# NilsJochem/audio-matcher

Hardware: AMD Instinct MI355X
Metric: audio samples/s matched (whole node), 10 s needle vs 1 h haystack, 1/2/4/8 GPU (higher is better)
Workload: dtype f32

## Files before the change

audio-matcher_amd/csrc/am_api.hip:

```cpp
#include "am_internal.h"

#include <climits>

using namespace am;


static size_t mode_len(size_t w, size_t s, int mode) {
    if (mode == AM_MODE_FULL) return w + s - 1;
    if (mode == AM_MODE_SAME) return w;
    return (w > s ? w - s : 0) + 1;
}


int am::find_peaks_host_array(Ctx* c, const float* d_scores, long long n, float min_prom, long long min_dist,
                              std::vector<am_peak>& all) {
    int rc;
    const PeakPolicy pol = snapshot_opts(nullptr).peak_policy();
    Segment sg; sg.a = 0; sg.b = n;
    PeakArena arena{};
    if ((rc = prepare_results(c, 1, AM_MAX_PEAKS_PER_CHUNK, &arena))) return rc;
    if ((rc = c->side[0].peaks.ensure(sizeof(am_peak) * AM_MAX_PEAKS_PER_CHUNK))) return rc;
    if ((rc = upload_segments(c, std::vector<Segment>(1, sg)))) return rc;
    if ((rc = launch_pick(c, c->side[0], d_scores, n, 0, 1, min_prom, min_dist, nullptr, nullptr, 0, arena, pol))) return rc;
    AM_HIP(hipStreamSynchronize(c->stream));
// ... 460 lines not shown
    AM_HIP(launch_synth(c->stream, d_out, seed, stream, first, (long long)n, amp));
    AM_HIP(hipStreamSynchronize(c->stream));
    return AM_OK;
}

int am_axpy_device(int device, float* d_dst, const float* d_src, size_t n, float gain) {
    if (!d_dst || !d_src) return fail(AM_ERR_INVALID_ARG, "null pointer");
    Ctx* c = nullptr;
    int rc = get_ctx(device, &c);
    if (rc) return rc;
    if (n == 0) return AM_OK;
    std::lock_guard<std::recursive_mutex> lk(c->mu);
    AM_HIP(launch_axpy(c->stream, d_dst, d_src, (long long)n, gain));
    AM_HIP(hipStreamSynchronize(c->stream));
    return AM_OK;
}

int am_synth_pcm16_stereo_device(int device, int16_t* d_out, uint32_t seed, uint32_t stream, uint64_t first, size_t frames, float amp) {
    if (!d_out) return fail(AM_ERR_INVALID_ARG, "null pointer");
    Ctx* c = nullptr;
    int rc = get_ctx(device, &c);
    if (rc) return rc;
    if (frames == 0) return AM_OK;
    std::lock_guard<std::recursive_mutex> lk(c->mu);
    AM_HIP(launch_synth_pcm16(c->stream, d_out, seed, stream, first, (long long)frames, amp));
    AM_HIP(hipStreamSynchronize(c->stream));
    return AM_OK;
}

int am_add_pcm16_device(int device, int16_t* d_dst, const int16_t* d_src, size_t frames) {
    if (!d_dst || !d_src) return fail(AM_ERR_INVALID_ARG, "null pointer");
    Ctx* c = nullptr;
    int rc = get_ctx(device, &c);
    if (rc) return rc;
    if (frames == 0) return AM_OK;
    std::lock_guard<std::recursive_mutex> lk(c->mu);
    AM_HIP(launch_add_pcm16(c->stream, d_dst, d_src, (long long)frames));
    AM_HIP(hipStreamSynchronize(c->stream));
    return AM_OK;
}


int am_debug_column_bench(int device, int wide, int npairs, int iters, int dense, double* k1_ms, double* k3_ms) {
    Ctx* c = nullptr;
    int rc = get_ctx(device, &c);
    if (rc) return rc;
    std::lock_guard<std::recursive_mutex> lk(c->mu);
    if (npairs < 1 || npairs > 64 || iters < 1 || !k1_ms || !k3_ms) return fail(AM_ERR_INVALID_ARG, "bad arguments");
    const Plan* pl = nullptr;
    if ((rc = wide ? get_plan(c, 23, &pl, 9) : get_plan(c, 22, &pl))) return rc;
    const long long N = 1ll << pl->dev.logN, s = 441000, hop = ((N - s + 1) / kTile) * kTile;
    const long long nblocks = 2ll * npairs, out_count = nblocks * hop, src_len = out_count + s - 1 + kTile;
    DevBuf src, work, scores, stats32, side;
    struct Release { DevBuf* b[5]; ~Release() { for (DevBuf* x : b) x->release(); } } release_all{{&src, &work, &scores, &stats32, &side}};
    if ((rc = src.ensure((size_t)src_len * 4)) || (rc = work.ensure((size_t)npairs * (size_t)N * sizeof(float2))) ||
        (rc = scores.ensure((size_t)out_count * 4)) || (rc = stats32.ensure((size_t)(out_count / 32) * sizeof(float2))) ||
        (rc = side.ensure(sparse_bytes(nblocks, pl->dev)))) return rc;
    AM_HIP(launch_synth(c->stream, (float*)src.p, 7, 1, 0, src_len, 0.25f));
    Job job{};
    job.src = src.p; job.src_len = src_len; job.lead = 0; job.src_kind = 0;
    job.dst = (float*)scores.p; job.out_count = out_count; job.hop = (int)hop; job.nblocks = (int)nblocks; job.first_pair = 0;
    ScanCfg scan{};
    fill_scan_cfg(&scan, stats32.p, side.p, nblocks, pl->dev, dense ? -1.0f : 1e30f, FLT_MAX, 60 * 44100, 70 * 44100 - s);
    hipEvent_t e[3];
    for (auto& x : e) AM_HIP(hipEventCreate(&x));
    double t1 = 0, t3 = 0;
    for (int it = -2; it < iters; ++it) {
        AM_HIP(hipEventRecord(e[0], c->stream));
        AM_HIP(launch_k1(c->stream, job, npairs, (float2*)work.p, pl->dev, 0));
        AM_HIP(hipEventRecord(e[1], c->stream));
        AM_HIP(launch_k3(c->stream, job, npairs, (const float2*)work.p, pl->dev, 1e-3f, scan, 0, false));
        AM_HIP(hipEventRecord(e[2], c->stream));
        AM_HIP(hipStreamSynchronize(c->stream));
        float a = 0, b = 0;
        AM_HIP(hipEventElapsedTime(&a, e[0], e[1]));
        AM_HIP(hipEventElapsedTime(&b, e[1], e[2]));
        if (it >= 0) { t1 += a; t3 += b; }
    }
    for (auto& x : e) (void)hipEventDestroy(x);
    *k1_ms = t1 / iters; *k3_ms = t3 / iters;
    return AM_OK;
}

}
```

audio-matcher_amd/csrc/am_context.hip:

```cpp
#include "am_internal.h"

namespace am {

thread_local std::string t_err;

int fail(int code, const std::string& msg) {
    t_err = msg;
    return code;
}
int hip_fail(hipError_t e, const char* what) {
    char buf[256];
    snprintf(buf, sizeof(buf), "%s: %s", what, hipGetErrorString(e));
    t_err = buf;
    return e == hipErrorOutOfMemory ? AM_ERR_OOM : AM_ERR_HIP;
}

static std::mutex g_hooks_mu;
static Hooks g_hooks;
Hooks snapshot_hooks() {
    std::lock_guard<std::mutex> lk(g_hooks_mu);
    return g_hooks;
}

using OptRule = const char* (*)(long long& v);
static const char* opt_any(long long&) { return nullptr; }
static const char* opt_bool(long long& v) { v = v ? 1 : 0; return nullptr; }
static const char* opt_log_n(long long& v) { return v != 0 && (v < kLogNMin || v > kLogNMax) ? "log_n out of range" : nullptr; }
static const char* opt_half(long long& v) { v = v <= 0 ? 0 : (v >= 2 ? 2 : 1); return nullptr; }
static const char* opt_every(long long& v) { v = v < 1 ? 1 : v; return nullptr; }
static const char* opt_arm_at(long long& v) { v = v < -1 ? -2 : v; return nullptr; }
static const char* opt_needle_group(long long& v) { return v < 1 || v > kMaxNeedleGroup ? "needle_group out of range" : nullptr; }
static const char* opt_pairs(long long& v) { return v < 1 || v > 64 ? "pairs_per_group out of range" : nullptr; }
static const char* opt_score_norm(long long& v) { return v < 0 || v > 1 ? "score_norm out of range (0 = off, 1 = NCC)" : nullptr; }
static const char* opt_floor_db(long long& v) { return v < 0 || v > 200 ? "score_norm_floor_db out of range (0..200)" : nullptr; }
static const char* opt_trace_form(long long& v) { return v < 0 || v > 2 ? "trace_form out of range (0 = by bin length, 1 = wave form, 2 = sliced form)" : nullptr; }
static const char* opt_distance(long long& v) {
    return v < 0 || v > 3 ? "distance_rule out of range (bit 0: inclusive, bit 1: between plateau starts)" : nullptr;
}
struct Option {
    const char* name;
    std::atomic<long long> value;
    OptRule rule;
    long long Opts::*field;
};
static Option g_options[] = {
    {"log_n", {0}, opt_log_n, &Opts::log_n},
    {"pairs_per_group", {64}, opt_pairs, &Opts::pairs_per_group},
    {"profile_mask", {-1}, opt_any, &Opts::profile_mask},
    {"profile_every", {1}, opt_every, &Opts::profile_every},
    {"half_pipeline", {0}, opt_half, &Opts::half},
    {"batch_overlap", {1}, opt_bool, &Opts::batch_overlap},
    {"needle_group", {8}, opt_needle_group, &Opts::needle_group},
    {"pick_stream_priority", {0}, opt_bool, &Opts::pick_priority},
    {"pick_group", {1}, opt_bool, &Opts::pick_group},
    {"k3_group", {1}, opt_bool, &Opts::k3_group},
    {"host_pick_wait", {1}, opt_bool, &Opts::host_pick_wait},
    {"device_redo", {1}, opt_bool, &Opts::device_redo},
    {"tail_block", {1}, opt_bool, &Opts::tail_block},
    {"dense_scores", {0}, opt_bool, &Opts::dense},
    {"score_norm", {0}, opt_score_norm, &Opts::score_norm},
    {"score_norm_floor_db", {60}, opt_floor_db, &Opts::score_norm_floor_db},
    {"debug_no_realloc", {0}, opt_bool, &Opts::debug_no_realloc},
    {"debug_redo_arm_at", {-2}, opt_arm_at, &Opts::debug_redo_arm_at},
    {"trace_form", {0}, opt_trace_form, &Opts::trace_form},
    {"peak_filter_order", {0}, opt_bool, &Opts::peak_filter_order},
    {"distance_rule", {0}, opt_distance, &Opts::distance_rule},
    {"tail_window", {0}, opt_bool, &Opts::tail_window},
    {"surrounding_from", {0}, opt_bool, &Opts::surrounding_from},
};
static Option* find_option(const char* key) {
    for (Option& r : g_options)
        if (!strcmp(key, r.name)) return &r;
    return nullptr;
}

thread_local const Opts* t_opts_pin = nullptr;
Opts snapshot_opts(const am_needle* h) {
    if (t_opts_pin) return *t_opts_pin;
    Opts o;
    for (const Option& r : g_options) o.*r.field = r.value.load(std::memory_order_relaxed);
    if (h && h->opt_log_n >= 0) o.log_n = h->opt_log_n;
    if (h && h->opt_half >= 0) o.half = h->opt_half;
    if (h && h->opt_score_norm >= 0) o.score_norm = h->opt_score_norm;
    return o;
}

thread_local int t_no_realloc = 0;
int realloc_refused(const char* what, size_t bytes, size_t cap) {
    char buf[160];
    snprintf(buf, sizeof(buf), "debug_no_realloc: %s buffer would grow from %zu to %zu bytes while a call is queueing", what, cap, bytes);
    return fail(AM_ERR_HIP, buf);
}

static const char* kKernelNames[] = {"k1_cols_fwd", "k2_rows", "k3_cols_inv", "tile_stats", "peaks", "other", "trace", "discover"};
static std::mutex g_ctx_mu;
static std::map<int, Ctx*> g_ctx;

int get_ctx(int device, Ctx** out) {
    std::lock_guard<std::mutex> lk(g_ctx_mu);
    int n = 0;
    hipError_t e = hipGetDeviceCount(&n);
    if (e != hipSuccess || n <= 0) return fail(AM_ERR_NO_DEVICE, "no HIP device available");
    if (device < 0 || device >= n) return fail(AM_ERR_NO_DEVICE, "device ordinal out of range");
    auto it = g_ctx.find(device);
    if (it != g_ctx.end()) { *out = it->second; AM_HIP(hipSetDevice(device)); return AM_OK; }
    AM_HIP(hipSetDevice(device));
    (void)hipSetDeviceFlags(hipDeviceScheduleSpin);
    (void)hipGetLastError();
    AM_HIP(fft_kernels_init());
    Ctx* c = new Ctx();
    c->device = device;
    c->hdr.flags = hipHostMallocMapped | hipHostMallocCoherent;
    c->failcnt.flags = hipHostMallocMapped | hipHostMallocCoherent;
    c->spill.flags = hipHostMallocMapped | hipHostMallocCoherent;
    hipError_t se = hipStreamCreateWithFlags(&c->stream, hipStreamNonBlocking);
    if (se != hipSuccess) { delete c; return hip_fail(se, "hipStreamCreate"); }
    {
        int least = 0, greatest = 0;
        if (snapshot_opts(nullptr).pick_priority && hipDeviceGetStreamPriorityRange(&least, &greatest) == hipSuccess && least != greatest)
            (void)hipStreamCreateWithPriority(&c->stream2, hipStreamNonBlocking, least);
        else
            (void)hipStreamCreateWithFlags(&c->stream2, hipStreamNonBlocking);
        (void)hipGetLastError();
    }
    (void)hipStreamCreateWithFlags(&c->stream_tail, hipStreamNonBlocking);
    (void)hipEventCreateWithFlags(&c->ev_fork, kSyncEvent);
    (void)hipEventCreateWithFlags(&c->ev_join, kSyncEvent);
    (void)hipGetLastError();
    for (int i = 0; i < 2; ++i) {
        (void)hipEventCreateWithFlags(&c->ev_k3[i], kSyncEvent);
        (void)hipEventCreateWithFlags(&c->ev_pick[i], kSyncEvent);
    }
    g_ctx[device] = c;
    *out = c;
    return AM_OK;
}

static hipEvent_t prof_event(Ctx* c) {
    if (!c->pool.empty()) { hipEvent_t e = c->pool.back(); c->pool.pop_back(); return e; }
    hipEvent_t e = nullptr;
    (void)hipEventCreateWithFlags(&e, AM_EVENT_NO_SYSTEM_FENCE ? hipEventDisableSystemFence : hipEventDefault);
// ... 445 lines not shown
```

audio-matcher_amd/csrc/am_correlate.hip:

```cpp
#include "am_internal.h"

namespace am {

static int pick_log_n(size_t s, long long out_count, const Opts& o, int* logN_out) {
    int min_log = kLogNMin;
    while (min_log <= kLogNMax && ((size_t)1 << min_log) < s + 1) ++min_log;
    if (min_log > kLogNMax) return fail(AM_ERR_INVALID_ARG, "needle too long for a forced transform size (2^23 at most; leave log_n at 0 for needle partitioning)");
    if (o.log_n > 0) {
        int l = (int)o.log_n;
        if (l < min_log) l = min_log;
        if (l > kLogNMax) l = kLogNMax;
        *logN_out = l;
        return AM_OK;
    }
    const long long span = out_count + (long long)s - 1;
    if (span > (1ll << 19)) {
        if ((long long)s <= kWideFromSamples) { *logN_out = 21; return AM_OK; }
        if ((long long)s <= kWidestFromSamples) {
            long long hop21 = (1ll << 21) - (long long)s + 1;
            if (hop21 >= 8 * kTile) hop21 = (hop21 / kTile) * kTile;
            *logN_out = (hop21 > 0 && out_count <= 2 * hop21) ? 21 : 22;
            return AM_OK;
        }
        if ((long long)s <= kSegmentFrom) {
            long long hop22 = (1ll << 22) - (long long)s + 1;
            if (hop22 >= 8 * kTile) hop22 = (hop22 / kTile) * kTile;
            *logN_out = (hop22 > 0 && out_count <= 2 * hop22) ? 22 : 23;
            return AM_OK;
        }
    }
    int pref = min_log;
    while (pref < kLogNMax) {
        const double n = (double)((size_t)1 << pref);
        if ((n - (double)s + 1.0) / n >= kMinEfficiency) break;
        ++pref;
    }
    int single = kLogNMin;
    while (single < kLogNMax && (long long)((size_t)1 << single) < span) ++single;
    *logN_out = std::min(pref, std::max(single, min_log));
    return AM_OK;
}

int plan_geometry(size_t s, long long out_count, const Opts& o, Geometry* g) {
    int rc = pick_log_n(s, out_count, o, &g->logN);
    if (rc) return rc;
    g->N = 1ll << g->logN;
    g->hop = g->N - (long long)s + 1;
    if (g->hop >= 8 * kTile) g->hop = (g->hop / kTile) * kTile;
    g->nblocks = (out_count + g->hop - 1) / g->hop;
    g->npairs = (g->nblocks + 1) / 2;
    return AM_OK;
}
bool tail_plan(size_t s, long long out_count, const Opts& o, const Geometry& g, TailPlan* t) {
    t->on = false;
    if (!o.tail_block || o.log_n != 0 || g.logN < 22 || !(g.nblocks & 1) || g.nblocks < 3 || (g.hop % kTile) != 0) return false;
    const long long T = (g.nblocks - 1) * g.hop, rest = out_count - T;
    for (int lt = 21; lt < g.logN; ++lt) {
        const long long N = 1ll << lt;
        long long hop = N - (long long)s + 1;
        if (hop < 8 * kTile) continue;
        hop = (hop / kTile) * kTile;
        if (2 * hop < rest) continue;
        t->on = true; t->T = T;
        t->g.logN = lt; t->g.N = N; t->g.hop = hop; t->g.nblocks = (rest + hop - 1) / hop; t->g.npairs = 1;
        return true;
    }
    return false;
}

static size_t sparse_word_bytes(long long nblocks, const PlanDev& pl) {
    return sizeof(unsigned long long) * (size_t)nblocks * ballot_layout(pl.logN1, pl.logN2).words;
}
size_t sparse_bytes(long long nblocks, const PlanDev& pl) {
    return sparse_word_bytes(nblocks, pl) + sizeof(float) * (size_t)nblocks * ballot_layout(pl.logN1, pl.logN2).tiles;
}
void fill_scan_cfg(ScanCfg* cfg, void* stats32, void* side, long long nblocks, const PlanDev& pl, float margin, float hist_min,
                          long long seg_c, long long seg_d) {
    cfg->stats32 = static_cast<float2*>(stats32);
    cfg->wbits = static_cast<unsigned long long*>(side);
    cfg->tile_theta = reinterpret_cast<float*>(static_cast<char*>(side) + sparse_word_bytes(nblocks, pl));
    cfg->margin = margin;
    cfg->hist_min = hist_min;
    cfg->seg_c = seg_c; cfg->seg_d = seg_d;
    cfg->inv_c = seg_c > 0 ? 1.0 / (double)seg_c : 0.0;
}
SparseScores sparse_view(const ScanCfg& cfg, long long hop, const PlanDev& pl) {
    if (cfg.margin < 0.0f) return SparseScores{nullptr, cfg.stats32, nullptr, (int)hop, pl.logN2, pl.logN1, 1.0 / (double)hop};
    return SparseScores{cfg.wbits, cfg.stats32, cfg.tile_theta, (int)hop, pl.logN2, pl.logN1, 1.0 / (double)hop};
}

bool needle_is_segmented(const am_needle* h, const Opts& o) {
    return (long long)h->n > kSegmentFrom && o.log_n == 0;
}
static void needle_segments(am_needle* h) {
    if (!h->segments.empty()) return;
    const long long n = (long long)h->n;
    const long long nseg = (n + kSegmentLen - 1) / kSegmentLen;
    for (long long i = 0; i < nseg; ++i) {
        const long long a = n * i / nseg, b = n * (i + 1) / nseg;
        am_needle* sub = new am_needle();
        sub->ctx = h->ctx; sub->d_needle = h->d_needle + a; sub->n = (size_t)(b - a);
        sub->inv_autocorr = h->inv_autocorr; sub->owns_data = false;
        h->segments.push_back(sub);
        h->seg_off.push_back(a);
    }
}

bool plan_fuses_scan(const PlanDev& pl, const Geometry& g) { return plan_has_scan(pl) && (g.hop % kTile) == 0; }

int pass_plan(am_needle* h, const Opts& o, long long out_count, bool allow_tail, PassPlan* pp) {
    Ctx* c = h->ctx;
    *pp = PassPlan{};
    int rc;
    if (needle_is_segmented(h, o)) {
        pp->kind = PassKind::Partitioned;
        needle_segments(h);
        Opts os = o;
        os.half = 0;
        pp->parts.resize(h->segments.size());
        for (size_t i = 0; i < pp->parts.size(); ++i) {
            if ((rc = pass_plan(h->segments[i], os, out_count, false, &pp->parts[i]))) return rc;
            pp->need.work = std::max(pp->need.work, pp->parts[i].need.work);
        }
        return AM_OK;
    }
    if (h->n <= (size_t)kDirectMaxNeedle && o.log_n == 0) return AM_OK;
    pp->kind = PassKind::Transform;
    Geometry& g = pp->g;
    if ((rc = plan_geometry(h->n, out_count, o, &g))) return rc;
    if ((rc = get_plan(c, g.logN, &pp->pl))) return rc;
    if ((rc = needle_k2_spectrum(h, o, pp->pl, &pp->hc, &pp->hs))) return rc;
    pp->fused = plan_fuses_scan(pp->pl->dev, g);
    if (allow_tail && pp->fused && c->stream_tail && c->ev_fork && c->ev_join && tail_plan(h->n, out_count, o, g, &pp->tail)) {
        if ((rc = get_plan(c, pp->tail.g.logN, &pp->tail_pl))) return rc;
        if ((rc = needle_k2_spectrum(h, o, pp->tail_pl, &pp->tail_hc, &pp->tail_hs))) return rc;
        pp->need.work_tail = (size_t)pp->tail.g.N * sizeof(float2);
    }
    pp->nblocks = pp->tail.on ? g.nblocks - 1 : g.nblocks;
    pp->npairs = pp->tail.on ? g.npairs - 1 : g.npairs;
    pp->main_count = pp->tail.on ? pp->tail.T : out_count;
    pp->ppg = std::min(std::max<long long>(1, o.pairs_per_group), pp->npairs);
    pp->need.work = (size_t)pp->ppg * (size_t)g.N * sizeof(float2);
    pp->need.npairs = g.npairs;
    if (pp->fused) {
        pp->need.stats32 = (size_t)((out_count + 31) / 32) * sizeof(float2);
        pp->need.side = sparse_bytes(g.nblocks, pp->pl->dev);
    }
    return AM_OK;
}

static int run_tail_block(Ctx* c, const PassPlan& pp, const void* d_src, long long src_len,
                          float* d_dst, long long out_count, float factor, const ScanCfg& main_scan, int src_kind) {
    hipStream_t st = c->stream_tail;
    const TailPlan& tail = pp.tail;
    const PlanDev& pl = pp.tail_pl->dev;
    const HalfScale& hs = pp.tail_hs;
    int rc;
    if ((rc = c->work_tail.ensure(pp.need.work_tail))) return rc;
    Job job = tail_job(tail, d_src, src_len, out_count, src_kind);
    job.dst = d_dst + tail.T;
    ScanCfg scan{};
    scan.stats32 = main_scan.stats32 ? main_scan.stats32 + tail.T / 32 : nullptr;
    scan.margin = -1.0f; scan.hist_min = FLT_MAX;
    { ProfScope ps(c, KN_OTHER, st); AM_HIP(launch_k1(st, job, 1, (float2*)c->work_tail.p, pl, hs.level)); }
    { ProfScope ps(c, KN_OTHER, st); AM_HIP(launch_k2(st, 1, (float2*)c->work_tail.p, pp.tail_hc, pl, nullptr, hs.level, hs.hscale, hs.pre, true)); }
    { ProfScope ps(c, KN_OTHER, st); AM_HIP(launch_k3(st, job, 1, (const float2*)c->work_tail.p, pl, hs.k3(factor), scan, hs.level, false)); }
    if (main_scan.stats32 && main_scan.margin >= 0.0f && main_scan.wbits && main_scan.tile_theta) {
        const BallotLayout bl = ballot_layout(pp.pl->dev.logN1, pp.pl->dev.logN2);
        const size_t blk = (size_t)(pp.g.nblocks - 1);
        AM_HIP(hipMemsetAsync(main_scan.wbits + blk * bl.words, 0xFF, bl.words * sizeof(unsigned long long), st));
        AM_HIP(hipMemsetD32Async(reinterpret_cast<hipDeviceptr_t>(main_scan.tile_theta + blk * bl.tiles), (int)0xFF7FFFFFu, bl.tiles, st));
    }
    return AM_OK;
}

static int run_correlation_one(am_needle* h, const PassPlan& pp, const void* d_src, long long src_len, long long lead,
                               float* d_dst, long long out_count, float factor,
                               const ScanRequest* scan_req, ScanResult* res, int src_kind, bool accumulate);

int run_correlation(am_needle* h, const Opts& o, const void* d_src, long long src_len, long long lead,
                           float* d_dst, long long out_count, float factor,
                           const ScanRequest* scan_req, ScanResult* res, int src_kind, const PassPlan* plan) {
    int rc;
    PassPlan own;
    if (!plan) {
        if ((rc = pass_plan(h, o, out_count, scan_req && !scan_req->no_scan && lead == 0, &own))) return rc;
        plan = &own;
    }
    if (res) { res->fused = false; res->redo_ok = false; res->sparse = plain_scores(); }
    if (plan->kind != PassKind::Partitioned) return run_correlation_one(h, *plan, d_src, src_len, lead, d_dst, out_count, factor, scan_req, res, src_kind, false);
    if (scan_req && scan_req->skip_launch) return fail(AM_ERR_INVALID_ARG, "internal: streaming ingest does not run early pairs for partitioned needles");
    for (size_t i = 0; i < plan->parts.size(); ++i) {
        ScanRequest plain{};
        if (scan_req) {
            plain.margin = -1.0f; plain.range_a = scan_req->range_a; plain.range_b = scan_req->range_b;
            plain.before_k3 = i == 0 ? scan_req->before_k3 : nullptr;
            plain.no_scan = true;
        }
        if ((rc = run_correlation_one(h->segments[i], plan->parts[i], d_src, src_len, lead - h->seg_off[i], d_dst, out_count, factor,
                                      scan_req ? &plain : nullptr, nullptr, src_kind, i > 0)))
            return rc;
    }
    return AM_OK;
}

static int run_correlation_one(am_needle* h, const PassPlan& pp, const void* d_src, long long src_len, long long lead,
                               float* d_dst, long long out_count, float factor,
                               const ScanRequest* scan_req, ScanResult* res, int src_kind, bool accumulate) {
    Ctx* c = h->ctx;
    Job job{};
    job.src = d_src; job.src_len = src_len; job.lead = lead; job.src_kind = src_kind;
    job.dst = d_dst; job.out_count = out_count;
    if (pp.kind == PassKind::Direct) {
        ProfScope ps(c, KN_OTHER);
        AM_HIP(launch_direct(c->stream, job, h->d_needle, (int)h->n, factor));
        return AM_OK;
    }
    int rc;
    const PlanDev& pl = pp.pl->dev;
    const HalfScale& hs = pp.hs;
    const TailPlan& tail = pp.tail;
    const long long N = pp.g.N, hop = pp.g.hop, npairs = pp.npairs, ppg = pp.ppg;
    const ScanBuffers out = (scan_req && scan_req->out.work) ? scan_req->out : scan_buffers(c->side[0]);
    DevBuf& wk = *out.work;
    if ((rc = wk.ensure((size_t)ppg * (size_t)N * sizeof(float2)))) return rc;
    ScanCfg scan{};
    bool fused = false;
    if (scan_req && !scan_req->no_scan) {
        if (res) res->sparse = SparseScores{nullptr, nullptr, nullptr, (int)hop, pl.logN2, pl.logN1, 1.0 / (double)hop};
        if (pp.fused) {
            const long long side_blocks = std::max(pp.g.nblocks, scan_req->side_nblocks);
            if ((rc = out.stats32->ensure((size_t)((out_count + 31) / 32) * sizeof(float2)))) return rc;
            if ((rc = out.wflags->ensure(sparse_bytes(side_blocks, pl)))) return rc;
            fill_scan_cfg(&scan, out.stats32->p, out.wflags->p, side_blocks, pl, scan_req->margin, scan_req->hist_min, scan_req->seg_c, scan_req->seg_d);
            fused = true;
            if (res) { res->fused = true; res->sparse = sparse_view(scan, hop, pl); }
        }
    }
    const float k3scale = hs.k3(factor);
    job.out_count = pp.main_count; job.hop = (int)hop; job.nblocks = (int)pp.nblocks;
    if (scan_req && scan_req->skip_launch) return AM_OK;
    long long pair_lo = 0, pair_hi = npairs;
    bool with_tail = tail.on;
    if (scan_req && scan_req->range_b > scan_req->range_a) {
        pair_lo = (scan_req->range_a / hop) / 2;
        pair_hi = std::min(npairs, ((scan_req->range_b - 1) / hop) / 2 + 1);
        with_tail = tail.on && scan_req->range_b > tail.T;
    }
    if (scan_req && scan_req->tail_by_caller) with_tail = false;
// ... 268 lines not shown
```

audio-matcher_amd/csrc/am_engine.hip:

```cpp
#include "am_internal.h"

namespace am {

static int launch_pick_group(Ctx* c, const K3Group& kg, long long n_scores, int seg_off, int nsegs, float min_prom, long long min_dist,
                             const SparseScores& sp_common, int* bad, const int* hdr_off, const PeakArena& arena, const PeakPolicy& pol,
                             hipStream_t st) {
    if (nsegs == 0 || n_scores <= 0 || kg.n <= 0) return AM_OK;
    int rc;
    const size_t nz = (size_t)kg.n, total = nz * (size_t)nsegs;
    const long long ntiles = (n_scores + kTile - 1) / kTile;
    PickGroup pg{};
    pg.n = kg.n;
    for (int z = 0; z < kg.n; ++z) {
        if ((rc = c->grp_stats[z].ensure((size_t)ntiles * sizeof(float2)))) return rc;
        pg.g[z] = kg.dst[z]; pg.stats[z] = static_cast<float2*>(c->grp_stats[z].p);
        pg.stats32[z] = kg.stats32[z]; pg.wbits[z] = kg.wbits[z]; pg.theta[z] = kg.tile_theta[z];
        pg.hdr_off[z] = hdr_off[z];
    }
    { ProfScope ps(c, KN_STATS, st);
      AM_HIP(launch_stats_reduce(st, pg.stats32[0], n_scores, pg.stats[0], bad, &pg)); }
    if ((rc = wide_reserve(c, total))) return rc;
    if ((rc = c->side[0].peaks.ensure(total * AM_MAX_PEAKS_PER_CHUNK * sizeof(am_peak)))) return rc;
    {
        ProfScope ps(c, KN_PEAKS, st);
// ... 56 lines not shown
            ScoreSide& sd = c->side[set];
            if ((rc = sd.scores.ensure(max_scores * sizeof(float)))) return rc;
            if ((rc = sd.peaks.ensure(sizeof(am_peak) * max_segs * AM_MAX_PEAKS_PER_CHUNK))) return rc;
            if ((rc = sd.stats.ensure((max_scores + kTile - 1) / kTile * sizeof(float2)))) return rc;
        }
        return wide_reserve(c, max_segs);
    }
    int wait_pick(bool on_host) {
        if (!overlap || seq < 2) return AM_OK;
        if (on_host) AM_HIP(hipEventSynchronize(c->ev_pick[set()]));
        else AM_HIP(hipStreamWaitEvent(c->stream, c->ev_pick[set()], 0));
        return AM_OK;
    }
    int k3_done() {
        if (!overlap) return AM_OK;
        AM_HIP(hipEventRecord(c->ev_k3[set()], c->stream));
        AM_HIP(hipStreamWaitEvent(c->stream2, c->ev_k3[set()], 0));
        return AM_OK;
    }
    int pick_done() {
        if (overlap) AM_HIP(hipEventRecord(c->ev_pick[set()], c->stream2));
        ++seq;
        return AM_OK;
    }
    int drain() {
        AM_HIP(hipStreamSynchronize(c->stream));
        if (overlap) AM_HIP(hipStreamSynchronize(c->stream2));
        return AM_OK;
    }
};

static int match_alone(am_needle* h, const void* d_hay, size_t len, const am_match_params* p, am_peak* out, size_t cap, size_t slot,
                       size_t* n_out, int src_kind, const PartSpec* part, int* worst) {
    const int rc = match_many(h, &d_hay, &len, 1, p, out ? out + slot * cap : nullptr, cap, &n_out[slot], src_kind, 0, 1, false, nullptr, part);
    if (rc == AM_ERR_CAPACITY) *worst = rc;
    return rc == AM_ERR_CAPACITY ? AM_OK : rc;
}

static int pick_alone(am_needle* h, const Opts& o, const am_match_params* p, const void* src, long long src_len, float factor,
                      const ScanRequest& req, long long n_scores, int seg_idx, const Segment& sg, int spare_hdr, uint64_t shift, int src_kind,
                      const NormSpec& nrm, std::vector<am_peak>& all) {
    Ctx* c = h->ctx;
    const PeakPolicy pol = o.peak_policy();
    int rc;
    PeakArena own{};
    if ((rc = c->spill.ensure(sizeof(am_peak) * AM_MAX_PEAKS_PER_CHUNK))) return rc;
    AM_HIP(hipMemsetAsync(c->arena_cur.p, 0, sizeof(unsigned), c->stream));
    own.base = static_cast<am_peak*>(c->spill.p); own.cursor = static_cast<unsigned*>(c->arena_cur.p);
    own.cap = AM_MAX_PEAKS_PER_CHUNK;
    ScoreSide& side = c->side[0];
    if ((rc = side.scores.ensure((size_t)n_scores * sizeof(float)))) return rc;
    float* d_scores = (float*)side.scores.p;
    ScanResult res{};
    if ((rc = run_correlation(h, o, src, src_len, 0, d_scores, n_scores, factor, &req, &res, src_kind))) return rc;
    if (nrm.on) {
        if ((rc = normalise_scores(c, c->stream, nrm, src, src_len, src_kind, 0, (long long)h->n, d_scores, sg.a, std::min(sg.b, n_scores))))
            return rc;
        res.fused = false;
    }
    if ((rc = launch_pick(c, side, d_scores, n_scores, seg_idx, 1, p->min_prominence, (long long)p->min_distance, nullptr, &res, spare_hdr, own, pol))) return rc;
    AM_HIP(hipStreamSynchronize(c->stream));
    const SegHeader& hd = static_cast<const SegHeader*>(c->hdr.p)[spare_hdr];
    const size_t old = all.size();
    if (hd.overflow & 1) {
        if ((rc = pick_chunk_big(c, d_scores, n_scores, seg_idx, sg, p->min_prominence, (long long)p->min_distance, &res, hd.seg_min, all, pol)))
            return rc;
    } else append_header_peaks(hd, own, all);
    for (size_t j = old; j < all.size(); ++j) { all[j].start += shift; all[j].end += shift; }
    return AM_OK;
}

struct TailSlots { size_t scores, stats; };
static bool tail_batchable(const TailPlan& t) { return t.on && t.g.logN == 21; }
static int launch_tail_batch(am_needle* h, const std::vector<PassPlan>& plans, const std::vector<size_t>& members, int half_idx,
                             const TailSlots& sl, const void* const* d_hays, const size_t* lens, float factor, int src_kind) {
    Ctx* c = h->ctx;
    const PassPlan& lead = plans[members[0]];
    const TailPlan& first = lead.tail;
    const Plan* pl = lead.tail_pl;
    const float2* hc = lead.tail_hc;
    const HalfScale& hs = lead.tail_hs;
    TailBatch tb{};
    tb.n = (int)members.size();
    for (int j = 0; j < tb.n; ++j) {
        const size_t k = members[j];
        const size_t slot = (size_t)half_idx * kMaxTailBatch + (size_t)j;
        const Job job = tail_job(plans[k].tail, d_hays[k], (long long)lens[k], (long long)(lens[k] - h->n + 1), src_kind);
        tb.src[j] = job.src;
        tb.src_len[j] = job.src_len;
        tb.out_count[j] = job.out_count;
        tb.dst[j] = static_cast<float*>(c->tail_scores.p) + slot * sl.scores;
        tb.stats32[j] = static_cast<float2*>(c->tail_stats.p) + slot * sl.stats;
    }
    float2* work = static_cast<float2*>(c->work_tail.p);
    { ProfScope ps(c, KN_OTHER); AM_HIP(launch_tail_batch_k1(c->stream, tb, (int)first.g.hop, src_kind, work, pl->dev, hs.level)); }
    { ProfScope ps(c, KN_OTHER); AM_HIP(launch_k2(c->stream, tb.n, work, hc, pl->dev, nullptr, hs.level, hs.hscale, hs.pre, true)); }
    { ProfScope ps(c, KN_OTHER); AM_HIP(launch_tail_batch_k3(c->stream, tb, (int)first.g.hop, work, pl->dev, hs.k3(factor), hs.level)); }
    return AM_OK;
}

static int classify_nonfinite(am_needle* h, const PassPlan& pp, const float* d_hay, size_t len,
                              const std::vector<Segment>& segs, int s0, int s1,
                              std::vector<char>* drop, std::vector<char>* again) {
    Ctx* c = h->ctx;
    const long long s = (long long)h->n;
    const int nch = s1 - s0;
    drop->assign(nch, 0); again->assign(nch, 0);
    std::vector<Segment> ranges;
    for (int i = s0; i < s1; ++i)
        ranges.push_back(Segment{segs[i].a, std::min<long long>((long long)len, segs[i].b + s - 1)});
    const long long npairs = pp.kind == PassKind::Transform ? pp.npairs : 0;
    for (long long q = 0; q < npairs; ++q) ranges.push_back(pp.pair_reads(q, (long long)len));
    if (pp.tail.on) ranges.push_back(pp.tail_reads((long long)len));
    std::vector<int> flags(ranges.size(), 0);
    int rc = nonfinite_flags(c, d_hay, ranges.data(), (int)ranges.size(), flags.data());
    if (rc) return rc;
    for (int i = 0; i < nch; ++i) {
        if (flags[i]) { (*drop)[i] = 1; continue; }
        if (pp.kind == PassKind::Partitioned) { (*again)[i] = 1; continue; }
        const Segment sg = segs[s0 + i];
        for (long long q = 0; q < npairs && !(*again)[i]; ++q)
            if (flags[nch + q] && 2 * q * pp.g.hop < sg.b && (2 * q + 2) * pp.g.hop > sg.a) (*again)[i] = 1;
        if (pp.tail.on && flags[nch + npairs] && pp.tail.T < sg.b) (*again)[i] = 1;
    }
    return AM_OK;
}

int match_many(am_needle* h, const void* const* d_hays, const size_t* lens, size_t n_hay,
               const am_match_params* p, am_peak* out, size_t cap_per_hay, size_t* n_out, int src_kind,
               size_t index_base, size_t index_stride, bool fire_hooks, const StreamPre* pre, const PartSpec* part) {
    Ctx* c = h->ctx;
    const Opts o = snapshot_opts(h);
    const PeakPolicy pol = o.peak_policy();
    Hooks hooks = fire_hooks ? snapshot_hooks() : Hooks{};
    if (part) hooks.fn = nullptr;
    if (part && n_hay != 1) return fail(AM_ERR_INVALID_ARG, "internal: a part is one haystack");
    auto G = [&](size_t k) { return index_base + k * index_stride; };
    const size_t s = h->n;
    if (p->chunk == 0) return fail(AM_ERR_INVALID_ARG, "chunk must be > 0");
    if (p->scale < AM_SCALE_NONE || p->scale > AM_SCALE_MY) return fail(AM_ERR_INVALID_ARG, "bad scale");
    const NormSpec nrm = norm_spec(h, o);
    if (nrm.on && (pre || part)) return fail(AM_ERR_INVALID_ARG, AM_NORM_UNSUPPORTED);
    int rc = norm_check(nrm, p->scale);
    if (rc) return rc;
    const bool my = p->scale == AM_SCALE_MY;
    const float factor = nrm.on ? norm_factor(nrm) : scale_factor(h, p->scale, (size_t)(p->chunk + p->overlap));
    const int sm = p->scale == AM_SCALE_LIB ? 1 : 0;
    ScanRequest base{};
    base.margin = nrm.on ? -1.0f : write_margin(o, p);
    const bool sparse_ok = base.margin >= 0.0f;
    base.hist_min = nrm.on ? FLT_MAX : h->hist_min(sm);
    base.seg_c = (long long)p->chunk;
    base.seg_d = (long long)(p->chunk + p->overlap) - (long long)s;
    for (size_t k = 0; k < n_hay; ++k) n_out[G(k)] = 0;
    ChunkPlan cp;
    plan_chunks(s, d_hays, lens, n_hay, p, o, my, part ? part->max_windows : (size_t)-1, &cp);
    const std::vector<Segment>& segs = cp.segs;
    const std::vector<int>& seg_off = cp.seg_off;
    const size_t nsegs = segs.size();
    if (nsegs == 0 && cp.short_segs.empty()) return AM_OK;
    if (cp.too_many(1)) return fail(AM_ERR_INVALID_ARG, "chunk size too small for this haystack (more than 2^18 chunks)");
    size_t n_active = 0;
    for (size_t k = 0; k < n_hay; ++k) n_active += cp.ns(k) > 0;
    ScoreSets sets(c, o, n_active);
    if ((rc = sets.size(cp.max_scores, cp.max_segs))) return rc;
    std::vector<PassPlan> plans(n_hay);
    Footprint need;
    for (size_t k = 0; k < n_hay; ++k) {
        if (cp.n_chunks[k] == 0 || cp.ns(k) == 0) continue;
        if ((rc = pass_plan(h, o, (long long)(lens[k] - s + 1), pre == nullptr, &plans[k]))) return rc;
        need.take(plans[k].need);
    }
    std::vector<int> tail_slot(n_hay, -1);
    TailSlots tslots{0, 0};
    bool batch_tails = false;
    if (need.work_tail) {
        size_t n_tails = 0;
        for (size_t k = 0; k < n_hay; ++k)
            if (tail_batchable(plans[k].tail)) {
                ++n_tails;
// ... 289 lines not shown
        tail_plan(s, out_count, o, geo[k], &tails[k]);
    }
    std::map<int, std::vector<const float2*>> hcs;
    auto spectra = [&](int logN) -> int {
        if (hcs.count(logN)) return AM_OK;
        const Plan* pl = nullptr;
        int rc2 = get_plan(c, logN, &pl);
        std::vector<const float2*>& v = hcs[logN];
        v.resize(m);
        HalfScale hs;
        for (size_t i = 0; i < m && !rc2; ++i) rc2 = needle_k2_spectrum(needles[ord[i]], o, pl, &v[i], &hs);
        return rc2;
    };
    for (size_t k = 0; k < n_hay; ++k)
        if (ns_max(k) > 0 && (rc = spectra(geo[k].logN))) return rc;
    const size_t group_opt = (size_t)std::min<long long>(std::max<long long>(1, o.needle_group), kMaxNeedleGroup);
    {
        const bool groups_ok = o.k3_group && group_opt > 1 && m > 1 && !o.half && (m % group_opt) != 1 && c->stream_tail != nullptr;
        for (size_t k = 0; k < n_hay; ++k) {
            if (!tails[k].on) continue;
            const Plan* plk = nullptr;
            if (ns_max(k) == 0 || !groups_ok || !tail_batchable(tails[k]) || get_plan(c, geo[k].logN, &plk) || !plan_is_c512(plk->dev)) {
                tails[k].on = false;
                continue;
            }
            max_tail = std::max(max_tail, (size_t)tails[k].g.N);
            if ((rc = spectra(tails[k].g.logN))) return rc;
        }
        if (max_tail) {
            if ((rc = c->work_tail.ensure(std::max(c->work_tail.cap, max_tail * sizeof(float2))))) return rc;
            if ((rc = c->work_tail2.ensure(std::min(group_opt, m) * max_tail * sizeof(float2)))) return rc;
        }
    }
    size_t n_pairs_active = 0;
    for (size_t k = 0; k < n_hay; ++k) n_pairs_active += ns_max(k) > 0 ? m : 0;
    ScoreSets sets(c, o, n_pairs_active);
    DevBuf& fwd = c->side[0].work;
    if ((rc = fwd.ensure(max_matrix * sizeof(float2)))) return rc;
    if ((rc = c->work2.ensure(std::min(group_opt, m) * max_matrix * sizeof(float2)))) return rc;
    if ((rc = sets.size(max_scores, max_segs))) return rc;
    for (int set = 0; set < sets.count(); ++set) {
        if ((rc = c->side[set].stats32.ensure((max_scores + 31) / 32 * sizeof(float2)))) return rc;
        if ((rc = c->side[set].wflags.ensure(max_wflags))) return rc;
    }
    const size_t k3_group = (o.k3_group && group_opt > 1 && m > 1 && !o.half && max_wflags > 0) ? std::min(group_opt, m) : 0;
    for (int set = 0; set < sets.count(); ++set)
        for (size_t q = 0; q < k3_group; ++q) {
            if ((rc = c->grp_scores[set][q].ensure(max_scores * sizeof(float)))) return rc;
            if ((rc = c->grp_stats32[set][q].ensure((max_scores + 31) / 32 * sizeof(float2)))) return rc;
            if ((rc = c->grp_wflags[set][q].ensure(max_wflags))) return rc;
        }
    if (k3_group && o.pick_group) {
        const size_t total = k3_group * max_segs;
        for (size_t z = 0; z < k3_group; ++z)
            if ((rc = c->grp_stats[z].ensure((max_scores + kTile - 1) / kTile * sizeof(float2)))) return rc;
        if ((rc = wide_reserve(c, total))) return rc;
        if ((rc = c->side[0].peaks.ensure(total * AM_MAX_PEAKS_PER_CHUNK * sizeof(am_peak)))) return rc;
    }
    PeakArena arena{};
    if ((rc = prepare_results(c, nhdr, nhdr * 8 + 4096, &arena))) return rc;
    if ((rc = upload_segments(c, all_segs))) return rc;
    if ((rc = c->badflag.ensure(sizeof(int) * n_hay))) return rc;
    int* h_bad = static_cast<int*>(c->badflag.p);
    memset(h_bad, 0, sizeof(int) * n_hay);
    SegHeader* h_hdr = static_cast<SegHeader*>(c->hdr.p);
    const float margin = write_margin(o, p);
    QueueingScope queueing(o.debug_no_realloc != 0);
    for (size_t k = 0; k < n_hay; ++k) {
        if (ns_max(k) == 0) continue;
        if (hooks.fn) hooks.fn(hooks.user, G(k), 0, (size_t)ns_max(k));
        const Geometry& g = geo[k];
        const Plan* pl = nullptr;
        if ((rc = get_plan(c, g.logN, &pl))) return rc;
        const std::vector<const float2*>& hc = hcs[g.logN];
        const long long out_count = (long long)(lens[k] - s_min + 1);
        const int half = (o.half && (plan_is_r16(pl->dev) || plan_is_c512(pl->dev))) ? (o.half >= 2 ? 2 : 1) : 0;
        const size_t group = (!half && plan_k2_has_group(pl->dev)) ? group_opt : 1;
        const size_t matrix = (size_t)g.npairs * (size_t)g.N;
        const bool fused = plan_fuses_scan(pl->dev, g);
        const TailPlan& tail = tails[k];
        const int main_pairs = (int)(tail.on ? g.npairs - 1 : g.npairs);
        const Plan* plt = nullptr;
        Job job{}, job_t{};
        job.src = d_hays[k]; job.src_len = (long long)lens[k]; job.lead = 0; job.src_kind = src_kind;
        job.out_count = tail.on ? tail.T : out_count; job.hop = (int)g.hop; job.nblocks = (int)(tail.on ? g.nblocks - 1 : g.nblocks); job.first_pair = 0;
        { ProfScope ps(c, KN_K1); AM_HIP(launch_k1(c->stream, job, main_pairs, (float2*)fwd.p, pl->dev, half)); }
        if (tail.on) {
            if ((rc = get_plan(c, tail.g.logN, &plt))) return rc;
            job_t = tail_job(tail, d_hays[k], (long long)lens[k], out_count, src_kind);
            ProfScope ps(c, KN_OTHER);
            AM_HIP(launch_k1(c->stream, job_t, 1, (float2*)c->work_tail.p, plt->dev, 0));
        }
        for (size_t i = 0; i < m; ++i) {
            am_needle* h = needles[ord[i]];
            const size_t in_group = i % group;
            const float2* inv_rows = (const float2*)c->work2.p + in_group * matrix;
            const size_t gn = std::min(group, m - (i - in_group));
            if (group > 1 && in_group == 0) {
                K2Group grp{};
                grp.n = (int)gn;
                for (int q = 0; q < grp.n; ++q) { grp.hc[q] = hc[i + q]; grp.dst[q] = (float2*)c->work2.p + (size_t)q * matrix; }
                { ProfScope ps(c, KN_K2); AM_HIP(launch_k2_group(c->stream, main_pairs, (const float2*)fwd.p, grp, pl->dev)); }
                if (tail.on) {
                    K2Group gt{};
                    gt.n = (int)gn;
                    const std::vector<const float2*>& hct = hcs[tail.g.logN];
                    for (int q = 0; q < gt.n; ++q) { gt.hc[q] = hct[i + q]; gt.dst[q] = (float2*)c->work_tail2.p + (size_t)q * (size_t)tail.g.N; }
                    ProfScope ps(c, KN_OTHER);
                    AM_HIP(launch_k2_group(c->stream, 1, (const float2*)c->work_tail.p, gt, plt->dev));
                }
            }
            const bool grouped_k3 = k3_group && group > 1 && gn > 1 && fused && !half && plan_k3_has_group(pl->dev);
            if (grouped_k3 && in_group != 0) continue;
            const int set = sets.set();
            if (grouped_k3) {
                K3Group kg{};
                kg.n = (int)gn;
                ScanResult scans[kMaxNeedleGroup];
                int* const bad = (src_kind == 0 || o.half) ? &h_bad[k] : nullptr;
                ScanCfg common{};
                bool same_plan = true, same_edges = true;
                for (size_t q = 0; q < gn; ++q) {
                    am_needle* hq = needles[ord[i + q]];
                    ScanCfg cfg{};
                    fill_scan_cfg(&cfg, c->grp_stats32[set][q].p, c->grp_wflags[set][q].p, g.nblocks, pl->dev, margin, hq->hist_min(sm),
                                  (long long)p->chunk, (long long)(p->chunk + pj[ord[i + q]].overlap) - (long long)hq->n);
                    scans[q] = ScanResult{};
                    scans[q].fused = true;
                    scans[q].sparse = sparse_view(cfg, g.hop, pl->dev);
                    if (q == 0) common = cfg;
                    same_plan = same_plan && plan_of[i + q] == plan_of[i];
                    same_edges = same_edges && cfg.seg_d == common.seg_d;
                    kg.work[q] = (const float2*)c->work2.p + q * matrix;
                    kg.dst[q] = (float*)c->grp_scores[set][q].p;
                    kg.stats32[q] = cfg.stats32; kg.wbits[q] = cfg.wbits; kg.tile_theta[q] = cfg.tile_theta;
                    kg.hist_min[q] = cfg.hist_min;
                    kg.out_scale[q] = half_scale(hq, o, pl->dev).k3(scale_factor(hq, p->scale, 1));
                    kg.out_count[q] = std::max(0ll, std::min(count_of(k, i + q), job.out_count));
                    kg.seg_d[q] = cfg.seg_d;
                }
                kg.seg_c = common.seg_c; kg.inv_c = common.inv_c;
                if (!same_edges) common.seg_c = 0;
                if ((rc = sets.wait_pick(false))) return rc;
                { ProfScope ps(c, KN_K3); AM_HIP(launch_k3_group(c->stream, job, main_pairs, kg, pl->dev, common)); }
                if (tail.on) {
                    K3Group kt = kg;
                    for (size_t q = 0; q < gn; ++q) {
                        kt.work[q] = (const float2*)c->work_tail2.p + q * (size_t)tail.g.N;
                        kt.dst[q] = kg.dst[q] + tail.T; kt.stats32[q] = kg.stats32[q] + tail.T / 32;
                        kt.wbits[q] = nullptr; kt.tile_theta[q] = nullptr; kt.hist_min[q] = FLT_MAX;
                        kt.out_count[q] = std::max(0ll, count_of(k, i + q) - tail.T);
                        kt.seg_d[q] = 0;
                    }
                    kt.seg_c = 0; kt.inv_c = 0.0;
                    ScanCfg dense{};
                    dense.stats32 = kt.stats32[0]; dense.margin = -1.0f; dense.hist_min = FLT_MAX;
                    ProfScope ps(c, KN_OTHER);
                    AM_HIP(launch_k3_group(c->stream, job_t, 1, kt, plt->dev, dense));
                    if (margin >= 0.0f)
                        AM_HIP(launch_tail_preset_group(c->stream, kg, (long long)(g.nblocks - 1), pl->dev.logN1, pl->dev.logN2));
                }
                if ((rc = sets.k3_done())) return rc;
                if (o.pick_group && same_plan && plan_i(i).ns(k) > 0) {
                    int hoff[kMaxNeedleGroup];
                    for (size_t q = 0; q < gn; ++q) hoff[q] = hdr_of(k, i + q);
                    if ((rc = launch_pick_group(c, kg, count_of(k, i), seg_of(k, i), plan_i(i).ns(k), p->min_prominence, (long long)p->min_distance,
                                                scans[0].sparse, bad, hoff, arena, pol, sets.pick_stream()))) return rc;
                } else
                for (size_t q = 0; q < gn; ++q)
                    if (plan_i(i + q).ns(k) > 0 &&
                        (rc = launch_pick(c, c->side[0], kg.dst[q], count_of(k, i + q), seg_of(k, i + q), plan_i(i + q).ns(k), p->min_prominence,
                                          (long long)p->min_distance, bad, &scans[q], hdr_of(k, i + q), arena, pol, sets.pick_stream()))) return rc;
                if ((rc = sets.pick_done())) return rc;
                continue;
            }
            const int ns = plan_i(i).ns(k);
            if (ns == 0) continue;
            float* d_scores = sets.scores();
            Job jn = job;
            jn.dst = d_scores;
            jn.out_count = std::min(count_of(k, i), job.out_count);
            ScoreSide& side = sets.side();
            int* const bad = (src_kind == 0 || o.half) ? &h_bad[k] : nullptr;
            ScanResult scan{};
            scan.fused = fused;
            scan.sparse = SparseScores{nullptr, nullptr, nullptr, (int)g.hop, pl->dev.logN2, pl->dev.logN1, 1.0 / (double)g.hop};
            ScanCfg cfg{};
            if (fused) {
                fill_scan_cfg(&cfg, side.stats32.p, side.wflags.p, g.nblocks, pl->dev, margin, h->hist_min(sm), (long long)p->chunk,
                              (long long)(p->chunk + pj[ord[i]].overlap) - (long long)h->n);
                scan.sparse = sparse_view(cfg, g.hop, pl->dev);
            }
            const float factor = scale_factor(h, p->scale, 1);
            const HalfScale hs = half_scale(h, o, pl->dev);
            if (group == 1) {
                ProfScope ps(c, KN_K2);
                AM_HIP(launch_k2(c->stream, (int)g.npairs, (float2*)fwd.p, hc[i], pl->dev, (float2*)c->work2.p, hs.level, hs.hscale, hs.pre));
            }
            if ((rc = sets.wait_pick(false))) return rc;
            { ProfScope ps(c, KN_K3); AM_HIP(launch_k3(c->stream, jn, (int)g.npairs, inv_rows, pl->dev, hs.k3(factor), cfg, half)); }
            if ((rc = sets.k3_done())) return rc;
            if ((rc = launch_pick(c, side, d_scores, count_of(k, i), seg_of(k, i), ns, p->min_prominence, (long long)p->min_distance,
                                  bad, &scan, hdr_of(k, i), arena, pol, sets.pick_stream()))) return rc;
            if ((rc = sets.pick_done())) return rc;
        }
    }
    queueing.end();
    if ((rc = sets.drain())) return rc;
    std::vector<am_peak> all;
    std::vector<std::pair<size_t, size_t>> redo;
    for (size_t k = 0; k < n_hay; ++k) {
        for (size_t i = 0; i < m; ++i) {
            const int ns = plan_i(i).ns(k);
            if (ns == 0) continue;
            const size_t j = ord[i];
            const SegHeader* hd = h_hdr + hdr_of(k, i);
            const size_t slot = G(k) * nn + j;
            bool again = h_bad[k] != 0;
            float lowest = FLT_MAX;
            for (int q = 0; q < ns && !again; ++q) {
                if (hd[q].overflow & 7) again = true;
                lowest = std::min(lowest, hd[q].seg_min);
            }
            if (!again) needles[j]->remember_min(sm, lowest);
            if (again) { redo.emplace_back(k, j); continue; }
            all.clear();
            for (int q = 0; q < ns; ++q) append_header_peaks(hd[q], arena, all);
            rc = merge_peaks(all, &pj[j], o.surrounding_from != 0, out ? out + slot * cap_per_pair : nullptr, cap_per_pair, &n_out[slot]);
            if (rc == AM_ERR_CAPACITY) worst = rc;
            else if (rc) return rc;
        }
    }
    for (const auto& kj : redo)
        if ((rc = match_alone(needles[kj.second], d_hays[kj.first], lens[kj.first], &pj[kj.second], out, cap_per_pair, G(kj.first) * nn + kj.second,
                              n_out, src_kind, nullptr, &worst))) return rc;
    if (hooks.fn)
        for (size_t k = 0; k < n_hay; ++k)
            if (ns_max(k) > 0) hooks.fn(hooks.user, G(k), 1, (size_t)ns_max(k));
    return worst;
}

// ... 2 lines not shown
```

audio-matcher_amd/csrc/am_fft.hip:

```cpp
#include "am_kernels.h"

#include <float.h>
#include <stdlib.h>
#include <algorithm>
#include <atomic>
#include <hip/hip_fp16.h>

namespace am {

__device__ __forceinline__ float2 cadd(float2 a, float2 b) { return make_float2(a.x + b.x, a.y + b.y); }
__device__ __forceinline__ float2 csub(float2 a, float2 b) { return make_float2(a.x - b.x, a.y - b.y); }
__device__ __forceinline__ float2 cmul(float2 a, float2 b) {
    return make_float2(a.x * b.x - a.y * b.y, a.x * b.y + a.y * b.x);
}
__device__ __forceinline__ float2 cmulc(float2 a, float2 b) {
    return make_float2(a.x * b.x + a.y * b.y, a.y * b.x - a.x * b.y);
}
__device__ __forceinline__ float2 mul_neg_i(float2 a) { return make_float2(a.y, -a.x); }
__device__ __forceinline__ float2 mul_pos_i(float2 a) { return make_float2(-a.y, a.x); }

__device__ __forceinline__ float2 tw_big(const PlanDev& pl, unsigned m) {
    return cmul(pl.twhi[m >> pl.logLo], pl.twlo[m & ((1u << pl.logLo) - 1u)]);
}

// ... 263 lines not shown
struct K1Twiddles { float2 w256, w256q, base0, base1, step0, step1, step0q, step1q; };
__device__ __forceinline__ K1Twiddles k1_twiddles(const PlanDev& pl, long long col, int hi) {
    const unsigned maskN = (unsigned)((1ll << pl.logN) - 1);
    K1Twiddles w;
    w.w256 = pl.tw1[hi];
    w.w256q = pl.tw1[4 * hi];
    w.base0 = tw_big(pl, ((unsigned)col * (unsigned)hi) & maskN);
    w.base1 = tw_big(pl, (((unsigned)col + 1u) * (unsigned)hi) & maskN);
    tw_big_pair(pl, ((unsigned)col * 16u) & maskN, w.step0, w.step0q);
    tw_big_pair(pl, (((unsigned)col + 1u) * 16u) & maskN, w.step1, w.step1q);
    return w;
}
template <int KIND>
__device__ __forceinline__ void k1_load(const Job& job, long long col, int in_stride, int hi, long long baseA, long long baseB,
                                        bool validB, bool fast, float2 (&x0)[16], float2 (&x1)[16]) {
    if (fast) {
#pragma unroll
        for (int a = 0; a < 16; ++a) {
            const long long off = (long long)(a * 16 + hi) * in_stride + col;
            const float2 va = load_sample2<KIND>(job.src, baseA + off), vb = load_sample2<KIND>(job.src, baseB + off);
            x0[a] = make_float2(va.x, vb.x);
            x1[a] = make_float2(va.y, vb.y);
        }
    } else {
#pragma unroll
        for (int a = 0; a < 16; ++a) {
            const long long n = (long long)(a * 16 + hi) * in_stride + col;
            const float2 va = load2_padded<KIND>(job.src, baseA + n, job.src_len);
            const float2 vb = validB ? load2_padded<KIND>(job.src, baseB + n, job.src_len) : make_float2(0.f, 0.f);
            x0[a] = make_float2(va.x, vb.x);
            x1[a] = make_float2(va.y, vb.y);
        }
    }
}
__device__ __forceinline__ void k1_transform(const K1Twiddles& w, float2* lds2, int hi, int cp, float2 (&x0)[16], float2 (&x1)[16]) {
    dif<16, false>(x0);
    dif<16, false>(x1);
    twiddle_brev<16, false>(x0, w.w256, w.w256q);
    twiddle_brev<16, false>(x1, w.w256, w.w256q);
#pragma unroll
    for (int ap = 0; ap < 16; ++ap) lds2[(ap * 16 + hi) * 17 + cp] = x0[brev<16>(ap)];
    __syncthreads();
#pragma unroll
    for (int b = 0; b < 16; ++b) x0[b] = lds2[(hi * 16 + b) * 17 + cp];
    __syncthreads();
#pragma unroll
    for (int ap = 0; ap < 16; ++ap) lds2[(ap * 16 + hi) * 17 + cp] = x1[brev<16>(ap)];
    __syncthreads();
#pragma unroll
    for (int b = 0; b < 16; ++b) x1[b] = lds2[(hi * 16 + b) * 17 + cp];
    dif<16, false>(x0);
    dif<16, false>(x1);
    twiddle_chain<16, false, true>(x0, w.base0, w.step0, w.step0q);
    twiddle_chain<16, false, true>(x1, w.base1, w.step1, w.step1q);
}
template <int KIND>
__device__ __forceinline__ void k1_tile(const Job& job, const PlanDev& pl, float2* lds2, long long col, int in_stride,
                                        int hi, int cp, long long baseA, long long baseB, bool validB, bool fast,
                                        float2 (&x0)[16], float2 (&x1)[16]) {
    const K1Twiddles w = k1_twiddles(pl, col, hi);
    k1_load<KIND>(job, col, in_stride, hi, baseA, baseB, validB, fast, x0, x1);
    k1_transform(w, lds2, hi, cp, x0, x1);
}

__device__ __forceinline__ void k1_transform_h16(const K1Twiddles& w, uint2* ldsu, int hi, int cp, h2 (&x0)[16], h2 (&x1)[16]) {
    dif<16, false>(x0);
    dif<16, false>(x1);
    twiddle_apply2<16, false, true>(x0, x1, w.w256);
#pragma unroll
    for (int ap = 0; ap < 16; ++ap) ldsu[(ap * 16 + hi) * 17 + cp] = make_uint2(h2_bits(x0[brev<16>(ap)]), h2_bits(x1[brev<16>(ap)]));
    __syncthreads();
#pragma unroll
    for (int b = 0; b < 16; ++b) {
        const uint2 v = ldsu[(hi * 16 + b) * 17 + cp];
        x0[b] = bits_h2(v.x);
        x1[b] = bits_h2(v.y);
    }
    dif<16, false>(x0);
    dif<16, false>(x1);
    twiddle_chain<16, false, true>(x0, w.base0, w.step0);
    twiddle_chain<16, false, true>(x1, w.base1, w.step1);
}

template <int KIND, int HALF>
__device__ __forceinline__ void k1_cols_fwd_r16_tile(const Job& job, float2* __restrict__ work, const PlanDev& pl) {
    extern __shared__ float4 lds4[];
    const int t = threadIdx.x;
    const int hi = t >> 4, cp = t & 15;
    const int n2_0 = blockIdx.x << kColsLog;
    const int pair = job.first_pair + blockIdx.y;
    const long long blkA = 2ll * pair, blkB = blkA + 1;
    const bool validB = blkB < job.nblocks;
    const long long N = 1ll << pl.logN;
    const long long baseA = blkA * job.hop - job.lead;
    const long long baseB = blkB * job.hop - job.lead;
    const bool fast = ((reinterpret_cast<uintptr_t>(job.src) & 7) == 0) && ((baseA & 1) == 0) && ((baseB & 1) == 0) &&
                      baseA >= 0 && baseA + N <= job.src_len && validB && baseB + N <= job.src_len;
    float2 x0[16], x1[16];
    if constexpr (HALF == 2) {
        const long long col = (long long)n2_0 + 2 * cp;
        const K1Twiddles w = k1_twiddles(pl, col, hi);
        k1_load<KIND>(job, col, kN2, hi, baseA, baseB, validB, fast, x0, x1);
        h2 hx0[16], hx1[16];
#pragma unroll
        for (int a = 0; a < 16; ++a) { hx0[a] = to_h2(x0[a]); hx1[a] = to_h2(x1[a]); }
        k1_transform_h16(w, reinterpret_cast<uint2*>(lds4), hi, cp, hx0, hx1);
        uint2* __restrict__ out2 = reinterpret_cast<uint2*>(reinterpret_cast<unsigned*>(work) + ((size_t)blockIdx.y << pl.logN) + n2_0) + cp;
#pragma unroll
        for (int bp = 0; bp < 16; ++bp) {
            const size_t k1 = (size_t)(hi + 16 * bp);
            out2[k1 * (kN2 / 2)] = make_uint2(h2_bits(hx0[brev<16>(bp)]), h2_bits(hx1[brev<16>(bp)]));
        }
        return;
    }
    k1_tile<KIND>(job, pl, reinterpret_cast<float2*>(lds4), (long long)n2_0 + 2 * cp, kN2, hi, cp, baseA, baseB, validB, fast, x0, x1);
    if (HALF) {
        uint2* __restrict__ out2 = reinterpret_cast<uint2*>(reinterpret_cast<unsigned*>(work) + ((size_t)blockIdx.y << pl.logN) + n2_0) + cp;
#pragma unroll
        for (int bp = 0; bp < 16; ++bp) {
            const size_t k1 = (size_t)(hi + 16 * bp);
            out2[k1 * (kN2 / 2)] = make_uint2(pack_h2(x0[brev<16>(bp)]), pack_h2(x1[brev<16>(bp)]));
        }
        return;
    }
    float4* __restrict__ out4 = reinterpret_cast<float4*>(work + ((size_t)blockIdx.y << pl.logN) + n2_0) + cp;
#pragma unroll
    for (int bp = 0; bp < 16; ++bp) {
        const size_t k1 = (size_t)(hi + 16 * bp);
        out4[k1 * (kN2 / 2)] = make_float4(x0[brev<16>(bp)].x, x0[brev<16>(bp)].y,
                                             x1[brev<16>(bp)].x, x1[brev<16>(bp)].y);
    }
}
template <int KIND, int HALF>
__global__ void __launch_bounds__(256, 3)
k1_cols_fwd_r16(Job job, float2* __restrict__ work, PlanDev pl) {
    k1_cols_fwd_r16_tile<KIND, HALF>(job, work, pl);
}
template <int KIND, int HALF>
__global__ void __launch_bounds__(256, 3)
tail_cols_fwd_r16(TailBatch tb, int hop, float2* __restrict__ work, PlanDev pl) {
    const unsigned z = blockIdx.y;
    Job job;
    job.src = tb.src[z]; job.src_len = tb.src_len[z]; job.lead = 0; job.dst = nullptr; job.out_count = tb.out_count[z];
    job.hop = hop; job.nblocks = (int)((tb.out_count[z] + hop - 1) / hop); job.first_pair = -(int)z; job.src_kind = KIND;
    k1_cols_fwd_r16_tile<KIND, HALF>(job, work, pl);
}

__device__ __forceinline__ void wave_sync_lds() {
    __builtin_amdgcn_fence(__ATOMIC_ACQ_REL, "wavefront");
    __builtin_amdgcn_wave_barrier();
}

struct K2Lane {
    int t, hi, cp;
    unsigned voff;
    float2 wj0, wj1, wc0, wc1;
    float2 qj0, qj1, qc0, qc1;
};
__device__ __forceinline__ K2Lane k2_lane(const PlanDev& pl, int t = threadIdx.x) {
    K2Lane k;
    k.t = t; k.hi = k.t >> 4; k.cp = k.t & 15;
    k.voff = (unsigned)k.t * 16u;
    const float4 j = pl.k2j[2 * k.t], jq = pl.k2j[2 * k.t + 1], c = pl.k2c[2 * k.cp], cq = pl.k2c[2 * k.cp + 1];
    k.wj0 = make_float2(j.x, j.y); k.wj1 = make_float2(j.z, j.w);
    k.qj0 = make_float2(jq.x, jq.y); k.qj1 = make_float2(jq.z, jq.w);
    k.wc0 = make_float2(c.x, c.y); k.wc1 = make_float2(c.z, c.w);
    k.qc0 = make_float2(cq.x, cq.y); k.qc1 = make_float2(cq.z, cq.w);
    return k;
}

__device__ __forceinline__ void k2_forward12(const K2Lane& k, __amdgpu_buffer_rsrc_t rrow, float4* lds4) {
    const int t = k.t, hi = k.hi, cp = k.cp;
    float2 x0[16], x1[16];
#pragma unroll
    for (int a = 0; a < 16; ++a) {
        const float4 v = buf_load4(rrow, k.voff, a * 4096);
        x0[a] = make_float2(v.x, v.y);
        x1[a] = make_float2(v.z, v.w);
    }
    dif<16, false>(x0);
    dif<16, false>(x1);
    twiddle_brev<16, false>(x0, k.wj0, k.qj0);
    twiddle_brev<16, false>(x1, k.wj1, k.qj1);
#pragma unroll
    for (int ap = 0; ap < 16; ++ap)
        lds4[ap * 256 + t] = make_float4(x0[brev<16>(ap)].x, x0[brev<16>(ap)].y,
                                         x1[brev<16>(ap)].x, x1[brev<16>(ap)].y);
    __syncthreads();
#pragma unroll
    for (int b = 0; b < 16; ++b) {
        const float4 v = lds4[hi * 256 + b * 16 + cp];
        x0[b] = make_float2(v.x, v.y);
        x1[b] = make_float2(v.z, v.w);
    }
    dif<16, false>(x0);
    dif<16, false>(x1);
    twiddle_brev<16, false>(x0, k.wc0, k.qc0);
    twiddle_brev<16, false>(x1, k.wc1, k.qc1);
    wave_sync_lds();
#pragma unroll
    for (int bp = 0; bp < 16; ++bp)
        lds4[(hi * 16 + bp) * 16 + (cp ^ bp)] = make_float4(x0[brev<16>(bp)].x, x0[brev<16>(bp)].y,
                                                            x1[brev<16>(bp)].x, x1[brev<16>(bp)].y);
    wave_sync_lds();
}

__device__ __forceinline__ void k2_forward3(const K2Lane& k, const float4* lds4, float2 (&z)[32]) {
#pragma unroll
    for (int i = 0; i < 16; ++i) {
        const float4 v = lds4[k.t * 16 + (i ^ k.cp)];
        z[2 * i] = make_float2(v.x, v.y);
        z[2 * i + 1] = make_float2(v.z, v.w);
    }
    dif<32, false>(z);
}

__device__ __forceinline__ void k2_fetch_quarter(__amdgpu_buffer_rsrc_t rh, unsigned voff, int part, float4 (&h)[4]) {
#pragma unroll
    for (int i = 0; i < 4; ++i) h[i] = buf_load4(rh, voff, (part * 4 + i) * 4096);
}
__device__ __forceinline__ void k2_multiply_quarter(const float2 (&z)[32], const float4 (&h)[4], int part, float2 (&q)[32]) {
#pragma unroll
    for (int i = 0; i < 4; ++i) {
        const int e = part * 4 + i;
        q[brev<32>(2 * e)] = cmul(z[2 * e], make_float2(h[i].x, h[i].y));
        q[brev<32>(2 * e + 1)] = cmul(z[2 * e + 1], make_float2(h[i].z, h[i].w));
    }
}
// ... 632 lines not shown
#pragma unroll
    for (int a = 0; a < 16; ++a) {
        const unsigned pos = chunk ^ ((((unsigned)a & 3u) << 1) | hb);
        lds2[a * (16 << HB) + hi * 16 + (int)((pos << 1) | half)] = make_float2(c0[a], c1[a]);
    }
}
template <int HB>
__device__ __forceinline__ void scan_row_minmax(const float4* lds4, int row, bool whole, int nvalid, float& mn, float& mx) {
    const unsigned k = scan_swizzle<HB>((unsigned)row);
    float4 v[8];
#pragma unroll
    for (int i = 0; i < 8; ++i) v[i] = lds4[row * 8 + (int)((unsigned)i ^ k)];
    if (!whole) {
        mn = FLT_MAX; mx = -FLT_MAX;
#pragma unroll
        for (int i = 0; i < 8; ++i) {
            const int c0 = i << 2;
            const float e[4] = {v[i].x, v[i].y, v[i].z, v[i].w};
#pragma unroll
            for (int j = 0; j < 4; ++j)
                if (c0 + j < nvalid) { mn = fminf(mn, e[j]); mx = fmaxf(mx, e[j]); }
        }
        return;
    }
    mn = min3_raw(v[0].x, v[0].y, v[0].z); mx = max3_raw(v[0].x, v[0].y, v[0].z);
    mn = min3_raw(mn, v[0].w, v[1].x);     mx = max3_raw(mx, v[0].w, v[1].x);
#pragma unroll
    for (int i = 1; i < 8; ++i) {
        if (i > 1) { mn = min3_raw(mn, v[i - 1].w, v[i].x); mx = max3_raw(mx, v[i - 1].w, v[i].x); }
        mn = min3_raw(mn, v[i].y, v[i].z); mx = max3_raw(mx, v[i].y, v[i].z);
    }
    mn = fminf(mn, v[7].w); mx = fmaxf(mx, v[7].w);
}

__device__ __forceinline__ long long mod_recip(long long x, long long c, double inv_c) {
    long long q = (long long)((double)x * inv_c);
    long long r = x - q * c;
    if (r < 0) r += c;
    else if (r >= c) r -= c;
    return r;
}
__device__ __forceinline__ bool run_has_chunk_edge(long long lo, long long c, long long d, double inv_c) {
    if (c <= 0) return true;
    if (mod_recip(lo + 31, c, inv_c) <= 31) return true;
    const long long hi2 = lo + 31 - d;
    if (hi2 < 0) return false;
    return mod_recip(hi2, c, inv_c) <= 31;
}

struct K3Edges {
    long long outA, outB;
    int relcA, reldA, relcB, reldB;
    bool one_edge;
};
__device__ __forceinline__ K3Edges k3_edges(const Job& job, const ScanCfg& scan, long long blkA, long long blkB) {
    K3Edges e;
    e.outA = blkA * job.hop; e.outB = blkB * job.hop;
    e.one_edge = scan.stats32 != nullptr && scan.seg_c >= (long long)job.hop + 32;
    e.relcA = e.reldA = e.relcB = e.reldB = 0x7fffffff;
    if (scan.edges_n > 0) {
        const int s = (int)(blkA >> 1) - job.first_pair;
        e.relcA = scan.edge_rel[s][0]; e.reldA = scan.edge_rel[s][1];
        e.relcB = scan.edge_rel[s][2]; e.reldB = scan.edge_rel[s][3];
        return e;
    }
    if (e.one_edge) {
        const long long c = scan.seg_c, d = scan.seg_d;
        const long long m = mod_recip(e.outA, c, scan.inv_c);
        const long long ecA = m == 0 ? e.outA : e.outA + (c - m);
        long long edA = d;
        if (e.outA > d) {
            const long long m2 = mod_recip(e.outA - d, c, scan.inv_c);
            edA = m2 == 0 ? e.outA : e.outA + (c - m2);
        }
        const long long ecB = ecA >= e.outB ? ecA : ecA + c;
        const long long edB = edA >= e.outB ? edA : edA + c;
        auto rel = [](long long edge, long long start) { const long long r = edge - start; return r < 0x7fffffffll ? (int)r : 0x7fffffff; };
        e.relcA = rel(ecA, e.outA); e.reldA = rel(edA, e.outA);
        e.relcB = rel(ecB, e.outB); e.reldB = rel(edB, e.outB);
    }
    return e;
}

template <int HB, bool ACC = false, bool SCALED = false>
__device__ __forceinline__ void k3_finish(const Job& job, const ScanCfg& scan, const K3Edges& ed, float2* lds2,
                                          int n2_0, int out_stride, int t, long long blkA, long long blkB,
                                          float out_scale, const float2 (&x0)[16], const float2 (&x1)[16]) {
    const int hi = t >> 4, cp = t & 15;
    const long long col = n2_0 + 2 * cp;
    const long long outA = ed.outA, outB = ed.outB;
    const bool one_edge = ed.one_edge;
    const bool dst8 = ((reinterpret_cast<uintptr_t>(job.dst) & 7) == 0) && ((job.hop & 1) == 0);
    long long limA = job.out_count - outA; if (limA > job.hop) limA = job.hop;
    long long limB = blkB < job.nblocks ? job.out_count - outB : 0; if (limB > job.hop) limB = job.hop;
    float sa0[16], sa1[16], sb0[16], sb1[16];
#pragma unroll
    for (int a = 0; a < 16; ++a) {
        const float2 v0 = x0[brev<16>(a)], v1 = x1[brev<16>(a)];
        if (SCALED) {
            sa0[a] = v0.x; sa1[a] = v1.x;
            sb0[a] = v0.y; sb1[a] = v1.y;
        } else {
            sa0[a] = v0.x * out_scale; sa1[a] = v1.x * out_scale;
            sb0[a] = v0.y * out_scale; sb1[a] = v1.y * out_scale;
        }
    }
    unsigned wantA[2] = {0x11111111u, 0x11111111u}, wantB[2] = {0x11111111u, 0x11111111u};
    if (!ACC && scan.stats32 != nullptr) {
        const int row = scan_row_of<HB>(t);
        const int rowrun = row * out_stride + n2_0;
        const int leftA = (int)limA - rowrun, leftB = (int)limB - rowrun;
        const bool wholeA = leftA >= 32 || leftA <= 0, wholeB = leftB >= 32 || leftB <= 0;
        const float4* lds4 = reinterpret_cast<const float4*>(lds2);
        float rmnA, rmxA, rmnB, rmxB;
        __syncthreads();
        scan_put<HB>(lds2, hi, cp, sa0, sa1);
        wave_sync_lds();
        scan_row_minmax<HB>(lds4, row, wholeA, leftA < 32 ? leftA : 32, rmnA, rmxA);
        wave_sync_lds();
        scan_put<HB>(lds2, hi, cp, sb0, sb1);
        wave_sync_lds();
        scan_row_minmax<HB>(lds4, row, wholeB, leftB < 32 ? leftB : 32, rmnB, rmxB);
        float tminA = wave_min_f(leftA > 0 ? rmnA : FLT_MAX), tminB = wave_min_f(leftB > 0 ? rmnB : FLT_MAX);
        float* slots = reinterpret_cast<float*>(lds2 + scan_row_of<HB>(t & ~63) * 16);
        wave_sync_lds();
        if ((t & 63) == 0) { slots[0] = tminA; slots[1] = tminB; }
        __syncthreads();
#pragma unroll
        for (int w = 0; w < (1 << (HB - 2)); ++w) {
            const float* v = reinterpret_cast<const float*>(lds2 + scan_row_of<HB>(w * 64) * 16);
            tminA = fminf(tminA, v[0]);
            tminB = fminf(tminB, v[1]);
        }
        const bool dense = scan.margin < 0.0f;
        const float thA = dense ? -FLT_MAX : fminf(fminf(tminA, tminB), scan.hist_min) + scan.margin, thB = thA;
        bool edgeA, edgeB;
        if (one_edge) {
            edgeA = leftA > 0 && ((unsigned)(ed.relcA - rowrun) <= 31u || (unsigned)(ed.reldA - rowrun) <= 31u);
            edgeB = leftB > 0 && ((unsigned)(ed.relcB - rowrun) <= 31u || (unsigned)(ed.reldB - rowrun) <= 31u);
        } else {
            edgeA = leftA > 0 && run_has_chunk_edge(outA + rowrun, scan.seg_c, scan.seg_d, scan.inv_c);
            edgeB = leftB > 0 && run_has_chunk_edge(outB + rowrun, scan.seg_c, scan.seg_d, scan.inv_c);
        }
        const bool pa = (leftA > 0 && rmxA >= thA) || edgeA, pb = (leftB > 0 && rmxB >= thB) || edgeB;
        const unsigned long long ba = __ballot(pa), bb = __ballot(pb);
        const unsigned sh = (unsigned)hi & 3u;
        wantA[0] = ((unsigned)ba >> sh) & 0x11111111u; wantA[1] = ((unsigned)(ba >> 32) >> sh) & 0x11111111u;
        wantB[0] = ((unsigned)bb >> sh) & 0x11111111u; wantB[1] = ((unsigned)(bb >> 32) >> sh) & 0x11111111u;
        const long long tileA = blkA * (out_stride >> kColsLog) + ((unsigned)n2_0 >> kColsLog), tileB = tileA + (out_stride >> kColsLog);
        if (t == 0 && scan.tile_theta != nullptr) {
            scan.tile_theta[tileA] = thA;
            if (blkB < job.nblocks) scan.tile_theta[tileB] = thB;
        }
        if ((t & 63) == 0 && scan.wbits != nullptr) {
            scan.wbits[(tileA << (HB - 2)) + (t >> 6)] = ba;
            if (blkB < job.nblocks) scan.wbits[(tileB << (HB - 2)) + (t >> 6)] = bb;
        }
        if (leftA > 0) scan.stats32[(outA + rowrun) >> 5] = make_float2(rmnA, rmxA);
        if (leftB > 0) scan.stats32[(outB + rowrun) >> 5] = make_float2(rmnB, rmxB);
    }
    if (wantA[0] | wantA[1]) {
#pragma unroll
        for (int a = 0; a < 16; ++a) {
            if (!((wantA[a >> 3] >> ((a & 7) * 4)) & 1u)) continue;
            const long long n = (long long)(a * (1 << HB) + hi) * out_stride + col;
            if (dst8 && n + 1 < limA) {
                float2* ptr = reinterpret_cast<float2*>(job.dst + outA + n);
                float2 v = make_float2(sa0[a], sa1[a]);
                if (ACC) { const float2 o = *ptr; v.x += o.x; v.y += o.y; }
                *ptr = v;
            } else {
                if (n < limA) job.dst[outA + n] = sa0[a] + (ACC ? job.dst[outA + n] : 0.0f);
                if (n + 1 < limA) job.dst[outA + n + 1] = sa1[a] + (ACC ? job.dst[outA + n + 1] : 0.0f);
            }
            if (ACC && (a & 3) == 3) __builtin_amdgcn_sched_barrier(0);
        }
    }
    if (wantB[0] | wantB[1]) {
#pragma unroll
        for (int a = 0; a < 16; ++a) {
            if (!((wantB[a >> 3] >> ((a & 7) * 4)) & 1u)) continue;
            const long long n = (long long)(a * (1 << HB) + hi) * out_stride + col;
            if (dst8 && n + 1 < limB) {
                float2* ptr = reinterpret_cast<float2*>(job.dst + outB + n);
                float2 v = make_float2(sb0[a], sb1[a]);
                if (ACC) { const float2 o = *ptr; v.x += o.x; v.y += o.y; }
                *ptr = v;
            } else {
                if (n < limB) job.dst[outB + n] = sb0[a] + (ACC ? job.dst[outB + n] : 0.0f);
                if (n + 1 < limB) job.dst[outB + n + 1] = sb1[a] + (ACC ? job.dst[outB + n + 1] : 0.0f);
            }
            if (ACC && (a & 3) == 3) __builtin_amdgcn_sched_barrier(0);
        }
    }
}


template <bool ACC = false>
__device__ __forceinline__ void k3_tile(const Job& job, const PlanDev& pl, const ScanCfg& scan, float2* lds2,
                                        int n2_0, int out_stride, int t, long long blkA, long long blkB,
                                        float out_scale, float2 (&x0)[16], float2 (&x1)[16], const ScanCfg* geo = nullptr) {
    const int hi = t >> 4, cp = t & 15;
    const long long N = 1ll << pl.logN;
    const long long col = n2_0 + 2 * cp;
    const K3Edges ed = k3_edges(job, geo ? *geo : scan, blkA, blkB);
    const unsigned maskN = (unsigned)(N - 1);
    const float2 w256 = pl.tw1[hi], w256q = pl.tw1[4 * hi];
    {
        const unsigned n2 = (unsigned)col;
        float2 base0 = tw_big(pl, (n2 * (unsigned)hi) & maskN);
        float2 base1 = tw_big(pl, ((n2 + 1) * (unsigned)hi) & maskN);
        base0.x *= out_scale; base0.y *= out_scale;
        base1.x *= out_scale; base1.y *= out_scale;
        float2 step0, step1, step0q, step1q;
        tw_big_pair(pl, (n2 * 16u) & maskN, step0, step0q);
        tw_big_pair(pl, ((n2 + 1) * 16u) & maskN, step1, step1q);
        twiddle_chain<16, true, false>(x0, base0, step0, step0q);
        dif<16, true>(x0);
#pragma unroll
        for (int b = 0; b < 16; ++b) lds2[(hi * 16 + b) * 16 + cp] = x0[brev<16>(b)];
        twiddle_chain<16, true, false>(x1, base1, step1, step1q);
    }
    dif<16, true>(x1);
    __syncthreads();
#pragma unroll
    for (int ap = 0; ap < 16; ++ap) x0[ap] = lds2[(ap * 16 + hi) * 16 + cp];
    __syncthreads();
#pragma unroll
    for (int b = 0; b < 16; ++b) lds2[(hi * 16 + b) * 16 + cp] = x1[brev<16>(b)];
    twiddle_nat<16, true>(x0, w256, w256q);
    dif<16, true>(x0);
    __syncthreads();
#pragma unroll
    for (int ap = 0; ap < 16; ++ap) x1[ap] = lds2[(ap * 16 + hi) * 16 + cp];
    twiddle_nat<16, true>(x1, w256, w256q);
    dif<16, true>(x1);
    k3_finish<4, ACC, true>(job, scan, ed, lds2, n2_0, out_stride, t, blkA, blkB, out_scale, x0, x1);
}

__device__ __forceinline__ void k3_tile_h16(const Job& job, const PlanDev& pl, const ScanCfg& scan, float2* lds2,
                                            int n2_0, int out_stride, int t, long long blkA, long long blkB,
                                            float out_scale, h2 (&hx0)[16], h2 (&hx1)[16]) {
    const int hi = t >> 4, cp = t & 15;
    const long long N = 1ll << pl.logN;
    const long long col = n2_0 + 2 * cp;
    const K3Edges ed = k3_edges(job, scan, blkA, blkB);
    const unsigned maskN = (unsigned)(N - 1);
    const float2 w256 = pl.tw1[hi];
    {
        const unsigned n2 = (unsigned)col;
        const float2 base0 = tw_big(pl, (n2 * (unsigned)hi) & maskN);
        const float2 base1 = tw_big(pl, ((n2 + 1) * (unsigned)hi) & maskN);
        const float2 step0 = tw_big(pl, (n2 * 16u) & maskN);
        const float2 step1 = tw_big(pl, ((n2 + 1) * 16u) & maskN);
        twiddle_chain<16, true, false>(hx0, base0, step0);
        twiddle_chain<16, true, false>(hx1, base1, step1);
    }
    dif<16, true>(hx0);
    dif<16, true>(hx1);
    uint2* ldsu = reinterpret_cast<uint2*>(lds2);
#pragma unroll
    for (int b = 0; b < 16; ++b) ldsu[(hi * 16 + b) * 16 + cp] = make_uint2(h2_bits(hx0[brev<16>(b)]), h2_bits(hx1[brev<16>(b)]));
    __syncthreads();
    float2 x0[16], x1[16];
#pragma unroll
    for (int ap = 0; ap < 16; ++ap) {
        const uint2 v = ldsu[(ap * 16 + hi) * 16 + cp];
        x0[ap] = to_f2(bits_h2(v.x));
        x1[ap] = to_f2(bits_h2(v.y));
    }
    twiddle_nat<16, true>(x0, w256);
    twiddle_nat<16, true>(x1, w256);
    dif<16, true>(x0);
    dif<16, true>(x1);
    k3_finish<4>(job, scan, ed, lds2, n2_0, out_stride, t, blkA, blkB, out_scale, x0, x1);
}

constexpr int kK3Waves = 3;
constexpr int kK3LoadAux = 2, kK3hLoadAux = 2;
template <int HALF, bool ACC>
__device__ __forceinline__ void k3_cols_inv_r16_tile(unsigned lin, float4* lds4, const Job& job, const float2* __restrict__ work,
                                                     const PlanDev& pl, float out_scale, const ScanCfg& scan, const ScanCfg* geo = nullptr) {
    const int t = threadIdx.x;
    const int hi = t >> 4, cp = t & 15;
    const unsigned xcd = lin & 7u, seq = lin >> 3;
    const unsigned slot = seq >> 5, half = (seq >> 4) & 1u, tl = seq & 15u;
    const int n2_0 = (int)(((half * 8u + xcd) * 16u + tl) << kColsLog);
    const int pair = job.first_pair + (int)slot;
    if (scan.only_pairs != nullptr && scan.only_pairs[pair] == 0) return;
    const long long blkA = 2ll * pair, blkB = blkA + 1;
    if constexpr (HALF == 2) {
        const uint2* __restrict__ in2 = reinterpret_cast<const uint2*>(reinterpret_cast<const unsigned*>(work) + ((size_t)slot << pl.logN) + n2_0) + cp;
        h2 hx0[16], hx1[16];
#pragma unroll
        for (int bp = 0; bp < 16; ++bp) {
            const uint2 v = in2[(size_t)(hi + 16 * bp) * (kN2 / 2)];
            hx0[bp] = bits_h2(v.x);
            hx1[bp] = bits_h2(v.y);
        }
        k3_tile_h16(job, pl, scan, reinterpret_cast<float2*>(lds4), n2_0, kN2, t, blkA, blkB, out_scale, hx0, hx1);
        return;
    }
    float2 x0[16], x1[16];
    if (HALF) {
        const uint2* __restrict__ in2 = reinterpret_cast<const uint2*>(reinterpret_cast<const unsigned*>(work) + ((size_t)slot << pl.logN) + n2_0) + cp;
#pragma unroll
        for (int bp = 0; bp < 16; ++bp) {
            const uint2 v = in2[(size_t)(hi + 16 * bp) * (kN2 / 2)];
            x0[bp] = unpack_h2(v.x);
            x1[bp] = unpack_h2(v.y);
        }
    } else {
        const __amdgpu_buffer_rsrc_t rin = make_rsrc(work + ((size_t)slot << pl.logN) + n2_0, (unsigned)((((size_t)1 << pl.logN) - n2_0) * 8));
        const unsigned voff = (unsigned)hi * (kN2 * 8u) + (unsigned)cp * 16u;
#pragma unroll
        for (int bp = 0; bp < 16; ++bp) {
            const float4 v = buf_load4<kK3LoadAux>(rin, voff, (unsigned)bp * (16u * kN2 * 8u));
            x0[bp] = make_float2(v.x, v.y);
            x1[bp] = make_float2(v.z, v.w);
        }
    }
    k3_tile<ACC>(job, pl, scan, reinterpret_cast<float2*>(lds4), n2_0, kN2, t, blkA, blkB, out_scale, x0, x1, geo);
}
template <int HALF, bool ACC = false, int REDO = 0>
__global__ void __launch_bounds__(256, REDO ? 4 : kK3Waves)
k3_cols_inv_r16(Job job, const float2* __restrict__ work, PlanDev pl, float out_scale, ScanCfg scan) {
    extern __shared__ float4 lds4[];
    if constexpr (REDO != 0) {
        for (unsigned lin = blockIdx.x; lin < (unsigned)scan.redo_tiles; lin += gridDim.x) {
            k3_cols_inv_r16_tile<HALF, ACC>(lin, lds4, job, work, pl, out_scale, scan);
            __syncthreads();
        }
    } else {
        k3_cols_inv_r16_tile<HALF, ACC>(blockIdx.x, lds4, job, work, pl, out_scale, scan);
    }
}

__global__ void __launch_bounds__(256, kK3Waves)
k3_cols_inv_r16_group(Job job, PlanDev pl, ScanCfg scan, K3Group grp) {
    extern __shared__ float4 lds4[];
    const unsigned z = blockIdx.y;
    job.dst = grp.dst[z]; job.out_count = grp.out_count[z];
    ScanCfg mine;
    mine.stats32 = grp.stats32[z]; mine.wbits = grp.wbits[z]; mine.tile_theta = grp.tile_theta[z]; mine.hist_min = grp.hist_min[z];
    mine.margin = scan.margin; mine.seg_c = grp.seg_c; mine.seg_d = grp.seg_d[z]; mine.inv_c = grp.inv_c;
    mine.only_pairs = nullptr; mine.redo_tiles = 0; mine.edges_n = 0;
    k3_cols_inv_r16_tile<0, false>(blockIdx.x, lds4, job, grp.work[z], pl, grp.out_scale[z], mine, &scan);
}

template <int HALF>
__global__ void __launch_bounds__(256, kK3Waves)
tail_cols_inv_r16(TailBatch tb, int hop, const float2* __restrict__ work, PlanDev pl, float out_scale) {
    extern __shared__ float4 lds4[];
    const unsigned z = blockIdx.y;
    Job job;
    job.src = nullptr; job.src_len = 0; job.lead = 0; job.dst = tb.dst[z]; job.out_count = tb.out_count[z];
    job.hop = hop; job.nblocks = (int)((tb.out_count[z] + hop - 1) / hop); job.first_pair = 0; job.src_kind = 0;
    ScanCfg mine;
    mine.stats32 = tb.stats32[z]; mine.wbits = nullptr; mine.tile_theta = nullptr; mine.margin = -1.0f; mine.hist_min = FLT_MAX;
    mine.seg_c = 0; mine.seg_d = 0; mine.inv_c = 0.0; mine.only_pairs = nullptr; mine.redo_tiles = 0; mine.edges_n = 0;
    const float2* mywork = HALF ? reinterpret_cast<const float2*>(reinterpret_cast<const unsigned*>(work) + ((size_t)z << pl.logN))
                                : work + ((size_t)z << pl.logN);
    k3_cols_inv_r16_tile<HALF, false>(blockIdx.x, lds4, job, mywork, pl, out_scale, mine);
}

__global__ void __launch_bounds__(256)
tail_commit_kernel(const float* __restrict__ tsc, float* __restrict__ sc, long long n, const float2* __restrict__ tst, float2* __restrict__ st32,
                   unsigned long long* __restrict__ wbits, long long words, float* __restrict__ theta, int tiles) {
    const long long tid = (long long)blockIdx.x * blockDim.x + threadIdx.x, nth = (long long)gridDim.x * blockDim.x;
    const long long n4 = n >> 2;
    const float4* __restrict__ t4 = reinterpret_cast<const float4*>(tsc);
    float4* __restrict__ s4 = reinterpret_cast<float4*>(sc);
    for (long long i = tid; i < n4; i += nth) s4[i] = t4[i];
    for (long long i = (n4 << 2) + tid; i < n; i += nth) sc[i] = tsc[i];
    const long long n32 = (n + 31) >> 5;
    for (long long i = tid; i < n32; i += nth) st32[i] = tst[i];
    if (wbits != nullptr)
        for (long long i = tid; i < words; i += nth) wbits[i] = ~0ull;
    if (theta != nullptr)
        for (long long i = tid; i < tiles; i += nth) theta[i] = -FLT_MAX;
}

__global__ void __launch_bounds__(256)
tail_preset_group_kernel(K3Group grp, long long blk, int log_n1, int log_n2) {
    const unsigned z = blockIdx.y;
    const long long tiles = 1ll << (log_n2 - kColsLog), words = tiles << (log_n1 - 6);
    const long long tid = (long long)blockIdx.x * blockDim.x + threadIdx.x, nth = (long long)gridDim.x * blockDim.x;
    unsigned long long* __restrict__ wb = grp.wbits[z] + blk * words;
    float* __restrict__ th = grp.tile_theta[z] + blk * tiles;
    for (long long i = tid; i < words; i += nth) wb[i] = ~0ull;
    for (long long i = tid; i < tiles; i += nth) th[i] = -FLT_MAX;
}

constexpr int kC512Slab = 560;
__device__ __forceinline__ int c512_idx(int ap, int b, int cp) { return ap * kC512Slab + b * 17 + cp; }
constexpr int kC512Lds = (15 * kC512Slab + 31 * 17 + 16) * 8;
static_assert(kC512Lds >= 512 * 16 * 8, "K3's score scan needs 512 rows x 32 scores");
constexpr int kC512Slab3 = 32 * 16 + 16;
__device__ __forceinline__ int c512_idx3(int ap, int b, int cp) { return ap * kC512Slab3 + b * 16 + cp; }
static_assert((15 * kC512Slab3 + 31 * 16 + 16) * 8 <= kC512Lds, "K3's exchange fits the kernel's LDS");

template <int KIND, int HALF, int LN2 = kR16LogN2>
__global__ void __launch_bounds__(512, 4)
k1_cols_fwd_c512(Job job, float2* __restrict__ work, PlanDev pl) {
    constexpr int kN2 = 1 << LN2;
    extern __shared__ float4 lds4[];
    float2* lds2 = reinterpret_cast<float2*>(lds4);
    const int t = threadIdx.x;
    const int hi = t >> 4, cp = t & 15;
    const int ap = hi & 15, half = hi >> 4;
    const int k10 = ap + 16 * half;
    const int n2_0 = blockIdx.x << kColsLog;
    const int pair = job.first_pair + blockIdx.y;
    const long long blkA = 2ll * pair, blkB = blkA + 1;
    const bool validB = blkB < job.nblocks;
    const long long N = 1ll << pl.logN;
    const long long baseA = blkA * job.hop - job.lead;
    const long long baseB = blkB * job.hop - job.lead;
    const bool fast = ((reinterpret_cast<uintptr_t>(job.src) & 7) == 0) && ((baseA & 1) == 0) && ((baseB & 1) == 0) &&
                      baseA >= 0 && baseA + N <= job.src_len && validB && baseB + N <= job.src_len;
    const long long col = (long long)n2_0 + 2 * cp;
    const unsigned maskN = (unsigned)(N - 1);
    const float2 w512 = pl.tw1[hi];
    const float2 w512q = pl.tw1[4 * hi];
    const float2 base0 = tw_big(pl, ((unsigned)col * (unsigned)k10) & maskN);
    const float2 base1 = tw_big(pl, (((unsigned)col + 1u) * (unsigned)k10) & maskN);
    float2 step0, step1, step0q, step1q;
    if constexpr (HALF == 2) {
        step0 = tw_big(pl, ((unsigned)col * 32u) & maskN);
        step1 = tw_big(pl, (((unsigned)col + 1u) * 32u) & maskN);
    }
    float2 x0[16], x1[16];
    if (fast && KIND == 1) {
        const __amdgpu_buffer_rsrc_t rsrc = make_rsrc(static_cast<const char*>(job.src) + 4 * baseA, (unsigned)(4 * (N + job.hop)));
        const unsigned voff = 4u * ((unsigned)hi * kN2 + (unsigned)col), offB = 4u * (unsigned)job.hop;
#pragma unroll
        for (int a = 0; a < 16; ++a) {
            const float2 va = decode_sample2<KIND>(buf_load_u2<kK1LoadNt ? 2 : 0>(rsrc, voff, (unsigned)a * (4u * 32u * kN2)));
            const float2 vb = decode_sample2<KIND>(buf_load_u2<kK1LoadNt ? 2 : 0>(rsrc, voff, (unsigned)a * (4u * 32u * kN2) + offB));
            x0[a] = make_float2(va.x, vb.x);
            x1[a] = make_float2(va.y, vb.y);
        }
    } else if (fast) {
#pragma unroll
        for (int a = 0; a < 16; ++a) {
            const long long off = (long long)(a * 32 + hi) * kN2 + col;
// ... 607 lines not shown
    for (int idx = tid; idx < total; idx += nthr) {
        const int p = idx >> BL, c = idx & ((1 << BL) - 1);
        const unsigned k1 = __brev((unsigned)p) >> (32 - pl.logN1);
        const float2 w = tw_big(pl, ((unsigned)(n2_0 + c) * k1) & maskN);
        s[idx] = cmulc(in[(size_t)p * N2 + c], w);
    }
    __syncthreads();
    lds_fft_inv<BL>(s, pl.logN1, pl.tw1, tid, nthr);
    const long long outA = blkA * job.hop, outB = blkB * job.hop;
    for (int idx = tid; idx < total; idx += nthr) {
        const int r = idx >> BL, c = idx & ((1 << BL) - 1);
        const long long n = (long long)r * N2 + n2_0 + c;
        if (n >= job.hop) continue;
        const float2 v = s[idx];
        if (outA + n < job.out_count) job.dst[outA + n] = v.x * out_scale + (acc ? job.dst[outA + n] : 0.0f);
        if (validB && outB + n < job.out_count) job.dst[outB + n] = v.y * out_scale + (acc ? job.dst[outB + n] : 0.0f);
    }
}

template <int KIND>
__global__ void __launch_bounds__(256)
correlate_direct(Job job, const float* __restrict__ needle, int s, float out_scale) {
    __shared__ float nd[kDirectMaxNeedle];
    if ((int)threadIdx.x < s) nd[threadIdx.x] = needle[threadIdx.x];
    __syncthreads();
    for (long long j = (long long)blockIdx.x * 256 + threadIdx.x; j < job.out_count; j += (long long)gridDim.x * 256) {
        float acc = 0.0f;
        for (int n = 0; n < s; ++n) acc = fmaf(load_padded<KIND>(job.src, j + n - job.lead, job.src_len), nd[n], acc);
        job.dst[j] = acc * out_scale;
    }
}

hipError_t launch_direct(hipStream_t st, const Job& job, const float* needle, int s, float out_scale) {
    if (s < 1 || s > kDirectMaxNeedle || job.out_count <= 0) return hipErrorInvalidValue;
    long long blocks = (job.out_count + 255) / 256;
    if (blocks > 4096) blocks = 4096;
    if (job.src_kind == 1) hipLaunchKernelGGL(correlate_direct<1>, dim3((unsigned)blocks), dim3(256), 0, st, job, needle, s, out_scale);
    else hipLaunchKernelGGL(correlate_direct<0>, dim3((unsigned)blocks), dim3(256), 0, st, job, needle, s, out_scale);
    return hipGetLastError();
}

template <typename Fn>
struct Variant { Fn fn; int threads; int lds; };

template <typename Fn, typename... Args>
static hipError_t launch_row_lds(const Variant<Fn>& v, dim3 grid, size_t lds, hipStream_t st, const Args&... args) {
    if (v.fn == nullptr) return hipErrorInvalidValue;
    hipLaunchKernelGGL(v.fn, grid, dim3(v.threads), lds, st, args...);
    return hipGetLastError();
}
template <typename Fn, typename... Args>
static hipError_t launch_row(const Variant<Fn>& v, dim3 grid, hipStream_t st, const Args&... args) {
    return launch_row_lds(v, grid, (size_t)v.lds, st, args...);
}

bool plan_is_r16(const PlanDev& pl) { return pl.logN1 == kR16LogN1 && pl.logN2 == kR16LogN2; }
bool plan_is_c512(const PlanDev& pl) { return pl.logN1 == 9 && pl.logN2 == kR16LogN2; }
bool plan_is_c1024(const PlanDev& pl) { return pl.logN1 == 10 && pl.logN2 == kR16LogN2; }
bool plan_is_c512w(const PlanDev& pl) { return pl.logN1 == 9 && pl.logN2 == 14; }
bool plan_has_scan(const PlanDev& pl) { return plan_is_r16(pl) || plan_is_c512(pl) || plan_is_c1024(pl); }
bool plan_k2_is_r16(const PlanDev& pl) { return pl.logN2 == kR16LogN2 && pl.logN1 >= 3; }

enum ColPlan { kColR16, kColC512, kColC1024, kColC512w, kColGen, kColPlans };
static ColPlan col_plan(const PlanDev& pl) {
    return plan_is_r16(pl) ? kColR16 : plan_is_c512(pl) ? kColC512 : plan_is_c1024(pl) ? kColC1024 : plan_is_c512w(pl) ? kColC512w : kColGen;
}
static int half_level(int half) { return half == 2 ? 2 : half ? 1 : 0; }

static constexpr int kMaxLds = 160 * 1024;
static constexpr int kR16Lds = 64 * 1024;
static constexpr int kR16LdsK1 = 256 * 17 * 8;
static constexpr int kR16LdsK3 = 256 * 16 * 8;

using K1Fn = void (*)(Job, float2*, PlanDev);
static constexpr Variant<K1Fn> kK1[kColPlans][2][3] = {
     {{{k1_cols_fwd_r16<0, 0>, 256, kR16LdsK1}, {k1_cols_fwd_r16<0, 1>, 256, kR16LdsK1}, {k1_cols_fwd_r16<0, 2>, 256, kR16LdsK1}},
                 {{k1_cols_fwd_r16<1, 0>, 256, kR16LdsK1}, {k1_cols_fwd_r16<1, 1>, 256, kR16LdsK1}, {k1_cols_fwd_r16<1, 2>, 256, kR16LdsK1}}},
     {{{k1_cols_fwd_c512<0, 0>, 512, kC512Lds}, {k1_cols_fwd_c512<0, 1>, 512, kC512Lds}, {k1_cols_fwd_c512<0, 2>, 512, kC512Lds}},
                 {{k1_cols_fwd_c512<1, 0>, 512, kC512Lds}, {k1_cols_fwd_c512<1, 1>, 512, kC512Lds}, {k1_cols_fwd_c512<1, 2>, 512, kC512Lds}}},
     {{{k1_cols_fwd_c1024<0>, 1024, kC1024Lds}}, {{k1_cols_fwd_c1024<1>, 1024, kC1024Lds}}},
     {{{k1_cols_fwd_c512<0, 0, 14>, 512, kC512Lds}}},
     {{{k1_cols_fwd_gen<kColsLog, 0>, kFftThreads, kMaxLds}}, {{k1_cols_fwd_gen<kColsLog, 1>, kFftThreads, kMaxLds}}},
};
using TailK1Fn = void (*)(TailBatch, int, float2*, PlanDev);
static constexpr Variant<TailK1Fn> kTailK1[2][3] = {
    {{tail_cols_fwd_r16<0, 0>, 256, kR16LdsK1}, {tail_cols_fwd_r16<0, 1>, 256, kR16LdsK1}, {tail_cols_fwd_r16<0, 2>, 256, kR16LdsK1}},
    {{tail_cols_fwd_r16<1, 0>, 256, kR16LdsK1}, {tail_cols_fwd_r16<1, 1>, 256, kR16LdsK1}, {tail_cols_fwd_r16<1, 2>, 256, kR16LdsK1}},
};

using K2Fn = void (*)(float2*, const float2*, float2*, PlanDev, unsigned, float);
static constexpr Variant<K2Fn> kK2[2][2] = {
    {{k2_rows_r16_planes<false>, 256, kK2hLds}, {tail_rows_r16_planes<false>, 256, kK2hLds}},
    {{k2_rows_r16_planes<true>, 256, kK2hLds}, {tail_rows_r16_planes<true>, 256, kK2hLds}},
};
static constexpr Variant<K2Fn> kK2Spectrum = {k2_rows_r16_spectrum, 256, kR16Lds};
using K2hFn = void (*)(unsigned*, const unsigned*, unsigned*, PlanDev, unsigned, float);
static constexpr Variant<K2hFn> kK2h[2] = {{k2_rows_h16, 256, kK2hLds}, {tail_rows_h16, 256, kK2hLds}};
static constexpr Variant<K2hFn> kK2Mfma = {k2_rows_m16, 256, kK2mLds};
using K2GroupFn = void (*)(const float2*, K2Group, PlanDev, unsigned);
static constexpr Variant<K2GroupFn> kK2Group = {k2_rows_r16_group_planes, 256, kK2hLds};
using K2GenFn = void (*)(float2*, const float2*, float2*, PlanDev);
static constexpr Variant<K2GenFn> kK2Gen[2] = {{k2_rows_gen<false>, kFftThreads, kMaxLds}, {k2_rows_gen<true>, kFftThreads, kMaxLds}};

enum K3Form { kK3Plain, kK3Acc, kK3Redo, kK3Forms };
using K3Fn = void (*)(Job, const float2*, PlanDev, float, ScanCfg);
static constexpr Variant<K3Fn> kK3[kColGen][3][kK3Forms] = {
     {{{k3_cols_inv_r16<0>, 256, kR16LdsK3}, {}, {k3_cols_inv_r16<0, false, 1>, 256, kR16LdsK3}},
                 {{k3_cols_inv_r16<1>, 256, kR16LdsK3}, {}, {k3_cols_inv_r16<1, false, 1>, 256, kR16LdsK3}},
                 {{k3_cols_inv_r16<2>, 256, kR16LdsK3}, {}, {k3_cols_inv_r16<2, false, 1>, 256, kR16LdsK3}}},
     {{{k3_cols_inv_c512<0>, 512, kC512Lds}, {k3_cols_inv_c512<0, true>, 512, kC512Lds}, {k3_cols_inv_c512<0, false, 1>, 512, kC512Lds}},
                 {{k3_cols_inv_c512<1>, 512, kC512Lds}, {}, {k3_cols_inv_c512<1, false, 1>, 512, kC512Lds}},
                 {{k3_cols_inv_c512<2>, 512, kC512Lds}, {}, {k3_cols_inv_c512<2, false, 1>, 512, kC512Lds}}},
     {{{k3_cols_inv_c1024<false>, 1024, kC1024Lds}, {k3_cols_inv_c1024<true>, 1024, kC1024Lds}, {k3_cols_inv_c1024<false, 1>, 1024, kC1024Lds}}},
     {{{k3_cols_inv_c512w, 512, kC512Lds}}},
};
using K3GenFn = void (*)(Job, const float2*, PlanDev, float, int);
static constexpr Variant<K3GenFn> kK3Gen = {k3_cols_inv_gen<kColsLog>, kFftThreads, kMaxLds};
using K3GroupFn = void (*)(Job, PlanDev, ScanCfg, K3Group);
static constexpr Variant<K3GroupFn> kK3Group[kColGen] = {{k3_cols_inv_r16_group, 256, kR16LdsK3}, {k3_cols_inv_c512_group, 512, kC512Lds}};
using TailK3Fn = void (*)(TailBatch, int, const float2*, PlanDev, float);
static constexpr Variant<TailK3Fn> kTailK3[3] = {
    {tail_cols_inv_r16<0>, 256, kR16LdsK3}, {tail_cols_inv_r16<1>, 256, kR16LdsK3}, {tail_cols_inv_r16<2>, 256, kR16LdsK3}};

template <typename Fn>
static hipError_t allow_lds(const Variant<Fn>& v) {
    return v.fn == nullptr ? hipSuccess : hipFuncSetAttribute((const void*)v.fn, hipFuncAttributeMaxDynamicSharedMemorySize, v.lds);
}
template <typename T, size_t N>
static hipError_t allow_lds(const T (&table)[N]) {
    for (const T& t : table) {
        const hipError_t e = allow_lds(t);
        if (e != hipSuccess) return e;
    }
    return hipSuccess;
}
hipError_t fft_kernels_init() {
    hipError_t e = allow_lds(kK1);
    if (e == hipSuccess) e = allow_lds(kTailK1);
    if (e == hipSuccess) e = allow_lds(kK2);
    if (e == hipSuccess) e = allow_lds(kK2Spectrum);
    if (e == hipSuccess) e = allow_lds(kK2h);
    if (e == hipSuccess) e = allow_lds(kK2Mfma);
    if (e == hipSuccess) e = allow_lds(kK2Group);
    if (e == hipSuccess) e = allow_lds(kK2Gen);
    if (e == hipSuccess) e = allow_lds(kK3);
    if (e == hipSuccess) e = allow_lds(kK3Gen);
    if (e == hipSuccess) e = allow_lds(kK3Group);
    if (e == hipSuccess) e = allow_lds(kTailK3);
    return e;
}

hipError_t launch_k1(hipStream_t st, const Job& job, int npairs, float2* work, const PlanDev& pl, int half) {
    const dim3 grid((1u << pl.logN2) >> kColsLog, npairs);
    const ColPlan p = col_plan(pl);
    const int kind = job.src_kind == 1 ? 1 : 0;
    if (p == kColGen) return launch_row_lds(kK1[p][kind][0], grid, (sizeof(float2) << pl.logN1) << kColsLog, st, job, work, pl);
    return launch_row(kK1[p][kind][half_level(half)], grid, st, job, work, pl);
}

static int k2_mfma_initial() { const char* e = getenv("AM_K2_MFMA"); return e && atoi(e) ? 1 : 0; }
static std::atomic<int> g_k2_mfma{k2_mfma_initial()};
void set_k2_mfma(int on) { g_k2_mfma.store(on ? 1 : 0, std::memory_order_relaxed); }
bool k2_mfma_enabled() { return g_k2_mfma.load(std::memory_order_relaxed) != 0; }
int k2_mfma_table_dwords() { return kMfTotal; }

hipError_t launch_k2(hipStream_t st, int npairs, float2* work, const float2* hc, const PlanDev& pl, float2* dst,
                     int half, float hscale, float pre, bool tail) {
    if (!plan_k2_is_r16(pl))
        return launch_row_lds(kK2Gen[0], dim3(1u << pl.logN1, npairs), sizeof(float2) << pl.logN2, st, work, hc, dst, pl);
    const unsigned rows = (unsigned)npairs << pl.logN1;
    if (half == 2) {
        unsigned* const w = reinterpret_cast<unsigned*>(work);
        const unsigned* const h = reinterpret_cast<const unsigned*>(hc);
        unsigned* const d = reinterpret_cast<unsigned*>(dst);
        if (!tail && k2_mfma_enabled() && pl.mf != nullptr) {
            const unsigned grid = std::min<unsigned>(rows, 256u * 4u) & ~7u;
            return launch_row(kK2Mfma, dim3(grid ? grid : 8u), st, w, h, d, pl, (unsigned)npairs, pre);
        }
        return launch_row(kK2h[tail], dim3(rows), st, w, h, d, pl, (unsigned)npairs, pre);
    }
    return launch_row(kK2[half ? 1 : 0][tail], dim3(rows), st, work, hc, dst, pl, (unsigned)npairs, half ? hscale : 1.0f);
}

bool plan_k2_has_group(const PlanDev& pl) { return plan_k2_is_r16(pl); }

hipError_t launch_k2_group(hipStream_t st, int npairs, const float2* work, const K2Group& grp, const PlanDev& pl) {
    if (!plan_k2_has_group(pl) || grp.n < 1 || grp.n > kMaxNeedleGroup) return hipErrorInvalidValue;
    return launch_row(kK2Group, dim3((unsigned)npairs << pl.logN1), st, work, grp, pl, (unsigned)npairs);
}

hipError_t launch_k2_spectrum(hipStream_t st, float2* work, float2* hc_out, const PlanDev& pl) {
    if (plan_k2_is_r16(pl)) return launch_row(kK2Spectrum, dim3(1u << pl.logN1), st, work, (const float2*)nullptr, hc_out, pl, 1u, 1.0f);
    return launch_row_lds(kK2Gen[1], dim3(1u << pl.logN1, 1), sizeof(float2) << pl.logN2, st, work, (const float2*)nullptr, hc_out, pl);
}

static void fill_edges(const Job& job, int npairs, ScanCfg& scan) {
    scan.edges_n = 0;
    const long long c = scan.seg_c, d = scan.seg_d, hop = job.hop;
    if (scan.stats32 == nullptr || npairs > ScanCfg::kMaxEdgeSlots || c < hop + 32) return;
    auto rel = [](long long edge, long long start) { const long long r = edge - start; return r < 0x7fffffffll ? (int)r : 0x7fffffff; };
    for (int s = 0; s < npairs; ++s) {
        const long long outA = 2ll * (job.first_pair + s) * hop, outB = outA + hop;
        const long long m = outA % c;
        const long long ecA = m == 0 ? outA : outA + (c - m);
        long long edA = d;
        if (outA > d) {
            const long long m2 = (outA - d) % c;
            edA = m2 == 0 ? outA : outA + (c - m2);
        }
        const long long ecB = ecA >= outB ? ecA : ecA + c, edB = edA >= outB ? edA : edA + c;
        scan.edge_rel[s][0] = rel(ecA, outA); scan.edge_rel[s][1] = rel(edA, outA);
        scan.edge_rel[s][2] = rel(ecB, outB); scan.edge_rel[s][3] = rel(edB, outB);
    }
    scan.edges_n = npairs;
}

bool plan_k3_has_group(const PlanDev& pl) { return plan_is_c512(pl) || plan_is_r16(pl); }

hipError_t launch_tail_batch_k1(hipStream_t st, const TailBatch& tb, int hop, int src_kind, float2* work, const PlanDev& pl, int half) {
    if (!plan_is_r16(pl) || tb.n < 1 || tb.n > kMaxTailBatch) return hipErrorInvalidValue;
    const dim3 grid((1u << pl.logN2) >> kColsLog, (unsigned)tb.n);
    return launch_row(kTailK1[src_kind == 1 ? 1 : 0][half_level(half)], grid, st, tb, hop, work, pl);
}
hipError_t launch_tail_batch_k3(hipStream_t st, const TailBatch& tb, int hop, const float2* work, const PlanDev& pl, float out_scale, int half) {
    if (!plan_is_r16(pl) || tb.n < 1 || tb.n > kMaxTailBatch) return hipErrorInvalidValue;
    return launch_row(kTailK3[half_level(half)], dim3(kN2 >> kColsLog, (unsigned)tb.n), st, tb, hop, work, pl, out_scale);
}
hipError_t launch_tail_preset_group(hipStream_t st, const K3Group& grp, long long blk, int log_n1, int log_n2) {
    if (grp.n < 1 || grp.n > kMaxNeedleGroup) return hipErrorInvalidValue;
    for (int z = 0; z < grp.n; ++z) if (!grp.wbits[z] || !grp.tile_theta[z]) return hipErrorInvalidValue;
    hipLaunchKernelGGL(tail_preset_group_kernel, dim3(8, (unsigned)grp.n), dim3(256), 0, st, grp, blk, log_n1, log_n2);
    return hipGetLastError();
}
hipError_t launch_tail_commit(hipStream_t st, const float* tail_scores, float* scores, long long n, const float2* tail_stats32, float2* stats32,
                              unsigned long long* wbits, long long words, float* theta, int tiles) {
    const unsigned grid = (unsigned)std::min<long long>(512, std::max<long long>(1, (n / 4 + 255) / 256));
    hipLaunchKernelGGL(tail_commit_kernel, dim3(grid), dim3(256), 0, st, tail_scores, scores, n, tail_stats32, stats32, wbits, words, theta, tiles);
    return hipGetLastError();
}

hipError_t launch_k3_group(hipStream_t st, const Job& job, int npairs, const K3Group& grp, const PlanDev& pl, const ScanCfg& scan_in) {
    if (!plan_k3_has_group(pl) || grp.n < 1 || grp.n > kMaxNeedleGroup || scan_in.stats32 == nullptr) return hipErrorInvalidValue;
    for (int z = 0; z < grp.n; ++z) if (grp.out_count[z] > job.out_count) return hipErrorInvalidValue;
    ScanCfg scan = scan_in;
    scan.only_pairs = nullptr;
    fill_edges(job, npairs, scan);
    const dim3 grid((unsigned)npairs * (kN2 >> kColsLog), (unsigned)grp.n);
    return launch_row(kK3Group[col_plan(pl)], grid, st, job, pl, scan, grp);
}

hipError_t launch_k3(hipStream_t st, const Job& job, int npairs, const float2* work,
                     const PlanDev& pl, float out_scale, const ScanCfg& scan_in, int half, bool accumulate) {
    ScanCfg scan = scan_in;
    fill_edges(job, npairs, scan);
    const ColPlan p = col_plan(pl);
    if (p == kColGen) {
        if (accumulate && half) return hipErrorInvalidValue;
        const dim3 grid((1u << pl.logN2) >> kColsLog, npairs);
        return launch_row_lds(kK3Gen, grid, (sizeof(float2) << pl.logN1) << kColsLog, st, job, work, pl, out_scale, accumulate ? 1 : 0);
    }
    K3Form form = accumulate ? kK3Acc : kK3Plain;
    unsigned grid = (unsigned)npairs * ((1u << pl.logN2) >> kColsLog);
    if (scan.only_pairs != nullptr && !accumulate) {
        if (!plan_has_scan(pl)) return hipErrorInvalidValue;
        form = kK3Redo;
        scan.redo_tiles = (int)grid;
        const unsigned per_cu = p == kColC1024 ? 1u : p == kColC512 ? 2u : 4u;
        grid = std::min<unsigned>(grid, 256u * per_cu);
    }
    return launch_row(kK3[p][half_level(half)][form], dim3(grid), st, job, work, pl, out_scale, scan);
}

}
```

audio-matcher_amd/csrc/am_internal.h:

```cpp
#pragma once
#include <algorithm>
#include <atomic>
#include <cfloat>
#include <cmath>
#include <cstdio>
#include <cstring>
#include <map>
#include <mutex>
#include <string>
#include <vector>

#include "am_kernels.h"
#include "am_spans.h"

namespace am {

extern thread_local std::string t_err;
int fail(int code, const std::string& msg);
int hip_fail(hipError_t e, const char* what);
#define AM_HIP(call)                                         \
    do {                                                     \
        hipError_t e_ = (call);                              \
        if (e_ != hipSuccess) return hip_fail(e_, #call);    \
    } while (0)

struct Hooks {
    am_progress_fn fn = nullptr;
    void* user = nullptr;
    am_chunk_progress_fn chunk_fn = nullptr;
    void* chunk_user = nullptr;
};
Hooks snapshot_hooks();

struct Opts {
    long long log_n, pairs_per_group, half, batch_overlap, needle_group, dense, device_redo, debug_no_realloc, debug_redo_arm_at;
    long long peak_filter_order, distance_rule, tail_window, surrounding_from, k3_group, pick_group, tail_block, host_pick_wait;
    long long profile_mask, profile_every, pick_priority;
    long long score_norm, score_norm_floor_db;
    long long trace_form;
    PeakPolicy peak_policy() const { return PeakPolicy{(int)peak_filter_order, (int)(distance_rule & 1), (int)((distance_rule >> 1) & 1)}; }
};
static const float kHalfGain = 1024.0f;
static const double kMinEfficiency = 0.75;
static const int kLogNMin = 10, kLogNMax = 23;
static const long long kWideFromSamples = 140000;
static const long long kWidestFromSamples = 1500000;
static const long long kSegmentFrom = 1ll << 22;
static const long long kSegmentLen = 1ll << 22;

extern thread_local int t_no_realloc;
struct QueueingScope {
    bool on;
    explicit QueueingScope(bool enable) : on(enable) { if (on) ++t_no_realloc; }
    ~QueueingScope() { end(); }
    void end() { if (on) { --t_no_realloc; on = false; } }
    QueueingScope(const QueueingScope&) = delete;
    QueueingScope& operator=(const QueueingScope&) = delete;
};
int realloc_refused(const char* what, size_t bytes, size_t cap);

struct DevBuf {
    void* p = nullptr;
    size_t cap = 0;
    int ensure(size_t bytes) {
        if (bytes <= cap) return AM_OK;
        if (t_no_realloc > 0) return realloc_refused("a device", bytes, cap);
        release();
        size_t want = bytes + bytes / 8;
        hipError_t e = hipMalloc(&p, want);
        if (e != hipSuccess) {
            e = hipMalloc(&p, bytes);
            want = bytes;
            if (e != hipSuccess) { p = nullptr; return hip_fail(e, "hipMalloc(scratch)"); }
        }
        cap = want;
        return AM_OK;
    }
    void release() {
        if (p) (void)hipFree(p);
        p = nullptr; cap = 0;
    }
};
struct HostBuf {
    void* p = nullptr;
    size_t cap = 0;
    unsigned flags = hipHostMallocDefault;
    int ensure(size_t bytes) {
        if (bytes <= cap) return AM_OK;
        if (t_no_realloc > 0) return realloc_refused("a pinned host", bytes, cap);
        release();
        hipError_t e = hipHostMalloc(&p, bytes, flags);
        if (e != hipSuccess) { p = nullptr; return hip_fail(e, "hipHostMalloc"); }
        cap = bytes;
        return AM_OK;
    }
    void release() {
        if (p) (void)hipHostFree(p);
        p = nullptr; cap = 0;
    }
};

struct Plan {
    PlanDev dev{};
    float2* tables = nullptr;
    unsigned* mf = nullptr;
};

struct ScoreSide { DevBuf scores, stats, stats32, wflags, peaks, work; };

struct ProfRec { int name; hipEvent_t e0, e1; };
enum { KN_K1 = 0, KN_K2, KN_K3, KN_STATS, KN_PEAKS, KN_OTHER, KN_TRACE, KN_DISCOVER, KN_COUNT };

struct Ctx {
    int device = -1;
    hipStream_t stream = nullptr;
    hipStream_t stream2 = nullptr;
    hipStream_t stream_tail = nullptr;
    hipEvent_t ev_fork = nullptr, ev_join = nullptr;
    DevBuf work_tail, tail_scores, tail_stats;
// ... 33 lines not shown
    uint64_t prof_seq[KN_COUNT] = {0};
};

#ifndef AM_EVENT_NO_SYSTEM_FENCE
#define AM_EVENT_NO_SYSTEM_FENCE 1
#endif
constexpr unsigned kSyncEvent = hipEventDisableTiming | (AM_EVENT_NO_SYSTEM_FENCE ? hipEventDisableSystemFence : 0u);

int get_ctx(int device, Ctx** out);
struct ProfScope {
    Ctx* c; int name; hipStream_t st; hipEvent_t e0 = nullptr, e1 = nullptr;
    bool on;
    ProfScope(Ctx* c_, int name_, hipStream_t st_ = nullptr);
    ~ProfScope() {
        if (on) { (void)hipEventRecord(e1, st); c->pending.push_back({name, e0, e1}); }
    }
};
hipError_t copy_on_stream(Ctx* c, void* dst, const void* src, size_t bytes, hipMemcpyKind kind);
int get_plan(Ctx* c, int logN, const Plan** out, int force_logN1 = 0);

}

struct am_needle {
    am::Ctx* ctx = nullptr;
    float* d_needle = nullptr;
    size_t n = 0;
    float inv_autocorr = 0.f;
    double energy = 0.0;
    std::map<int, float2*> spectra;
    std::map<int, unsigned*> spectra16;
    std::map<int, unsigned*> spectra16m;
    static constexpr int kRecent = 8;
    float recent_min[2][kRecent];
    int recent_n[2] = {0, 0}, recent_pos[2] = {0, 0};
    void remember_min(int sm, float v) {
        recent_min[sm][recent_pos[sm]] = v;
        recent_pos[sm] = (recent_pos[sm] + 1) % kRecent;
        if (recent_n[sm] < kRecent) ++recent_n[sm];
    }
    int conservative_left[2] = {0, 0};
    int redo_armed_left[2] = {0, 0};
    float hist_min(int sm) const {
        float m = FLT_MAX;
        for (int i = 0; i < recent_n[sm]; ++i) m = std::min(m, recent_min[sm][i]);
        return m;
    }
    long long opt_log_n = -1, opt_half = -1, opt_score_norm = -1;
    std::vector<am_needle*> segments;
    std::vector<long long> seg_off;
    bool owns_data = true;
};

namespace am {

struct ScanBuffers { DevBuf* work; DevBuf* stats32; DevBuf* wflags; };
inline ScanBuffers scan_buffers(ScoreSide& sd) { return ScanBuffers{&sd.work, &sd.stats32, &sd.wflags}; }
struct ScanRequest {
    float margin;
    float hist_min;
    long long seg_c, seg_d;
    ScanBuffers out;
    hipEvent_t before_k3;
    long long range_a, range_b;
    long long side_nblocks;
    bool skip_launch;
    bool tail_by_caller;
    bool no_scan;
};
struct ScanResult {
    bool fused;
    SparseScores sparse;
    bool redo_ok;
    Job redo_job; PlanDev redo_pl; float redo_scale; int redo_half; int redo_npairs; const float2* redo_work; ScanCfg redo_cfg;
};
inline SparseScores plain_scores() { return SparseScores{nullptr, nullptr, nullptr, 1, 5, 5, 1.0}; }
struct Geometry {
    int logN;
    long long N, hop, nblocks, npairs;
};
struct TailPlan {
    bool on;
    long long T;
    Geometry g;
};
struct HalfScale {
    int level;
    float pre, hscale;
    float k3(float factor) const { return level ? factor / (hscale * pre) : factor; }
};
struct Footprint {
    size_t work = 0, stats32 = 0, side = 0, work_tail = 0;
    long long npairs = 0;
    void take(const Footprint& f) {
        work = std::max(work, f.work); stats32 = std::max(stats32, f.stats32); side = std::max(side, f.side);
        work_tail = std::max(work_tail, f.work_tail);
        npairs = std::max(npairs, f.npairs);
    }
};
enum class PassKind { Direct, Partitioned, Transform };
struct PassPlan {
    PassKind kind = PassKind::Direct;
    Geometry g{};
    const Plan* pl = nullptr;
    const float2* hc = nullptr;
    HalfScale hs{};
    bool fused = false;
    TailPlan tail{};
    const Plan* tail_pl = nullptr;
    const float2* tail_hc = nullptr;
    HalfScale tail_hs{};
    long long nblocks = 0, npairs = 0;
    long long ppg = 0;
    long long main_count = 0;
    std::vector<PassPlan> parts;
    Footprint need;
    Segment pair_reads(long long q, long long len) const {
        const long long last_block = (2 * q + 1 < nblocks) ? 2 * q + 1 : 2 * q;
        return Segment{2 * q * g.hop, std::min(len, last_block * g.hop + g.N)};
    }
    Segment tail_reads(long long len) const { return Segment{tail.T, std::min(len, tail.T + (tail.g.nblocks - 1) * tail.g.hop + tail.g.N)}; }
};
struct PartSpec {
    size_t max_windows;
    uint64_t first_sample;
    size_t chunk_base, chunk_total;
    std::vector<am_peak>* raw;
};
struct StreamPre {
    float* scores;
    DevBuf* stats32; DevBuf* side;
    long long pairs_done;
    long long layout_nblocks;
};

inline const void* advance_src(const void* src, size_t elements) {
    return static_cast<const char*>(src) + 4 * elements;
}

Opts snapshot_opts(const am_needle* h);
extern thread_local const Opts* t_opts_pin;
struct OptsPin {
    const Opts* prev;
    explicit OptsPin(const Opts* o) : prev(t_opts_pin) { t_opts_pin = o; }
    ~OptsPin() { t_opts_pin = prev; }
    OptsPin(const OptsPin&) = delete;
    OptsPin& operator=(const OptsPin&) = delete;
};
int check_needle(const am_needle* h);
int create_needle_common(Ctx* c, float* d_needle, size_t n, am_needle** out);
HalfScale half_scale(const am_needle* h, const Opts& o, const PlanDev& pl);
int needle_k2_spectrum(am_needle* h, const Opts& o, const Plan* pl, const float2** hc, HalfScale* hs);

struct NormSpec { bool on; double energy, thr; };
NormSpec norm_spec(const am_needle* h, const Opts& o);
int norm_check(const NormSpec& ns, int scale);
float norm_factor(const NormSpec& ns);
int norm_reserve(Ctx* c, long long max_src_len);
int normalise_scores(Ctx* c, hipStream_t st, const NormSpec& ns, const void* src, long long src_len, int src_kind, long long lead,
                     long long s, float* scores, long long a, long long b);
#define AM_NORM_UNSUPPORTED "score_norm: not supported by this entry point"

int hit_check_format(int sample_format);
double hit_floor(const am_needle* h);
double hit_floor_ratio(const am_needle* h);
struct HitWhere { long long pair; size_t hay, needle, hit; };
std::string hit_pair_name(const HitWhere& w);
// ... 181 lines not shown
```

audio-matcher_amd/csrc/am_kernels.h:

```cpp
#pragma once

#include <hip/hip_runtime.h>
#include <stdint.h>

#include "../../include/audiomatch.h"

namespace am {

struct Job {
    const void* src;
    long long src_len;
    long long lead;
    float* dst;
    long long out_count;
    int hop;
    int nblocks;
    int first_pair;
    int src_kind;
};

struct PlanDev {
    int logN, logN1, logN2, logLo;
    const float2* tw1;
    const float2* tw2;
    const float2* twlo;
    const float2* twhi;
    const float4* twlo4;
    const float4* twhi4;
    const float4* k2j;
    const float4* k2c;
    const unsigned* mf;
};

constexpr int kColsLog = 5;
constexpr int kCols = 1 << kColsLog;
constexpr int kTile = 1024;
constexpr int kFftThreads = 256;

struct Segment {
    long long a, b;
};

hipError_t launch_k1(hipStream_t st, const Job& job, int npairs, float2* work, const PlanDev& pl, int half = 0);
hipError_t launch_k2(hipStream_t st, int npairs, float2* work, const float2* hc, const PlanDev& pl, float2* dst = nullptr,
                     int half = 0, float hscale = 1.0f, float pre = 1.0f, bool tail = false);
hipError_t launch_spectrum_to_half(hipStream_t st, const float2* hc, long long n, float scale, unsigned* out);
void set_k2_mfma(int on);
bool k2_mfma_enabled();
int k2_mfma_table_dwords();
hipError_t launch_spectrum_to_half_mfma(hipStream_t st, const float2* hc, long long n, float scale, unsigned* out);
hipError_t launch_k2_spectrum(hipStream_t st, float2* work, float2* hc_out, const PlanDev& pl);
constexpr int kMaxNeedleGroup = 8;
struct K2Group {
    const float2* hc[kMaxNeedleGroup];
    float2* dst[kMaxNeedleGroup];
    int n;
};
bool plan_k2_has_group(const PlanDev& pl);
hipError_t launch_k2_group(hipStream_t st, int npairs, const float2* work, const K2Group& grp, const PlanDev& pl);
struct ScanCfg {
    float2* stats32;
    unsigned long long* wbits;
    float* tile_theta;
    float margin;
    float hist_min;
    long long seg_c, seg_d;
    double inv_c;
    const int* only_pairs;
    int redo_tiles;
    static constexpr int kMaxEdgeSlots = 64;
    int edges_n;
    int edge_rel[kMaxEdgeSlots][4];
};
hipError_t launch_k3(hipStream_t st, const Job& job, int npairs, const float2* work,
                     const PlanDev& pl, float out_scale, const ScanCfg& scan, int half = 0, bool accumulate = false);
struct K3Group {
    int n;
    const float2* work[kMaxNeedleGroup];
    float* dst[kMaxNeedleGroup];
    float2* stats32[kMaxNeedleGroup];
    unsigned long long* wbits[kMaxNeedleGroup];
    float* tile_theta[kMaxNeedleGroup];
    float hist_min[kMaxNeedleGroup];
    float out_scale[kMaxNeedleGroup];
    long long out_count[kMaxNeedleGroup];
    long long seg_d[kMaxNeedleGroup];
    long long seg_c;
    double inv_c;
};
bool plan_k3_has_group(const PlanDev& pl);
constexpr int kMaxTailBatch = 8;
struct TailBatch {
    int n;
    const void* src[kMaxTailBatch];
    long long src_len[kMaxTailBatch];
    float* dst[kMaxTailBatch];
    long long out_count[kMaxTailBatch];
    float2* stats32[kMaxTailBatch];
};
hipError_t launch_tail_batch_k1(hipStream_t st, const TailBatch& tb, int hop, int src_kind, float2* work, const PlanDev& pl, int half);
hipError_t launch_tail_batch_k3(hipStream_t st, const TailBatch& tb, int hop, const float2* work, const PlanDev& pl, float out_scale, int half);
hipError_t launch_tail_preset_group(hipStream_t st, const K3Group& grp, long long blk, int log_n1, int log_n2);
hipError_t launch_tail_commit(hipStream_t st, const float* tail_scores, float* scores, long long n, const float2* tail_stats32, float2* stats32,
                              unsigned long long* wbits, long long words, float* theta, int tiles);
hipError_t launch_k3_group(hipStream_t st, const Job& job, int npairs, const K3Group& grp, const PlanDev& pl, const ScanCfg& scan);
constexpr int kDirectMaxNeedle = 64;
hipError_t launch_direct(hipStream_t st, const Job& job, const float* needle, int s, float out_scale);
bool plan_is_r16(const PlanDev& pl);
bool plan_is_c512(const PlanDev& pl);
bool plan_is_c512w(const PlanDev& pl);
bool plan_is_c1024(const PlanDev& pl);
bool plan_has_scan(const PlanDev& pl);
bool plan_k2_is_r16(const PlanDev& pl);
hipError_t fft_kernels_init();

hipError_t launch_nonfinite_ranges(hipStream_t st, const float* x, const Segment* ranges, int nranges, int* flags);
hipError_t launch_tile_stats(hipStream_t st, const float* g, long long n, float2* stats, int* bad = nullptr);
struct PickGroup {
    int n;
    const float* g[kMaxNeedleGroup];
    float2* stats[kMaxNeedleGroup];
    const float2* stats32[kMaxNeedleGroup];
    const unsigned long long* wbits[kMaxNeedleGroup];
    const float* theta[kMaxNeedleGroup];
    int hdr_off[kMaxNeedleGroup];
};
hipError_t launch_stats_reduce(hipStream_t st, const float2* stats32, long long n, float2* stats, int* bad = nullptr,
                               const PickGroup* grp = nullptr);
constexpr int kInlinePeaks = 4;
struct SegHeader {
    int n;
    int overflow;
    float seg_min;
    int arena_off;
    am_peak first[kInlinePeaks];
};
struct PeakArena {
    am_peak* base;
    unsigned* cursor;
    unsigned cap;
};
struct SparseScores {
    const unsigned long long* wbits;
    const float2* stats32;
    const float* tile_theta;
    int hop, log_n2, log_n1;
    double inv_hop;
    int* redo_pairs;
    unsigned char* fail_flags;
};
struct WideState {
    int* state;
    unsigned* count;
    float* seg_min;
    unsigned long long* best;
    am_peak* list;
    unsigned cap;
    int* ntiles;
    int* tiles;
};
constexpr int kWideTileList = 1024;
struct PeakPolicy {
    int order;
    int inclusive;
    int from_start;
};
hipError_t launch_peaks_wide_one(hipStream_t st, const float* g, long long g_len, const float2* stats, const Segment* d_seg,
                                 float min_prom, long long min_dist, const SparseScores& sp, const WideState& wide, const PeakPolicy& pol);
hipError_t launch_peaks_big_finish(hipStream_t st, const am_peak* list, unsigned n, long long a, long long min_dist,
                                   unsigned long long* keys, unsigned* idx, long long* table, am_peak* out, unsigned* out_n,
                                   const PeakPolicy& pol);
hipError_t launch_peaks(hipStream_t st, const float* g, long long g_len, const float2* stats,
                        const Segment* d_segs, int nsegs, float min_prom, long long min_dist,
                        am_peak* d_out, SegHeader* d_hdr, const SparseScores& sp, const PeakArena& arena,
                        const WideState& wide, bool only_failed, const PeakPolicy& pol, const PickGroup* grp = nullptr);
int sumsq_parts(long long n);
hipError_t launch_sumsq(hipStream_t st, const float* x, long long n, double* d_parts);
hipError_t launch_synth(hipStream_t st, float* out, uint32_t seed, uint32_t stream, uint64_t first,
                        long long n, float amp);
hipError_t launch_axpy(hipStream_t st, float* dst, const float* src, long long n, float gain);
hipError_t launch_synth_pcm16(hipStream_t st, int16_t* out, uint32_t seed, uint32_t stream, uint64_t first, long long frames, float amp);
hipError_t launch_add_pcm16(hipStream_t st, int16_t* dst, const int16_t* src, long long frames);
hipError_t launch_pcm_downmix(hipStream_t st, const int16_t* in, long long frames, float* out);

__device__ __forceinline__ float norm_downmix(short2 lr) {
    return __fmul_rn((float)((int)lr.x + (int)lr.y), 0.5f * (1.0f / 65535.0f));
}
typedef __attribute__((address_space(1))) const float gfloat;
// ... 199 lines not shown
```

audio-matcher_amd/python/audiomatch_amd/__init__.py:

```python
from __future__ import annotations

import ctypes as C
import struct
import enum
import os
from dataclasses import dataclass

import numpy as np

_PKG = os.path.dirname(os.path.abspath(__file__))
_ROOT = os.path.abspath(os.path.join(_PKG, "..", ".."))
LIB_PATH = os.path.join(_ROOT, "libaudiomatch_amd.so")

AM_OK, AM_ERR_INVALID_ARG, AM_ERR_CAPACITY, AM_ERR_HIP, AM_ERR_NO_DEVICE, \
    AM_ERR_PEAK_OVERFLOW, AM_ERR_OOM = range(7)
AM_MAX_PEAKS_PER_CHUNK = 1024


class Fmt(enum.IntEnum):
    F32_MONO = 0
    S16_STEREO = 1


class Mode(enum.IntEnum):
# ... 263 lines not shown
    "am_find_peaks": (C.c_int, [C.c_int, C.c_void_p, C.c_size_t, C.c_float, C.c_uint64,
                                C.POINTER(AmPeak), C.c_size_t, C.POINTER(C.c_size_t)]),
    "am_pcm_s16_stereo_to_mono": (C.c_int, [C.c_int, C.c_void_p, C.c_size_t, C.c_void_p]),
    "am_pcm_s16_stereo_to_mono_device": (C.c_int, [C.c_int, C.c_void_p, C.c_size_t, C.c_void_p]),
    "am_device_malloc": (C.c_int, [C.c_int, C.c_size_t, C.POINTER(C.c_void_p)]),
    "am_device_free": (C.c_int, [C.c_int, C.c_void_p]),
    "am_host_alloc": (C.c_int, [C.c_size_t, C.POINTER(C.c_void_p)]),
    "am_host_free": (C.c_int, [C.c_void_p]),
    "am_host_register": (C.c_int, [C.c_void_p, C.c_size_t]),
    "am_host_unregister": (C.c_int, [C.c_void_p]),
    "am_memcpy_h2d": (C.c_int, [C.c_int, C.c_void_p, C.c_void_p, C.c_size_t]),
    "am_memcpy_d2h": (C.c_int, [C.c_int, C.c_void_p, C.c_void_p, C.c_size_t]),
    "am_device_synchronize": (C.c_int, [C.c_int]),
    "am_synth_uniform_device": (C.c_int, [C.c_int, C.c_void_p, C.c_uint32, C.c_uint32, C.c_uint64,
                                          C.c_size_t, C.c_float]),
    "am_axpy_device": (C.c_int, [C.c_int, C.c_void_p, C.c_void_p, C.c_size_t, C.c_float]),
    "am_synth_pcm16_stereo_device": (C.c_int, [C.c_int, C.c_void_p, C.c_uint32, C.c_uint32, C.c_uint64,
                                               C.c_size_t, C.c_float]),
    "am_add_pcm16_device": (C.c_int, [C.c_int, C.c_void_p, C.c_void_p, C.c_size_t]),
    "am_set_progress_callback": (C.c_int, [C.c_void_p, C.c_void_p]),
    "am_set_chunk_progress_callback": (C.c_int, [C.c_void_p, C.c_void_p]),
    "am_needle_set_option": (C.c_int, [C.c_void_p, C.c_char_p, C.c_longlong]),
    "am_needle_get_option": (C.c_int, [C.c_void_p, C.c_char_p, C.POINTER(C.c_longlong)]),
    "am_shard_plan": (C.c_int, [C.c_size_t, C.c_size_t, C.c_size_t, C.POINTER(C.c_size_t),
                                C.POINTER(C.c_size_t), C.POINTER(C.c_size_t)]),
    "am_pool_create": (C.c_int, [C.c_void_p, C.c_size_t, C.POINTER(C.c_int), C.c_size_t, C.POINTER(C.c_void_p)]),
    "am_pool_destroy": (None, [C.c_void_p]),
    "am_pool_size": (C.c_int, [C.c_void_p, C.POINTER(C.c_size_t)]),
    "am_pool_slot": (C.c_int, [C.c_void_p, C.c_size_t, C.POINTER(C.c_int), C.POINTER(C.c_void_p)]),
    "am_pool_match_batch": (C.c_int, [C.c_void_p, C.POINTER(C.c_void_p), C.POINTER(C.c_size_t), C.c_size_t,
                                      C.POINTER(AmMatchParams), C.POINTER(AmPeak), C.c_size_t,
                                      C.POINTER(C.c_size_t)]),
    "am_pool_match_batch_device": (C.c_int, [C.c_void_p, C.POINTER(C.c_void_p), C.POINTER(C.c_size_t), C.c_size_t,
                                             C.POINTER(AmMatchParams), C.POINTER(AmPeak), C.c_size_t,
                                             C.POINTER(C.c_size_t)]),
    "am_match_multi_batch_device": (C.c_int, [C.POINTER(C.c_void_p), C.c_size_t, C.POINTER(C.c_void_p), C.POINTER(C.c_size_t),
                                              C.c_size_t, C.c_int, C.POINTER(AmMatchParams), C.POINTER(AmPeak), C.c_size_t,
                                              C.POINTER(C.c_size_t)]),
    "am_pool_match_batch_pcm16": (C.c_int, [C.c_void_p, C.POINTER(C.c_void_p), C.POINTER(C.c_size_t), C.c_size_t,
                                            C.POINTER(AmMatchParams), C.POINTER(AmPeak), C.c_size_t,
                                            C.POINTER(C.c_size_t)]),
    "am_pool_match_batch_pcm16_device": (C.c_int, [C.c_void_p, C.POINTER(C.c_void_p), C.POINTER(C.c_size_t), C.c_size_t,
                                                   C.POINTER(AmMatchParams), C.POINTER(AmPeak), C.c_size_t,
                                                   C.POINTER(C.c_size_t)]),
    "am_match_multi_varlen_batch_device": (C.c_int, [C.POINTER(C.c_void_p), C.c_size_t, C.POINTER(C.c_uint64), C.POINTER(C.c_void_p),
                                                     C.POINTER(C.c_size_t), C.c_size_t, C.c_int, C.POINTER(AmMatchParams),
                                                     C.POINTER(AmPeak), C.c_size_t, C.POINTER(C.c_size_t)]),
    "am_match_multi_varlen": (C.c_int, [C.POINTER(C.c_void_p), C.c_size_t, C.POINTER(C.c_uint64), C.c_void_p, C.c_size_t,
                                        C.c_int, C.POINTER(AmMatchParams), C.POINTER(AmPeak), C.c_size_t,
                                        C.POINTER(C.c_size_t)]),
    "am_pool_create_multi": (C.c_int, [C.POINTER(C.c_void_p), C.c_size_t, C.c_size_t, C.POINTER(C.c_int), C.c_size_t,
                                       C.POINTER(C.c_void_p)]),
    "am_pool_needle_count": (C.c_int, [C.c_void_p, C.POINTER(C.c_size_t)]),
    "am_pool_match_multi_batch": (C.c_int, [C.c_void_p, C.POINTER(C.c_void_p), C.POINTER(C.c_size_t), C.c_size_t, C.c_int,
                                            C.POINTER(AmMatchParams), C.POINTER(AmPeak), C.c_size_t,
                                            C.POINTER(C.c_size_t)]),
    "am_pool_match_multi_batch_device": (C.c_int, [C.c_void_p, C.POINTER(C.c_void_p), C.POINTER(C.c_size_t), C.c_size_t, C.c_int,
                                                   C.POINTER(AmMatchParams), C.POINTER(AmPeak), C.c_size_t,
                                                   C.POINTER(C.c_size_t)]),
    "am_long_plan": (C.c_int, [C.c_size_t, C.c_size_t, C.POINTER(AmMatchParams), C.c_size_t, C.c_size_t, C.POINTER(C.c_size_t),
                               C.POINTER(C.c_size_t), C.POINTER(C.c_size_t), C.POINTER(C.c_size_t)]),
    "am_match_part_device": (C.c_int, [C.c_void_p, C.c_void_p, C.c_size_t, C.c_int, C.POINTER(AmMatchParams), C.c_size_t,
                                       C.c_uint64, C.POINTER(AmPeak), C.c_size_t, C.POINTER(C.c_size_t)]),
    "am_merge_peaks": (C.c_int, [C.POINTER(AmMatchParams), C.POINTER(AmPeak), C.c_size_t, C.POINTER(AmPeak), C.c_size_t,
                                 C.POINTER(C.c_size_t)]),
    "am_pool_match_long": (C.c_int, [C.c_void_p, C.c_void_p, C.c_size_t, C.c_int, C.POINTER(AmMatchParams), C.POINTER(AmPeak),
                                     C.c_size_t, C.POINTER(C.c_size_t)]),
    "am_pool_match_long_device": (C.c_int, [C.c_void_p, C.POINTER(C.c_void_p), C.c_size_t, C.c_int, C.POINTER(AmMatchParams),
                                            C.POINTER(AmPeak), C.c_size_t, C.POINTER(C.c_size_t)]),
    "am_merge_ready": (C.c_int, [C.POINTER(AmMatchParams), C.POINTER(AmPeak), C.c_size_t, C.c_uint64, C.c_int,
                                 C.POINTER(C.c_size_t)]),
    "am_monitor_begin": (C.c_int, [C.POINTER(C.c_void_p), C.c_size_t, C.POINTER(AmMatchParams), C.c_int, C.c_size_t,
                                   C.POINTER(C.c_void_p)]),
    "am_monitor_push": (C.c_int, [C.c_void_p, C.c_void_p, C.c_size_t]),
    "am_monitor_poll": (C.c_int, [C.c_void_p, C.POINTER(AmPeak), C.POINTER(C.c_uint32), C.c_size_t, C.POINTER(C.c_size_t)]),
    "am_monitor_end": (C.c_int, [C.c_void_p, C.POINTER(AmPeak), C.POINTER(C.c_uint32), C.c_size_t, C.POINTER(C.c_size_t)]),
    "am_monitor_info_get": (C.c_int, [C.c_void_p, C.POINTER(AmMonitorInfo)]),
    "am_monitor_destroy": (None, [C.c_void_p]),
    "am_match_stream_begin": (C.c_int, [C.c_void_p, C.c_int, C.c_size_t, C.POINTER(AmMatchParams), C.POINTER(C.c_void_p)]),
    "am_match_stream_push": (C.c_int, [C.c_void_p, C.c_void_p, C.c_size_t]),
    "am_match_stream_finish": (C.c_int, [C.c_void_p, C.POINTER(AmPeak), C.c_size_t, C.POINTER(C.c_size_t)]),
    "am_match_stream_destroy": (None, [C.c_void_p]),
    "am_debug_column_bench": (C.c_int, [C.c_int, C.c_int, C.c_int, C.c_int, C.c_int, C.POINTER(C.c_double), C.POINTER(C.c_double)]),
    "am_profile_enable": (C.c_int, [C.c_int, C.c_int]),
    "am_profile_reset": (C.c_int, [C.c_int]),
    "am_profile_query": (C.c_int, [C.c_int, C.c_char_p, C.POINTER(C.c_double), C.POINTER(C.c_uint64)]),
    "am_hit_scores_device": (C.c_int, [C.c_void_p, C.c_void_p, C.c_size_t, C.c_int, C.POINTER(AmPeak), C.c_size_t,
                                       C.POINTER(AmHitScore)]),
    "am_hit_scores": (C.c_int, [C.c_void_p, C.c_void_p, C.c_size_t, C.c_int, C.POINTER(AmPeak), C.c_size_t,
                                C.POINTER(AmHitScore)]),
    "am_hit_scores_batch_device": (C.c_int, [C.POINTER(C.c_void_p), C.c_size_t, C.POINTER(C.c_void_p), C.POINTER(C.c_size_t),
                                             C.c_size_t, C.c_int, C.POINTER(AmPeak), C.c_size_t, C.POINTER(C.c_size_t),
                                             C.POINTER(AmHitScore)]),
    "am_hit_segments_device": (C.c_int, [C.c_void_p, C.c_void_p, C.c_size_t, C.c_int, C.POINTER(AmPeak), C.c_size_t,
                                         C.POINTER(AmSegmentParams), C.POINTER(HitSegment)]),
    "am_hit_segments": (C.c_int, [C.c_void_p, C.c_void_p, C.c_size_t, C.c_int, C.POINTER(AmPeak), C.c_size_t,
                                  C.POINTER(AmSegmentParams), C.POINTER(HitSegment)]),
    "am_hit_segments_batch_device": (C.c_int, [C.POINTER(C.c_void_p), C.c_size_t, C.POINTER(C.c_void_p), C.POINTER(C.c_size_t),
                                               C.c_size_t, C.c_int, C.POINTER(AmPeak), C.c_size_t, C.POINTER(C.c_size_t),
                                               C.POINTER(AmSegmentParams), C.POINTER(HitSegment)]),
    "am_hit_segments_summary": (C.c_int, [C.POINTER(HitSegment), C.c_uint32, C.c_size_t, C.c_float,
                                          C.POINTER(AmSegmentSummary)]),
    "am_hit_bands_device": (C.c_int, [C.c_void_p, C.c_void_p, C.c_size_t, C.c_int, C.POINTER(AmPeak), C.c_size_t,
                                      C.POINTER(AmBandParams), C.POINTER(HitBand)]),
    "am_hit_bands": (C.c_int, [C.c_void_p, C.c_void_p, C.c_size_t, C.c_int, C.POINTER(AmPeak), C.c_size_t,
                               C.POINTER(AmBandParams), C.POINTER(HitBand)]),
    "am_hit_bands_batch_device": (C.c_int, [C.POINTER(C.c_void_p), C.c_size_t, C.POINTER(C.c_void_p), C.POINTER(C.c_size_t),
                                            C.c_size_t, C.c_int, C.POINTER(AmPeak), C.c_size_t, C.POINTER(C.c_size_t),
                                            C.POINTER(AmBandParams), C.POINTER(HitBand)]),
    "am_hit_bands_summary": (C.c_int, [C.POINTER(HitBand), C.c_uint32, C.c_float, C.POINTER(AmBandSummary)]),
    "am_band_edges_log": (C.c_int, [C.c_uint32, C.c_uint32, C.c_double, C.c_double, C.c_uint32, C.POINTER(AmBandParams)]),
    "am_hit_significance_device": (C.c_int, [C.c_void_p, C.c_void_p, C.c_size_t, C.c_int, C.POINTER(AmPeak), C.c_size_t,
                                             C.POINTER(AmSignificanceParams), C.POINTER(HitSignificance)]),
    "am_hit_significance": (C.c_int, [C.c_void_p, C.c_void_p, C.c_size_t, C.c_int, C.POINTER(AmPeak), C.c_size_t,
                                      C.POINTER(AmSignificanceParams), C.POINTER(HitSignificance)]),
    "am_hit_significance_batch_device": (C.c_int, [C.POINTER(C.c_void_p), C.c_size_t, C.POINTER(C.c_void_p), C.POINTER(C.c_size_t),
                                                   C.c_size_t, C.c_int, C.POINTER(AmPeak), C.c_size_t, C.POINTER(C.c_size_t),
                                                   C.POINTER(AmSignificanceParams), C.POINTER(HitSignificance)]),
    "am_resample_len": (C.c_int, [C.c_size_t, C.c_uint32, C.c_uint32, C.POINTER(C.c_size_t)]),
    "am_resample": (C.c_int, [C.c_int, C.c_void_p, C.c_size_t, C.c_int, C.c_uint32, C.c_uint32, C.c_void_p, C.c_size_t,
                              C.POINTER(C.c_size_t)]),
    "am_resample_device": (C.c_int, [C.c_int, C.c_void_p, C.c_size_t, C.c_int, C.c_uint32, C.c_uint32, C.c_void_p,
                                     C.c_size_t, C.POINTER(C.c_size_t)]),
    "am_needle_create_resampled": (C.c_int, [C.c_int, C.c_void_p, C.c_size_t, C.c_int, C.c_uint32, C.c_uint32,
                                             C.POINTER(C.c_void_p)]),
    "am_lag_products": (C.c_int, [C.c_int, C.c_void_p, C.c_size_t, C.c_int, C.c_uint32, C.POINTER(C.c_double)]),
    "am_lag_products_device": (C.c_int, [C.c_int, C.c_void_p, C.c_size_t, C.c_int, C.c_uint32, C.POINTER(C.c_double)]),
    "am_whiten_taps": (C.c_int, [C.POINTER(C.c_double), C.c_uint32, C.c_double, C.POINTER(C.c_float)]),
    "am_fir": (C.c_int, [C.c_int, C.c_void_p, C.c_size_t, C.c_int, C.POINTER(C.c_float), C.c_uint32, C.c_size_t, C.c_void_p,
                         C.c_size_t, C.POINTER(C.c_size_t)]),
    "am_fir_device": (C.c_int, [C.c_int, C.c_void_p, C.c_size_t, C.c_int, C.POINTER(C.c_float), C.c_uint32, C.c_size_t,
                                C.c_void_p, C.c_size_t, C.POINTER(C.c_size_t)]),
    "am_needle_create_filtered": (C.c_int, [C.c_int, C.c_void_p, C.c_size_t, C.c_int, C.POINTER(C.c_float), C.c_uint32,
                                            C.POINTER(C.c_void_p)]),
    "am_hit_window": (C.c_int, [C.c_void_p, C.c_size_t, C.c_int, C.c_uint64, C.c_float, C.c_uint64, C.c_uint64, C.c_void_p]),
    "am_warp_table": (C.c_int, [C.c_void_p]),
    "am_hit_warp_device": (C.c_int, [C.c_void_p, C.c_void_p, C.c_size_t, C.c_int, C.POINTER(AmPeak), C.c_size_t,
                                     C.POINTER(AmWarpParams), C.POINTER(HitWarp)]),
    "am_hit_warp": (C.c_int, [C.c_void_p, C.c_void_p, C.c_size_t, C.c_int, C.POINTER(AmPeak), C.c_size_t,
                              C.POINTER(AmWarpParams), C.POINTER(HitWarp)]),
    "am_hit_warp_batch_device": (C.c_int, [C.POINTER(C.c_void_p), C.c_size_t, C.POINTER(C.c_void_p), C.POINTER(C.c_size_t),
                                           C.c_size_t, C.c_int, C.POINTER(AmPeak), C.c_size_t, C.POINTER(C.c_size_t),
                                           C.POINTER(AmWarpParams), C.POINTER(HitWarp)]),
    "am_hit_window_warped": (C.c_int, [C.c_void_p, C.c_size_t, C.c_int, C.c_uint64, C.c_float, C.c_double, C.c_double,
                                       C.c_uint64, C.c_uint64, C.c_void_p]),
    "am_hit_channel_device": (C.c_int, [C.c_void_p, C.c_void_p, C.c_size_t, C.c_int, C.POINTER(AmPeak), C.c_size_t,
                                        C.POINTER(AmChannelParams), C.POINTER(HitChannel), C.c_void_p]),
    "am_hit_channel": (C.c_int, [C.c_void_p, C.c_void_p, C.c_size_t, C.c_int, C.POINTER(AmPeak), C.c_size_t,
                                 C.POINTER(AmChannelParams), C.POINTER(HitChannel), C.c_void_p]),
    "am_hit_channel_batch_device": (C.c_int, [C.POINTER(C.c_void_p), C.c_size_t, C.POINTER(C.c_void_p), C.POINTER(C.c_size_t),
                                              C.c_size_t, C.c_int, C.POINTER(AmPeak), C.c_size_t, C.POINTER(C.c_size_t),
                                              C.POINTER(AmChannelParams), C.POINTER(HitChannel), C.c_void_p]),
    "am_channel_solve": (C.c_int, [C.c_void_p, C.c_void_p, C.c_uint32, C.c_double, C.c_void_p, C.POINTER(C.c_int)]),
    "am_hit_residual": (C.c_int, [C.c_void_p, C.c_size_t, C.c_int, C.c_uint64, C.c_void_p, C.c_size_t, C.c_void_p, C.c_uint32,
                                  C.c_void_p, C.c_void_p]),
    "am_hit_stereo_device": (C.c_int, [C.c_void_p, C.c_void_p, C.c_size_t, C.c_int, C.POINTER(AmPeak), C.c_size_t,
                                       C.POINTER(AmStereoParams), C.POINTER(HitStereo)]),
    "am_hit_stereo": (C.c_int, [C.c_void_p, C.c_void_p, C.c_size_t, C.c_int, C.POINTER(AmPeak), C.c_size_t,
                                C.POINTER(AmStereoParams), C.POINTER(HitStereo)]),
    "am_hit_stereo_batch_device": (C.c_int, [C.POINTER(C.c_void_p), C.c_size_t, C.POINTER(C.c_void_p), C.POINTER(C.c_size_t),
                                             C.c_size_t, C.c_int, C.POINTER(AmPeak), C.c_size_t, C.POINTER(C.c_size_t),
                                             C.POINTER(AmStereoParams), C.POINTER(HitStereo)]),
    "am_hit_stereo_summary": (C.c_int, [C.POINTER(HitStereo), C.c_float, C.POINTER(AmStereoSummary)]),
    "am_pcm_s16_stereo_mix": (C.c_int, [C.c_int, C.c_void_p, C.c_size_t, C.c_float, C.c_float, C.c_void_p]),
    "am_pcm_s16_stereo_mix_device": (C.c_int, [C.c_int, C.c_void_p, C.c_size_t, C.c_float, C.c_float, C.c_void_p]),
    "am_needle_estimate_rows": (C.c_int, [C.c_int, C.c_void_p, C.c_size_t, C.POINTER(AmEstimateParams), C.c_void_p, C.c_void_p,
# ... 1 lines not shown
    "am_needle_estimate_device": (C.c_int, [C.c_int, C.POINTER(C.c_void_p), C.POINTER(C.c_size_t), C.c_size_t, C.c_int,
                                            C.POINTER(AmEstHit), C.c_size_t, C.POINTER(AmEstimateParams), C.c_void_p, C.c_void_p,
                                            C.c_void_p]),
    "am_set_option": (C.c_int, [C.c_char_p, C.c_longlong]),
    "am_match_best": (C.c_int, [C.c_void_p, C.c_void_p, C.c_size_t, C.c_int, C.POINTER(AmBestParams), C.POINTER(AmPeak),
                                C.POINTER(C.c_size_t)]),
    "am_match_best_device": (C.c_int, [C.c_void_p, C.c_void_p, C.c_size_t, C.c_int, C.POINTER(AmBestParams),
                                       C.POINTER(AmPeak), C.POINTER(C.c_size_t)]),
    "am_match_best_batch_device": (C.c_int, [C.c_void_p, C.POINTER(C.c_void_p), C.POINTER(C.c_size_t), C.c_size_t, C.c_int,
                                             C.POINTER(AmBestParams), C.POINTER(AmPeak), C.POINTER(C.c_size_t)]),
    "am_find_peaks_top": (C.c_int, [C.c_int, C.c_void_p, C.c_size_t, C.c_float, C.c_uint64, C.c_size_t,
                                    C.POINTER(AmPeak), C.POINTER(C.c_size_t)]),
    "am_trace_len": (C.c_int, [C.c_size_t, C.c_uint64, C.POINTER(C.c_size_t)]),
    "am_trace_scores": (C.c_int, [C.c_int, C.c_void_p, C.c_size_t, C.c_uint64, C.c_void_p, C.c_size_t, C.POINTER(C.c_size_t)]),
    "am_trace_scores_device": (C.c_int, [C.c_int, C.c_void_p, C.c_size_t, C.c_uint64, C.c_void_p, C.c_size_t,
                                         C.POINTER(C.c_size_t)]),
    "am_match_trace": (C.c_int, [C.c_void_p, C.c_void_p, C.c_size_t, C.c_int, C.POINTER(AmTraceParams), C.c_void_p, C.c_size_t,
                                 C.POINTER(C.c_size_t)]),
    "am_match_trace_device": (C.c_int, [C.c_void_p, C.c_void_p, C.c_size_t, C.c_int, C.POINTER(AmTraceParams), C.c_void_p,
                                        C.c_size_t, C.POINTER(C.c_size_t)]),
    "am_match_trace_batch_device": (C.c_int, [C.c_void_p, C.POINTER(C.c_void_p), C.POINTER(C.c_size_t), C.c_size_t, C.c_int,
                                              C.POINTER(AmTraceParams), C.c_void_p, C.c_size_t, C.POINTER(C.c_size_t)]),
    "am_trace_summary": (C.c_int, [C.c_void_p, C.c_size_t, C.c_uint64, C.POINTER(AmTraceStats)]),
    "am_find_peaks_top_device": (C.c_int, [C.c_int, C.c_void_p, C.c_size_t, C.c_float, C.c_uint64, C.c_size_t,
                                           C.POINTER(AmPeak), C.POINTER(C.c_size_t)]),
    "am_discover_len": (C.c_int, [C.c_size_t, C.POINTER(AmDiscoverParams), C.POINTER(C.c_size_t)]),
    "am_discover": (C.c_int, [C.c_int, C.c_void_p, C.c_size_t, C.c_void_p, C.c_size_t, C.c_int, C.POINTER(AmDiscoverParams),
                              C.c_void_p, C.c_size_t, C.POINTER(C.c_size_t)]),
    "am_discover_device": (C.c_int, [C.c_int, C.c_void_p, C.c_size_t, C.c_void_p, C.c_size_t, C.c_int,
                                     C.POINTER(AmDiscoverParams), C.c_void_p, C.c_size_t, C.POINTER(C.c_size_t)]),
    "am_probe_scores": (C.c_int, [C.c_int, C.c_void_p, C.c_size_t, C.c_uint64, C.c_uint64, C.c_uint64, C.c_void_p]),
    "am_probe_scores_device": (C.c_int, [C.c_int, C.c_void_p, C.c_size_t, C.c_uint64, C.c_uint64, C.c_uint64, C.c_void_p]),
    "am_discover_regions": (C.c_int, [C.c_void_p, C.c_size_t, C.POINTER(AmDiscoverParams), C.POINTER(AmRegionParams),
                                      C.c_void_p, C.c_size_t, C.POINTER(C.c_size_t)]),
    "am_get_option": (C.c_int, [C.c_char_p, C.POINTER(C.c_longlong)]),
}


def declared_symbols():
    return sorted(_SIGNATURES)


_lib = None


def lib():
    global _lib
    if _lib is None:
        if not os.path.exists(LIB_PATH):
            raise ImportError(
                f"{LIB_PATH} is missing: build it with `python audio-matcher_amd/build.py` "
                "(__graft_entry__.build()); there is no CPU fallback")
        L = C.CDLL(LIB_PATH)
        for name, (res, args) in _SIGNATURES.items():
            fn = getattr(L, name)
            fn.restype = res
            fn.argtypes = args
        _lib = L
    return _lib


def _check(rc: int):
    if rc != AM_OK:
        msg = lib().am_last_error_string()
        raise AudioMatchError(rc, msg.decode() if msg else "")


def device_count() -> int:
    n = C.c_int(0)
    rc = lib().am_device_count(C.byref(n))
    return n.value if rc == AM_OK else 0


def set_option(key: str, value: int):
    _check(lib().am_set_option(key.encode(), int(value)))


def get_option(key: str) -> int:
    v = C.c_longlong(0)
    _check(lib().am_get_option(key.encode(), C.byref(v)))
    return v.value


class DeviceBuffer:

    def __init__(self, device: int, nbytes: int):
        self.device, self.nbytes = device, int(nbytes)
        p = C.c_void_p()
        _check(lib().am_device_malloc(device, max(self.nbytes, 4), C.byref(p)))
        self.ptr = p.value

    @classmethod
    def from_numpy(cls, device: int, a: np.ndarray) -> "DeviceBuffer":
        a = np.ascontiguousarray(a)
        buf = cls(device, a.nbytes)
        if a.nbytes:
            _check(lib().am_memcpy_h2d(device, buf.ptr, a.ctypes.data, a.nbytes))
        return buf

    def to_numpy(self, dtype, count: int) -> np.ndarray:
        out = np.empty(count, dtype=dtype)
        if out.nbytes:
            _check(lib().am_memcpy_d2h(self.device, out.ctypes.data, self.ptr, out.nbytes))
        return out

    def free(self):
        if self.ptr:
            lib().am_device_free(self.device, self.ptr)
            self.ptr = None

    def __del__(self):
        try:
            self.free()
        except Exception:
            pass


class PinnedArray:

    def __init__(self, shape, dtype):
        self.nbytes = int(np.prod(shape)) * np.dtype(dtype).itemsize
        p = C.c_void_p()
        _check(lib().am_host_alloc(max(self.nbytes, 4), C.byref(p)))
        self.ptr = p.value
        self.array = np.frombuffer((C.c_char * self.nbytes).from_address(self.ptr), dtype=dtype).reshape(shape)

    def free(self):
        if self.ptr:
            self.array = None
            lib().am_host_free(self.ptr)
            self.ptr = None

    def __del__(self):
        try:
            self.free()
        except Exception:
            pass


class registered:

    def __init__(self, a: np.ndarray):
        self.a = a

    def __enter__(self):
        _check(lib().am_host_register(self.a.ctypes.data, self.a.nbytes))
        return self.a

    def __exit__(self, *exc):
        _check(lib().am_host_unregister(self.a.ctypes.data))


def synth_uniform_device(device: int, n: int, seed: int, stream: int, first: int = 0,
                         amp: float = 0.25) -> DeviceBuffer:
    buf = DeviceBuffer(device, n * 4)
    _check(lib().am_synth_uniform_device(device, buf.ptr, seed, stream, first, n, amp))
    return buf


def synth_pcm16_stereo_device(device: int, frames: int, seed: int, stream: int, first: int = 0,
                              amp: float = 0.25) -> DeviceBuffer:
    buf = DeviceBuffer(device, frames * 4)
    _check(lib().am_synth_pcm16_stereo_device(device, buf.ptr, seed, stream, first, frames, amp))
    return buf


# ... 1185 lines not shown
```

include/audiomatch.h:

```cpp
#ifndef AUDIOMATCH_H
#define AUDIOMATCH_H

#include <stddef.h>
#include <stdint.h>

#ifdef __cplusplus
extern "C" {
#endif

#define AM_ABI_VERSION 3

enum {
    AM_OK = 0,
    AM_ERR_INVALID_ARG = 1,
    AM_ERR_CAPACITY = 2,
    AM_ERR_HIP = 3,
    AM_ERR_NO_DEVICE = 4,
    AM_ERR_PEAK_OVERFLOW = 5,
    AM_ERR_OOM = 6
};

enum { AM_MODE_FULL = 0, AM_MODE_SAME = 1, AM_MODE_VALID = 2 };

enum { AM_SCALE_NONE = 0, AM_SCALE_LIB = 1, AM_SCALE_MY = 2 };
// ... 455 lines not shown
} am_stereo_summary;
int am_hit_stereo_summary(const am_stereo_hit* rec, float min_ncc, am_stereo_summary* out);

int am_device_malloc(int device, size_t bytes, void** out);
int am_device_free(int device, void* p);
int am_memcpy_h2d(int device, void* d_dst, const void* src, size_t bytes);
int am_memcpy_d2h(int device, void* dst, const void* d_src, size_t bytes);
int am_device_synchronize(int device);

int am_host_alloc(size_t bytes, void** out);
int am_host_free(void* p);
int am_host_register(void* p, size_t bytes);
int am_host_unregister(void* p);

int am_synth_uniform_device(int device, float* d_out, uint32_t seed, uint32_t stream,
                            uint64_t first, size_t n, float amp);
int am_axpy_device(int device, float* d_dst, const float* d_src, size_t n, float gain);

int am_synth_pcm16_stereo_device(int device, int16_t* d_out, uint32_t seed, uint32_t stream,
                                 uint64_t first, size_t frames, float amp);
int am_add_pcm16_device(int device, int16_t* d_dst, const int16_t* d_src, size_t frames);

int am_shard_plan(size_t n_items, size_t n_shards, size_t shard, size_t* first, size_t* stride, size_t* count);

typedef struct am_pool am_pool;
int am_pool_create(const float* needle, size_t n, const int* devices, size_t n_dev, am_pool** out);
void am_pool_destroy(am_pool* pool);
int am_pool_size(const am_pool* pool, size_t* n_dev);
int am_pool_slot(const am_pool* pool, size_t slot, int* device, const am_needle** needle);
int am_pool_match_batch(am_pool* pool, const float* const* haystacks, const size_t* lens, size_t n_hay,
                        const am_match_params* p, am_peak* out, size_t cap_per_hay, size_t* n_out);
int am_pool_match_batch_device(am_pool* pool, const float* const* d_haystacks, const size_t* lens, size_t n_hay,
                               const am_match_params* p, am_peak* out, size_t cap_per_hay, size_t* n_out);

int am_pool_match_batch_pcm16(am_pool* pool, const int16_t* const* interleaved, const size_t* frames, size_t n_hay,
                              const am_match_params* p, am_peak* out, size_t cap_per_hay, size_t* n_out);
int am_pool_match_batch_pcm16_device(am_pool* pool, const int16_t* const* d_interleaved, const size_t* frames, size_t n_hay,
                                     const am_match_params* p, am_peak* out, size_t cap_per_hay, size_t* n_out);
int am_pool_create_multi(const float* const* needles, size_t n_needles, size_t n, const int* devices, size_t n_dev, am_pool** out);
int am_pool_needle_count(const am_pool* pool, size_t* n_needles);
int am_pool_match_multi_batch(am_pool* pool, const void* const* haystacks, const size_t* lens, size_t n_hay, int sample_format,
                              const am_match_params* p, am_peak* out, size_t cap_per_pair, size_t* n_out);
int am_pool_match_multi_batch_device(am_pool* pool, const void* const* d_haystacks, const size_t* lens, size_t n_hay, int sample_format,
                                     const am_match_params* p, am_peak* out, size_t cap_per_pair, size_t* n_out);

int am_long_plan(size_t len, size_t needle_len, const am_match_params* p, size_t n_parts, size_t part,
                 size_t* first_window, size_t* n_windows, size_t* first_sample, size_t* n_samples);
int am_match_part_device(const am_needle* h, const void* d_part, size_t n_samples, int sample_format, const am_match_params* p,
                         size_t n_windows, uint64_t first_sample, am_peak* out, size_t cap, size_t* n_out);
int am_merge_peaks(const am_match_params* p, const am_peak* peaks, size_t n, am_peak* out, size_t cap, size_t* n_out);
int am_pool_match_long(am_pool* pool, const void* haystack, size_t len, int sample_format, const am_match_params* p,
                       am_peak* out, size_t cap, size_t* n_out);
int am_pool_match_long_device(am_pool* pool, const void* const* d_parts, size_t len, int sample_format, const am_match_params* p,
                              am_peak* out, size_t cap, size_t* n_out);

int am_merge_ready(const am_match_params* p, const am_peak* sorted, size_t n, uint64_t horizon, int ended, size_t* n_ready);

typedef struct am_monitor am_monitor;
int am_monitor_begin(const am_needle* const* needles, size_t n_needles, const am_match_params* params, int sample_format,
                     size_t group_windows, am_monitor** out);
int am_monitor_push(am_monitor* m, const void* samples, size_t n);
int am_monitor_poll(am_monitor* m, am_peak* out, uint32_t* needle, size_t cap, size_t* n_out);
int am_monitor_end(am_monitor* m, am_peak* out, uint32_t* needle, size_t cap, size_t* n_out);
typedef struct am_monitor_info {
    uint64_t received;
    uint64_t horizon;
    uint64_t resident_bytes;
    uint64_t pending;
} am_monitor_info;
int am_monitor_info_get(const am_monitor* m, am_monitor_info* info);
void am_monitor_destroy(am_monitor* m);

typedef void (*am_progress_fn)(void* user, size_t haystack_index, int stage, size_t n_chunks);
int am_set_progress_callback(am_progress_fn fn, void* user);
typedef void (*am_chunk_progress_fn)(void* user, size_t haystack_index, size_t chunk_index, size_t n_chunks, int stage);
int am_set_chunk_progress_callback(am_chunk_progress_fn fn, void* user);

int am_profile_enable(int device, int on);
int am_profile_reset(int device);
int am_profile_query(int device, const char* kernel, double* total_ms, uint64_t* launches);

int am_debug_column_bench(int device, int wide, int npairs, int iters, int dense, double* k1_ms, double* k3_ms);

int am_set_option(const char* key, long long value);
int am_get_option(const char* key, long long* value);
int am_needle_set_option(am_needle* h, const char* key, long long value);
int am_needle_get_option(const am_needle* h, const char* key, long long* value);

#ifdef __cplusplus
}
#endif
#endif
```

Baseline: 227.5 billion.

## Mirror tail-block spectrum to skip half the forward rows and inverse loads

For a single-block tail transform on the radix-16 plan, the forward column kernel now writes only the first 136 of 256 rows. The inverse kernel rebuilds the missing upper half from conjugate-symmetric mirrored rows with a twiddle correction, and the spectrum multiply processes only those rows. The scan of the unused second block in the tail is also skipped. This cuts memory traffic and arithmetic for the tail block, at the cost of more intricate indexing that could be wrong at edge rows; a debug score readback API is added as well.

New measurement: 227.4 billion. No clear change (-0.0%).

```diff
diff --git a/audio-matcher_amd/csrc/am_api.hip b/audio-matcher_amd/csrc/am_api.hip
--- a/audio-matcher_amd/csrc/am_api.hip
+++ b/audio-matcher_amd/csrc/am_api.hip
@@ -566,4 +566,21 @@
     return AM_OK;
 }
 
-}
+int am_debug_last_scores(int device, int which, int index, size_t first, size_t count, float* out) {
+    Ctx* c = nullptr;
+    int rc = get_ctx(device, &c);
+    if (rc) return rc;
+    std::lock_guard<std::recursive_mutex> lk(c->mu);
+    if (!out || index < 0) return fail(AM_ERR_INVALID_ARG, "bad arguments");
+    const DevBuf* b = nullptr;
+    if (which == 0 && index < 2) b = &c->side[index].scores;
+    else if (which == 1 && index < 2 * kMaxNeedleGroup) b = &c->grp_scores[index / kMaxNeedleGroup][index % kMaxNeedleGroup];
+    else if (which == 2) b = &c->tail_scores;
+    if (!b) return fail(AM_ERR_INVALID_ARG, "no such score buffer");
+    if (!b->p || first > b->cap / sizeof(float) || count > b->cap / sizeof(float) - first) return fail(AM_ERR_INVALID_ARG, "beyond the score buffer");
+    AM_HIP(hipDeviceSynchronize());
+    if (count) AM_HIP(hipMemcpy(out, static_cast<const float*>(b->p) + first, count * sizeof(float), hipMemcpyDeviceToHost));
+    return AM_OK;
+}
+
+}
diff --git a/audio-matcher_amd/csrc/am_context.hip b/audio-matcher_amd/csrc/am_context.hip
--- a/audio-matcher_amd/csrc/am_context.hip
+++ b/audio-matcher_amd/csrc/am_context.hip
@@ -57,6 +57,7 @@
     {"host_pick_wait", {1}, opt_bool, &Opts::host_pick_wait},
     {"device_redo", {1}, opt_bool, &Opts::device_redo},
     {"tail_block", {1}, opt_bool, &Opts::tail_block},
+    {"tail_mirror", {1}, opt_bool, &Opts::tail_mirror},
     {"dense_scores", {0}, opt_bool, &Opts::dense},
     {"score_norm", {0}, opt_score_norm, &Opts::score_norm},
     {"score_norm_floor_db", {60}, opt_floor_db, &Opts::score_norm_floor_db},
diff --git a/audio-matcher_amd/csrc/am_correlate.hip b/audio-matcher_amd/csrc/am_correlate.hip
--- a/audio-matcher_amd/csrc/am_correlate.hip
+++ b/audio-matcher_amd/csrc/am_correlate.hip
@@ -52,7 +52,7 @@
     return AM_OK;
 }
 bool tail_plan(size_t s, long long out_count, const Opts& o, const Geometry& g, TailPlan* t) {
-    t->on = false;
+    t->on = false; t->mirror = false;
     if (!o.tail_block || o.log_n != 0 || g.logN < 22 || !(g.nblocks & 1) || g.nblocks < 3 || (g.hop % kTile) != 0) return false;
     const long long T = (g.nblocks - 1) * g.hop, rest = out_count - T;
     for (int lt = 21; lt < g.logN; ++lt) {
@@ -63,6 +63,7 @@
         if (2 * hop < rest) continue;
         t->on = true; t->T = T;
         t->g.logN = lt; t->g.N = N; t->g.hop = hop; t->g.nblocks = (rest + hop - 1) / hop; t->g.npairs = 1;
+        t->mirror = o.tail_mirror != 0;
         return true;
     }
     return false;
@@ -162,9 +163,18 @@
     ScanCfg scan{};
     scan.stats32 = main_scan.stats32 ? main_scan.stats32 + tail.T / 32 : nullptr;
     scan.margin = -1.0f; scan.hist_min = FLT_MAX;
-    { ProfScope ps(c, KN_OTHER, st); AM_HIP(launch_k1(st, job, 1, (float2*)c->work_tail.p, pl, hs.level)); }
-    { ProfScope ps(c, KN_OTHER, st); AM_HIP(launch_k2(st, 1, (float2*)c->work_tail.p, pp.tail_hc, pl, nullptr, hs.level, hs.hscale, hs.pre, true)); }
-    { ProfScope ps(c, KN_OTHER, st); AM_HIP(launch_k3(st, job, 1, (const float2*)c->work_tail.p, pl, hs.k3(factor), scan, hs.level, false)); }
+    if (plan_is_r16(pl) && scan.stats32) {
+        TailBatch tb{};
+        tb.n = 1; tb.src[0] = job.src; tb.src_len[0] = job.src_len; tb.dst[0] = job.dst; tb.out_count[0] = job.out_count; tb.stats32[0] = scan.stats32;
+        const int rows = job.nblocks == 1 ? tail_mirror_rows(pl, hs.level, tail.mirror) : 0;
+        { ProfScope ps(c, KN_OTHER, st); AM_HIP(launch_tail_batch_k1(st, tb, job.hop, src_kind, (float2*)c->work_tail.p, pl, hs.level, rows)); }
+        { ProfScope ps(c, KN_OTHER, st); AM_HIP(launch_k2(st, 1, (float2*)c->work_tail.p, pp.tail_hc, pl, nullptr, hs.level, hs.hscale, hs.pre, true, rows)); }
+        { ProfScope ps(c, KN_OTHER, st); AM_HIP(launch_tail_batch_k3(st, tb, job.hop, (const float2*)c->work_tail.p, pl, hs.k3(factor), hs.level, tail.mirror)); }
+    } else {
+        { ProfScope ps(c, KN_OTHER, st); AM_HIP(launch_k1(st, job, 1, (float2*)c->work_tail.p, pl, hs.level)); }
+        { ProfScope ps(c, KN_OTHER, st); AM_HIP(launch_k2(st, 1, (float2*)c->work_tail.p, pp.tail_hc, pl, nullptr, hs.level, hs.hscale, hs.pre, true)); }
+        { ProfScope ps(c, KN_OTHER, st); AM_HIP(launch_k3(st, job, 1, (const float2*)c->work_tail.p, pl, hs.k3(factor), scan, hs.level, false)); }
+    }
     if (main_scan.stats32 && main_scan.margin >= 0.0f && main_scan.wbits && main_scan.tile_theta) {
         const BallotLayout bl = ballot_layout(pp.pl->dev.logN1, pp.pl->dev.logN2);
         const size_t blk = (size_t)(pp.g.nblocks - 1);
diff --git a/audio-matcher_amd/csrc/am_engine.hip b/audio-matcher_amd/csrc/am_engine.hip
--- a/audio-matcher_amd/csrc/am_engine.hip
+++ b/audio-matcher_amd/csrc/am_engine.hip
@@ -162,6 +162,7 @@
     const HalfScale& hs = lead.tail_hs;
     TailBatch tb{};
     tb.n = (int)members.size();
+    bool one_block = true;
     for (int j = 0; j < tb.n; ++j) {
         const size_t k = members[j];
         const size_t slot = (size_t)half_idx * kMaxTailBatch + (size_t)j;
@@ -171,11 +172,14 @@
         tb.out_count[j] = job.out_count;
         tb.dst[j] = static_cast<float*>(c->tail_scores.p) + slot * sl.scores;
         tb.stats32[j] = static_cast<float2*>(c->tail_stats.p) + slot * sl.stats;
+        one_block = one_block && job.nblocks == 1;
     }
     float2* work = static_cast<float2*>(c->work_tail.p);
-    { ProfScope ps(c, KN_OTHER); AM_HIP(launch_tail_batch_k1(c->stream, tb, (int)first.g.hop, src_kind, work, pl->dev, hs.level)); }
-    { ProfScope ps(c, KN_OTHER); AM_HIP(launch_k2(c->stream, tb.n, work, hc, pl->dev, nullptr, hs.level, hs.hscale, hs.pre, true)); }
-    { ProfScope ps(c, KN_OTHER); AM_HIP(launch_tail_batch_k3(c->stream, tb, (int)first.g.hop, work, pl->dev, hs.k3(factor), hs.level)); }
+    const bool mirror = first.mirror;
+    const int rows = one_block ? tail_mirror_rows(pl->dev, hs.level, mirror) : 0;
+    { ProfScope ps(c, KN_OTHER); AM_HIP(launch_tail_batch_k1(c->stream, tb, (int)first.g.hop, src_kind, work, pl->dev, hs.level, rows)); }
+    { ProfScope ps(c, KN_OTHER); AM_HIP(launch_k2(c->stream, tb.n, work, hc, pl->dev, nullptr, hs.level, hs.hscale, hs.pre, true, rows)); }
+    { ProfScope ps(c, KN_OTHER); AM_HIP(launch_tail_batch_k3(c->stream, tb, (int)first.g.hop, work, pl->dev, hs.k3(factor), hs.level, mirror)); }
     return AM_OK;
 }
 
@@ -631,14 +635,18 @@
         const int main_pairs = (int)(tail.on ? g.npairs - 1 : g.npairs);
         const Plan* plt = nullptr;
         Job job{}, job_t{};
+        int tail_rows = 0;
         job.src = d_hays[k]; job.src_len = (long long)lens[k]; job.lead = 0; job.src_kind = src_kind;
         job.out_count = tail.on ? tail.T : out_count; job.hop = (int)g.hop; job.nblocks = (int)(tail.on ? g.nblocks - 1 : g.nblocks); job.first_pair = 0;
         { ProfScope ps(c, KN_K1); AM_HIP(launch_k1(c->stream, job, main_pairs, (float2*)fwd.p, pl->dev, half)); }
         if (tail.on) {
             if ((rc = get_plan(c, tail.g.logN, &plt))) return rc;
             job_t = tail_job(tail, d_hays[k], (long long)lens[k], out_count, src_kind);
+            tail_rows = job_t.nblocks == 1 ? tail_mirror_rows(plt->dev, 0, tail.mirror) : 0;
+            TailBatch tb{};
+            tb.n = 1; tb.src[0] = job_t.src; tb.src_len[0] = job_t.src_len; tb.out_count[0] = job_t.out_count;
             ProfScope ps(c, KN_OTHER);
-            AM_HIP(launch_k1(c->stream, job_t, 1, (float2*)c->work_tail.p, plt->dev, 0));
+            AM_HIP(launch_tail_batch_k1(c->stream, tb, job_t.hop, src_kind, (float2*)c->work_tail.p, plt->dev, 0, tail_rows));
         }
         for (size_t i = 0; i < m; ++i) {
             am_needle* h = needles[ord[i]];
@@ -656,7 +664,7 @@
                     const std::vector<const float2*>& hct = hcs[tail.g.logN];
                     for (int q = 0; q < gt.n; ++q) { gt.hc[q] = hct[i + q]; gt.dst[q] = (float2*)c->work_tail2.p + (size_t)q * (size_t)tail.g.N; }
                     ProfScope ps(c, KN_OTHER);
-                    AM_HIP(launch_k2_group(c->stream, 1, (const float2*)c->work_tail.p, gt, plt->dev));
+                    AM_HIP(launch_k2_group(c->stream, 1, (const float2*)c->work_tail.p, gt, plt->dev, tail_rows));
                 }
             }
             const bool grouped_k3 = k3_group && group > 1 && gn > 1 && fused && !half && plan_k3_has_group(pl->dev);
@@ -705,7 +713,7 @@
                     ScanCfg dense{};
                     dense.stats32 = kt.stats32[0]; dense.margin = -1.0f; dense.hist_min = FLT_MAX;
                     ProfScope ps(c, KN_OTHER);
-                    AM_HIP(launch_k3_group(c->stream, job_t, 1, kt, plt->dev, dense));
+                    AM_HIP(launch_k3_group(c->stream, job_t, 1, kt, plt->dev, dense, tail.mirror ? 1 : 0));
                     if (margin >= 0.0f)
                         AM_HIP(launch_tail_preset_group(c->stream, kg, (long long)(g.nblocks - 1), pl->dev.logN1, pl->dev.logN2));
                 }
diff --git a/audio-matcher_amd/csrc/am_fft.hip b/audio-matcher_amd/csrc/am_fft.hip
--- a/audio-matcher_amd/csrc/am_fft.hip
+++ b/audio-matcher_amd/csrc/am_fft.hip
@@ -369,8 +369,9 @@
     twiddle_chain<16, false, true>(x1, w.base1, w.step1);
 }
 
+constexpr int kTailMirrorRows = 136;
 template <int KIND, int HALF>
-__device__ __forceinline__ void k1_cols_fwd_r16_tile(const Job& job, float2* __restrict__ work, const PlanDev& pl) {
+__device__ __forceinline__ void k1_cols_fwd_r16_tile(const Job& job, float2* __restrict__ work, const PlanDev& pl, int rows = 256) {
     extern __shared__ float4 lds4[];
     const int t = threadIdx.x;
     const int hi = t >> 4, cp = t & 15;
@@ -414,6 +415,7 @@
 #pragma unroll
     for (int bp = 0; bp < 16; ++bp) {
         const size_t k1 = (size_t)(hi + 16 * bp);
+        if (16 * bp + 15 >= kTailMirrorRows && (int)k1 >= rows) continue;
         out4[k1 * (kN2 / 2)] = make_float4(x0[brev<16>(bp)].x, x0[brev<16>(bp)].y,
                                              x1[brev<16>(bp)].x, x1[brev<16>(bp)].y);
     }
@@ -425,12 +427,12 @@
 }
 template <int KIND, int HALF>
 __global__ void __launch_bounds__(256, 3)
-tail_cols_fwd_r16(TailBatch tb, int hop, float2* __restrict__ work, PlanDev pl) {
+tail_cols_fwd_r16(TailBatch tb, int hop, float2* __restrict__ work, PlanDev pl, int rows) {
     const unsigned z = blockIdx.y;
     Job job;
     job.src = tb.src[z]; job.src_len = tb.src_len[z]; job.lead = 0; job.dst = nullptr; job.out_count = tb.out_count[z];
     job.hop = hop; job.nblocks = (int)((tb.out_count[z] + hop - 1) / hop); job.first_pair = -(int)z; job.src_kind = KIND;
-    k1_cols_fwd_r16_tile<KIND, HALF>(job, work, pl);
+    k1_cols_fwd_r16_tile<KIND, HALF>(job, work, pl, rows);
 }
 
 __device__ __forceinline__ void wave_sync_lds() {
@@ -1229,7 +1231,7 @@
     return e;
 }
 
-template <int HB, bool ACC = false, bool SCALED = false>
+template <int HB, bool ACC = false, bool SCALED = false, bool TAIL = false>
 __device__ __forceinline__ void k3_finish(const Job& job, const ScanCfg& scan, const K3Edges& ed, float2* lds2,
                                           int n2_0, int out_stride, int t, long long blkA, long long blkB,
                                           float out_scale, const float2 (&x0)[16], const float2 (&x1)[16]) {
@@ -1264,10 +1266,14 @@
         scan_put<HB>(lds2, hi, cp, sa0, sa1);
         wave_sync_lds();
         scan_row_minmax<HB>(lds4, row, wholeA, leftA < 32 ? leftA : 32, rmnA, rmxA);
-        wave_sync_lds();
-        scan_put<HB>(lds2, hi, cp, sb0, sb1);
-        wave_sync_lds();
-        scan_row_minmax<HB>(lds4, row, wholeB, leftB < 32 ? leftB : 32, rmnB, rmxB);
+        if (!TAIL || blkB < job.nblocks) {
+            wave_sync_lds();
+            scan_put<HB>(lds2, hi, cp, sb0, sb1);
+            wave_sync_lds();
+            scan_row_minmax<HB>(lds4, row, wholeB, leftB < 32 ? leftB : 32, rmnB, rmxB);
+        } else {
+            rmnB = FLT_MAX; rmxB = -FLT_MAX;
+        }
         float tminA = wave_min_f(leftA > 0 ? rmnA : FLT_MAX), tminB = wave_min_f(leftB > 0 ? rmnB : FLT_MAX);
         float* slots = reinterpret_cast<float*>(lds2 + scan_row_of<HB>(t & ~63) * 16);
         wave_sync_lds();
@@ -1343,7 +1349,7 @@
 }
 
 
-template <bool ACC = false>
+template <bool ACC = false, bool TAIL = false>
 __device__ __forceinline__ void k3_tile(const Job& job, const PlanDev& pl, const ScanCfg& scan, float2* lds2,
                                         int n2_0, int out_stride, int t, long long blkA, long long blkB,
                                         float out_scale, float2 (&x0)[16], float2 (&x1)[16], const ScanCfg* geo = nullptr) {
@@ -1382,7 +1388,7 @@
     for (int ap = 0; ap < 16; ++ap) x1[ap] = lds2[(ap * 16 + hi) * 16 + cp];
     twiddle_nat<16, true>(x1, w256, w256q);
     dif<16, true>(x1);
-    k3_finish<4, ACC, true>(job, scan, ed, lds2, n2_0, out_stride, t, blkA, blkB, out_scale, x0, x1);
+    k3_finish<4, ACC, true, TAIL>(job, scan, ed, lds2, n2_0, out_stride, t, blkA, blkB, out_scale, x0, x1);
 }
 
 __device__ __forceinline__ void k3_tile_h16(const Job& job, const PlanDev& pl, const ScanCfg& scan, float2* lds2,
@@ -1425,9 +1431,10 @@
 
 constexpr int kK3Waves = 3;
 constexpr int kK3LoadAux = 2, kK3hLoadAux = 2;
-template <int HALF, bool ACC>
+template <int HALF, bool ACC, bool TAIL = false>
 __device__ __forceinline__ void k3_cols_inv_r16_tile(unsigned lin, float4* lds4, const Job& job, const float2* __restrict__ work,
-                                                     const PlanDev& pl, float out_scale, const ScanCfg& scan, const ScanCfg* geo = nullptr) {
+                                                     const PlanDev& pl, float out_scale, const ScanCfg& scan, const ScanCfg* geo = nullptr,
+                                                     bool mirror = false) {
     const int t = threadIdx.x;
     const int hi = t >> 4, cp = t & 15;
     const unsigned xcd = lin & 7u, seq = lin >> 3;
@@ -1460,14 +1467,33 @@
     } else {
         const __amdgpu_buffer_rsrc_t rin = make_rsrc(work + ((size_t)slot << pl.logN) + n2_0, (unsigned)((((size_t)1 << pl.logN) - n2_0) * 8));
         const unsigned voff = (unsigned)hi * (kN2 * 8u) + (unsigned)cp * 16u;
-#pragma unroll
-        for (int bp = 0; bp < 16; ++bp) {
-            const float4 v = buf_load4<kK3LoadAux>(rin, voff, (unsigned)bp * (16u * kN2 * 8u));
-            x0[bp] = make_float2(v.x, v.y);
-            x1[bp] = make_float2(v.z, v.w);
-        }
-    }
-    k3_tile<ACC>(job, pl, scan, reinterpret_cast<float2*>(lds4), n2_0, kN2, t, blkA, blkB, out_scale, x0, x1, geo);
+        if (TAIL && mirror && blkB >= job.nblocks) {
+            const unsigned voffm = (hi ? 16u - (unsigned)hi : 16u) * (kN2 * 8u) + (unsigned)cp * 16u;
+            const unsigned n2 = (unsigned)n2_0 + 2u * (unsigned)cp, maskN = (1u << pl.logN) - 1u;
+            const float2 f0 = tw_big(pl, (n2 << kR16LogN1) & maskN), f1 = tw_big(pl, ((n2 + 1u) << kR16LogN1) & maskN);
+#pragma unroll
+            for (int bp = 0; bp < 8; ++bp) {
+                const float4 v = buf_load4<0>(rin, voff, (unsigned)bp * (16u * kN2 * 8u));
+                x0[bp] = make_float2(v.x, v.y);
+                x1[bp] = make_float2(v.z, v.w);
+            }
+#pragma unroll
+            for (int bp = 8; bp < 16; ++bp) {
+                const float4 v = buf_load4<kK3LoadAux>(rin, voffm, (unsigned)(15 - bp) * (16u * kN2 * 8u));
+                x0[bp] = make_float2(v.x * f0.x + v.y * f0.y, v.x * f0.y - v.y * f0.x);
+                x1[bp] = make_float2(v.z * f1.x + v.w * f1.y, v.z * f1.y - v.w * f1.x);
+                if (bp == 8 && hi == 0) { x0[bp] = make_float2(v.x, v.y); x1[bp] = make_float2(v.z, v.w); }
+            }
+        } else {
+#pragma unroll
+            for (int bp = 0; bp < 16; ++bp) {
+                const float4 v = buf_load4<kK3LoadAux>(rin, voff, (unsigned)bp * (16u * kN2 * 8u));
+                x0[bp] = make_float2(v.x, v.y);
+                x1[bp] = make_float2(v.z, v.w);
+            }
+        }
+    }
+    k3_tile<ACC, TAIL>(job, pl, scan, reinterpret_cast<float2*>(lds4), n2_0, kN2, t, blkA, blkB, out_scale, x0, x1, geo);
 }
 template <int HALF, bool ACC = false, int REDO = 0>
 __global__ void __launch_bounds__(256, REDO ? 4 : kK3Waves)
@@ -1497,7 +1523,7 @@
 
 template <int HALF>
 __global__ void __launch_bounds__(256, kK3Waves)
-tail_cols_inv_r16(TailBatch tb, int hop, const float2* __restrict__ work, PlanDev pl, float out_scale) {
+tail_cols_inv_r16(TailBatch tb, int hop, const float2* __restrict__ work, PlanDev pl, float out_scale, int mirror) {
     extern __shared__ float4 lds4[];
     const unsigned z = blockIdx.y;
     Job job;
@@ -1508,7 +1534,18 @@
     mine.seg_c = 0; mine.seg_d = 0; mine.inv_c = 0.0; mine.only_pairs = nullptr; mine.redo_tiles = 0; mine.edges_n = 0;
     const float2* mywork = HALF ? reinterpret_cast<const float2*>(reinterpret_cast<const unsigned*>(work) + ((size_t)z << pl.logN))
                                 : work + ((size_t)z << pl.logN);
-    k3_cols_inv_r16_tile<HALF, false>(blockIdx.x, lds4, job, mywork, pl, out_scale, mine);
+    k3_cols_inv_r16_tile<HALF, false, true>(blockIdx.x, lds4, job, mywork, pl, out_scale, mine, nullptr, HALF == 0 && mirror != 0);
+}
+__global__ void __launch_bounds__(256, kK3Waves)
+tail_cols_inv_r16_group(Job job, PlanDev pl, ScanCfg scan, K3Group grp, int mirror) {
+    extern __shared__ float4 lds4[];
+    const unsigned z = blockIdx.y;
+    job.dst = grp.dst[z]; job.out_count = grp.out_count[z];
+    ScanCfg mine;
+    mine.stats32 = grp.stats32[z]; mine.wbits = grp.wbits[z]; mine.tile_theta = grp.tile_theta[z]; mine.hist_min = grp.hist_min[z];
+    mine.margin = scan.margin; mine.seg_c = grp.seg_c; mine.seg_d = grp.seg_d[z]; mine.inv_c = grp.inv_c;
+    mine.only_pairs = nullptr; mine.redo_tiles = 0; mine.edges_n = 0;
+    k3_cols_inv_r16_tile<0, false, true>(blockIdx.x, lds4, job, grp.work[z], pl, grp.out_scale[z], mine, &scan, mirror != 0);
 }
 
 __global__ void __launch_bounds__(256)
@@ -2282,7 +2319,7 @@
      {{{k1_cols_fwd_c512<0, 0, 14>, 512, kC512Lds}}},
      {{{k1_cols_fwd_gen<kColsLog, 0>, kFftThreads, kMaxLds}}, {{k1_cols_fwd_gen<kColsLog, 1>, kFftThreads, kMaxLds}}},
 };
-using TailK1Fn = void (*)(TailBatch, int, float2*, PlanDev);
+using TailK1Fn = void (*)(TailBatch, int, float2*, PlanDev, int);
 static constexpr Variant<TailK1Fn> kTailK1[2][3] = {
     {{tail_cols_fwd_r16<0, 0>, 256, kR16LdsK1}, {tail_cols_fwd_r16<0, 1>, 256, kR16LdsK1}, {tail_cols_fwd_r16<0, 2>, 256, kR16LdsK1}},
     {{tail_cols_fwd_r16<1, 0>, 256, kR16LdsK1}, {tail_cols_fwd_r16<1, 1>, 256, kR16LdsK1}, {tail_cols_fwd_r16<1, 2>, 256, kR16LdsK1}},
@@ -2318,9 +2355,11 @@
 static constexpr Variant<K3GenFn> kK3Gen = {k3_cols_inv_gen<kColsLog>, kFftThreads, kMaxLds};
 using K3GroupFn = void (*)(Job, PlanDev, ScanCfg, K3Group);
 static constexpr Variant<K3GroupFn> kK3Group[kColGen] = {{k3_cols_inv_r16_group, 256, kR16LdsK3}, {k3_cols_inv_c512_group, 512, kC512Lds}};
-using TailK3Fn = void (*)(TailBatch, int, const float2*, PlanDev, float);
+using TailK3Fn = void (*)(TailBatch, int, const float2*, PlanDev, float, int);
 static constexpr Variant<TailK3Fn> kTailK3[3] = {
     {tail_cols_inv_r16<0>, 256, kR16LdsK3}, {tail_cols_inv_r16<1>, 256, kR16LdsK3}, {tail_cols_inv_r16<2>, 256, kR16LdsK3}};
+using TailK3GroupFn = void (*)(Job, PlanDev, ScanCfg, K3Group, int);
+static constexpr Variant<TailK3GroupFn> kTailK3Group = {tail_cols_inv_r16_group, 256, kR16LdsK3};
 
 template <typename Fn>
 static hipError_t allow_lds(const Variant<Fn>& v) {
@@ -2347,6 +2386,7 @@
     if (e == hipSuccess) e = allow_lds(kK3Gen);
     if (e == hipSuccess) e = allow_lds(kK3Group);
     if (e == hipSuccess) e = allow_lds(kTailK3);
+    if (e == hipSuccess) e = allow_lds(kTailK3Group);
     return e;
 }
 
@@ -2364,11 +2404,16 @@
 bool k2_mfma_enabled() { return g_k2_mfma.load(std::memory_order_relaxed) != 0; }
 int k2_mfma_table_dwords() { return kMfTotal; }
 
+static bool k2_rows_ok(int rows_per_pair, const PlanDev& pl) {
+    return rows_per_pair == 0 || (rows_per_pair > 0 && (rows_per_pair & 7) == 0 && rows_per_pair <= (1 << pl.logN1));
+}
 hipError_t launch_k2(hipStream_t st, int npairs, float2* work, const float2* hc, const PlanDev& pl, float2* dst,
-                     int half, float hscale, float pre, bool tail) {
+                     int half, float hscale, float pre, bool tail, int rows_per_pair) {
+    if (!k2_rows_ok(rows_per_pair, pl) || (rows_per_pair && !plan_k2_is_r16(pl))) return hipErrorInvalidValue;
     if (!plan_k2_is_r16(pl))
         return launch_row_lds(kK2Gen[0], dim3(1u << pl.logN1, npairs), sizeof(float2) << pl.logN2, st, work, hc, dst, pl);
-    const unsigned rows = (unsigned)npairs << pl.logN1;
+    const unsigned rows = rows_per_pair ? (unsigned)npairs * (unsigned)rows_per_pair
+                                        : (unsigned)npairs << pl.logN1;
     if (half == 2) {
         unsigned* const w = reinterpret_cast<unsigned*>(work);
         const unsigned* const h = reinterpret_cast<const unsigned*>(hc);
@@ -2384,9 +2429,10 @@
 
 bool plan_k2_has_group(const PlanDev& pl) { return plan_k2_is_r16(pl); }
 
-hipError_t launch_k2_group(hipStream_t st, int npairs, const float2* work, const K2Group& grp, const PlanDev& pl) {
-    if (!plan_k2_has_group(pl) || grp.n < 1 || grp.n > kMaxNeedleGroup) return hipErrorInvalidValue;
-    return launch_row(kK2Group, dim3((unsigned)npairs << pl.logN1), st, work, grp, pl, (unsigned)npairs);
+hipError_t launch_k2_group(hipStream_t st, int npairs, const float2* work, const K2Group& grp, const PlanDev& pl, int rows_per_pair) {
+    if (!plan_k2_has_group(pl) || grp.n < 1 || grp.n > kMaxNeedleGroup || !k2_rows_ok(rows_per_pair, pl)) return hipErrorInvalidValue;
+    const unsigned rows = rows_per_pair ? (unsigned)npairs * (unsigned)rows_per_pair : (unsigned)npairs << pl.logN1;
+    return launch_row(kK2Group, dim3(rows), st, work, grp, pl, (unsigned)npairs);
 }
 
 hipError_t launch_k2_spectrum(hipStream_t st, float2* work, float2* hc_out, const PlanDev& pl) {
@@ -2417,14 +2463,16 @@
 
 bool plan_k3_has_group(const PlanDev& pl) { return plan_is_c512(pl) || plan_is_r16(pl); }
 
-hipError_t launch_tail_batch_k1(hipStream_t st, const TailBatch& tb, int hop, int src_kind, float2* work, const PlanDev& pl, int half) {
+int tail_mirror_rows(const PlanDev& pl, int half, bool mirror) { return (mirror && !half && plan_is_r16(pl)) ? kTailMirrorRows : 0; }
+hipError_t launch_tail_batch_k1(hipStream_t st, const TailBatch& tb, int hop, int src_kind, float2* work, const PlanDev& pl, int half, int rows) {
+    if (!plan_is_r16(pl) || tb.n < 1 || tb.n > kMaxTailBatch || (rows != 0 && (half || rows != kTailMirrorRows))) return hipErrorInvalidValue;
+    const dim3 grid((1u << pl.logN2) >> kColsLog, (unsigned)tb.n);
+    return launch_row(kTailK1[src_kind == 1 ? 1 : 0][half_level(half)], grid, st, tb, hop, work, pl, rows ? rows : 1 << kR16LogN1);
+}
+hipError_t launch_tail_batch_k3(hipStream_t st, const TailBatch& tb, int hop, const float2* work, const PlanDev& pl, float out_scale, int half,
+                                bool mirror) {
     if (!plan_is_r16(pl) || tb.n < 1 || tb.n > kMaxTailBatch) return hipErrorInvalidValue;
-    const dim3 grid((1u << pl.logN2) >> kColsLog, (unsigned)tb.n);
-    return launch_row(kTailK1[src_kind == 1 ? 1 : 0][half_level(half)], grid, st, tb, hop, work, pl);
-}
-hipError_t launch_tail_batch_k3(hipStream_t st, const TailBatch& tb, int hop, const float2* work, const PlanDev& pl, float out_scale, int half) {
-    if (!plan_is_r16(pl) || tb.n < 1 || tb.n > kMaxTailBatch) return hipErrorInvalidValue;
-    return launch_row(kTailK3[half_level(half)], dim3(kN2 >> kColsLog, (unsigned)tb.n), st, tb, hop, work, pl, out_scale);
+    return launch_row(kTailK3[half_level(half)], dim3(kN2 >> kColsLog, (unsigned)tb.n), st, tb, hop, work, pl, out_scale, mirror && !half ? 1 : 0);
 }
 hipError_t launch_tail_preset_group(hipStream_t st, const K3Group& grp, long long blk, int log_n1, int log_n2) {
     if (grp.n < 1 || grp.n > kMaxNeedleGroup) return hipErrorInvalidValue;
@@ -2439,13 +2487,15 @@
     return hipGetLastError();
 }
 
-hipError_t launch_k3_group(hipStream_t st, const Job& job, int npairs, const K3Group& grp, const PlanDev& pl, const ScanCfg& scan_in) {
+hipError_t launch_k3_group(hipStream_t st, const Job& job, int npairs, const K3Group& grp, const PlanDev& pl, const ScanCfg& scan_in, int tail_mirror) {
     if (!plan_k3_has_group(pl) || grp.n < 1 || grp.n > kMaxNeedleGroup || scan_in.stats32 == nullptr) return hipErrorInvalidValue;
+    if (tail_mirror >= 0 && (!plan_is_r16(pl) || npairs != 1)) return hipErrorInvalidValue;
     for (int z = 0; z < grp.n; ++z) if (grp.out_count[z] > job.out_count) return hipErrorInvalidValue;
     ScanCfg scan = scan_in;
     scan.only_pairs = nullptr;
     fill_edges(job, npairs, scan);
     const dim3 grid((unsigned)npairs * (kN2 >> kColsLog), (unsigned)grp.n);
+    if (tail_mirror >= 0) return launch_row(kTailK3Group, grid, st, job, pl, scan, grp, tail_mirror);
     return launch_row(kK3Group[col_plan(pl)], grid, st, job, pl, scan, grp);
 }
 
diff --git a/audio-matcher_amd/csrc/am_internal.h b/audio-matcher_amd/csrc/am_internal.h
--- a/audio-matcher_amd/csrc/am_internal.h
+++ b/audio-matcher_amd/csrc/am_internal.h
@@ -34,7 +34,7 @@
 
 struct Opts {
     long long log_n, pairs_per_group, half, batch_overlap, needle_group, dense, device_redo, debug_no_realloc, debug_redo_arm_at;
-    long long peak_filter_order, distance_rule, tail_window, surrounding_from, k3_group, pick_group, tail_block, host_pick_wait;
+    long long peak_filter_order, distance_rule, tail_window, surrounding_from, k3_group, pick_group, tail_block, tail_mirror, host_pick_wait;
     long long profile_mask, profile_every, pick_priority;
     long long score_norm, score_norm_floor_db;
     long long trace_form;
@@ -234,6 +234,7 @@
     bool on;
     long long T;
     Geometry g;
+    bool mirror;
 };
 struct HalfScale {
     int level;
diff --git a/audio-matcher_amd/csrc/am_kernels.h b/audio-matcher_amd/csrc/am_kernels.h
--- a/audio-matcher_amd/csrc/am_kernels.h
+++ b/audio-matcher_amd/csrc/am_kernels.h
@@ -43,7 +43,7 @@
 
 hipError_t launch_k1(hipStream_t st, const Job& job, int npairs, float2* work, const PlanDev& pl, int half = 0);
 hipError_t launch_k2(hipStream_t st, int npairs, float2* work, const float2* hc, const PlanDev& pl, float2* dst = nullptr,
-                     int half = 0, float hscale = 1.0f, float pre = 1.0f, bool tail = false);
+                     int half = 0, float hscale = 1.0f, float pre = 1.0f, bool tail = false, int rows_per_pair = 0);
 hipError_t launch_spectrum_to_half(hipStream_t st, const float2* hc, long long n, float scale, unsigned* out);
 void set_k2_mfma(int on);
 bool k2_mfma_enabled();
@@ -57,7 +57,7 @@
     int n;
 };
 bool plan_k2_has_group(const PlanDev& pl);
-hipError_t launch_k2_group(hipStream_t st, int npairs, const float2* work, const K2Group& grp, const PlanDev& pl);
+hipError_t launch_k2_group(hipStream_t st, int npairs, const float2* work, const K2Group& grp, const PlanDev& pl, int rows_per_pair = 0);
 struct ScanCfg {
     float2* stats32;
     unsigned long long* wbits;
@@ -98,12 +98,14 @@
     long long out_count[kMaxTailBatch];
     float2* stats32[kMaxTailBatch];
 };
-hipError_t launch_tail_batch_k1(hipStream_t st, const TailBatch& tb, int hop, int src_kind, float2* work, const PlanDev& pl, int half);
-hipError_t launch_tail_batch_k3(hipStream_t st, const TailBatch& tb, int hop, const float2* work, const PlanDev& pl, float out_scale, int half);
+int tail_mirror_rows(const PlanDev& pl, int half, bool mirror);
+hipError_t launch_tail_batch_k1(hipStream_t st, const TailBatch& tb, int hop, int src_kind, float2* work, const PlanDev& pl, int half, int rows = 0);
+hipError_t launch_tail_batch_k3(hipStream_t st, const TailBatch& tb, int hop, const float2* work, const PlanDev& pl, float out_scale, int half,
+                                bool mirror = false);
 hipError_t launch_tail_preset_group(hipStream_t st, const K3Group& grp, long long blk, int log_n1, int log_n2);
 hipError_t launch_tail_commit(hipStream_t st, const float* tail_scores, float* scores, long long n, const float2* tail_stats32, float2* stats32,
                               unsigned long long* wbits, long long words, float* theta, int tiles);
-hipError_t launch_k3_group(hipStream_t st, const Job& job, int npairs, const K3Group& grp, const PlanDev& pl, const ScanCfg& scan);
+hipError_t launch_k3_group(hipStream_t st, const Job& job, int npairs, const K3Group& grp, const PlanDev& pl, const ScanCfg& scan, int tail_mirror = -1);
 constexpr int kDirectMaxNeedle = 64;
 hipError_t launch_direct(hipStream_t st, const Job& job, const float* needle, int s, float out_scale);
 bool plan_is_r16(const PlanDev& pl);
diff --git a/audio-matcher_amd/python/audiomatch_amd/__init__.py b/audio-matcher_amd/python/audiomatch_amd/__init__.py
--- a/audio-matcher_amd/python/audiomatch_amd/__init__.py
+++ b/audio-matcher_amd/python/audiomatch_amd/__init__.py
@@ -369,6 +369,7 @@
     "am_match_stream_finish": (C.c_int, [C.c_void_p, C.POINTER(AmPeak), C.c_size_t, C.POINTER(C.c_size_t)]),
     "am_match_stream_destroy": (None, [C.c_void_p]),
     "am_debug_column_bench": (C.c_int, [C.c_int, C.c_int, C.c_int, C.c_int, C.c_int, C.POINTER(C.c_double), C.POINTER(C.c_double)]),
+    "am_debug_last_scores": (C.c_int, [C.c_int, C.c_int, C.c_int, C.c_size_t, C.c_size_t, C.c_void_p]),
     "am_profile_enable": (C.c_int, [C.c_int, C.c_int]),
     "am_profile_reset": (C.c_int, [C.c_int]),
     "am_profile_query": (C.c_int, [C.c_int, C.c_char_p, C.POINTER(C.c_double), C.POINTER(C.c_uint64)]),
@@ -536,6 +537,12 @@
     return v.value
 
 
+def debug_last_scores(which: int, index: int, first: int, count: int, device: int = 0) -> np.ndarray:
+    out = np.empty(count, dtype=np.float32)
+    _check(lib().am_debug_last_scores(device, which, index, first, count, out.ctypes.data))
+    return out
+
+
 class DeviceBuffer:
 
     def __init__(self, device: int, nbytes: int):
diff --git a/include/audiomatch.h b/include/audiomatch.h
--- a/include/audiomatch.h
+++ b/include/audiomatch.h
@@ -561,6 +561,8 @@
 
 int am_debug_column_bench(int device, int wide, int npairs, int iters, int dense, double* k1_ms, double* k3_ms);
 
+int am_debug_last_scores(int device, int which, int index, size_t first, size_t count, float* out);
+
 int am_set_option(const char* key, long long value);
 int am_get_option(const char* key, long long* value);
 int am_needle_set_option(am_needle* h, const char* key, long long value);
```
